# acappemin/Video-to-Audio-and-Piano-RP

Measured on AMD Instinct MI355X. Metric: mel-frames/sec (10s VGGSound shape, 32-step CFM, CFG 2.0), higher is better.
Workload: dtype bf16x3; 1 GPU; BASELINE.json configs[1]: 1 clip(s)/GPU x 750 latent frames x 128 ch, 32-point sway grid = 31 CFG evaluations (62 DiT forwards), T5 context 16 tokens, V2A zero roll; clips_per_gpu=1, global_clips=1, parallelism=clip-sharded x1, 1 all-gather, hipgraph=True, schedule=three streams, side_streams=True, cascade_passes=1

## Files before the change

include/v2a_cfm.h:

```cpp
#ifndef V2A_CFM_H
#define V2A_CFM_H

#include <stdint.h>

#ifdef __cplusplus
extern "C" {
#endif

typedef void* v2a_stream_t;

enum {
  V2A_F32 = 0,
  V2A_BF16 = 1,
  V2A_BF16_SPLIT = 2
};

enum {
  V2A_OK = 0,
  V2A_ERR_ARG = -1,
  V2A_ERR_LAUNCH = -2
};

int v2a_abi_version(void);
const char* v2a_last_error(void);

enum {
  V2A_EPI_STORE = 0,
  V2A_EPI_SIGMOID = 1,
  V2A_EPI_GEGLU = 2,
  V2A_EPI_RESID = 3,
  V2A_EPI_GATE_RESID = 4,
  V2A_EPI_GEGLU_TANH = 5,
  V2A_EPI_GELU = 6,
  V2A_EPI_SWIGLU = 7
};

typedef struct v2a_gemm_args {
  const void* a[3];
  int64_t lda[3];
  int32_t ka[3];
  int32_t nseg;
  int32_t a_dtype;
  const void* w;
  int64_t ldw;
  const float* bias;
  int32_t M, N;
  int32_t compute_dtype;
  int32_t epilogue;
  void* out;
  int64_t ldo;
  int32_t out_dtype;
  void* out_bf16;
  int64_t ld_out_bf16;
  const float* resid;
  int64_t ldr;
  const float* gate;
  const int32_t* step;
  int64_t gate_step_stride, gate_batch_stride;
  int32_t rows_per_batch;
  const float* rope_table;
  int32_t rope_cols, rope_pos_offset;
  int32_t relu;
  const int32_t* a_row_offset;
  const int32_t* a_ktile_offset;
  const int32_t* out_row_offset;
  int32_t tile_hint;
  const float* norm_gamma;
  int64_t norm_step_stride, norm_batch_stride;
  int32_t norm_switch_row, norm_switch_offset;
  float* norm_ssq;
  int64_t ld_norm_ssq;
  const float* row_ssq;
  int64_t ld_row_ssq;
  int32_t row_ssq_parts, row_norm_dim;
  int32_t out_bf16_split;
  int64_t a_lo_offset[3];
  int64_t out_bf16_lo_offset;
} v2a_gemm_args;

int v2a_gemm(const v2a_gemm_args* args, v2a_stream_t stream);
int v2a_gemm_args_size(void);

enum { V2A_GEMM_REGISTER_STAGED = 0, V2A_GEMM_RING = 1, V2A_GEMM_8PHASE = 2 };
typedef struct v2a_gemm_choice {
  int32_t family;
  int32_t split;
  int32_t bm, bn, bk;
  int32_t waves_m, waves_n;
  int32_t stages;
  int32_t tiles;
  int32_t xcd_gm, xcd_gn;
  int32_t vec_epi;
} v2a_gemm_choice;
int v2a_gemm_choose(const v2a_gemm_args* args, v2a_gemm_choice* choice);

typedef struct v2a_tuning {
  int32_t gemm_force_tile;
  int32_t gemm_k_rotation;
  int32_t gemm_8phase;
  int32_t gemm_8phase_min_tiles;
  int32_t dwconv_rows_per_wave;
  int32_t gemm_xcd_order_1x8;
  int32_t attn_one_group_from;
  int32_t reserved[1];
} v2a_tuning;
int v2a_set_tuning(const v2a_tuning* tuning);

int v2a_rmsnorm(const float* x, int64_t ldx, void* y, int64_t ldy, int32_t y_dtype,
                int64_t rows, int32_t d,
                const float* gamma, const int32_t* step, int64_t gamma_step_stride,
                int64_t gamma_batch_stride, int32_t rows_per_batch, v2a_stream_t stream);

int v2a_dwconv_silu_residual(const float* x, float* out, const float* wt, const float* bias,
                             int32_t B, int32_t N, int32_t d, int32_t ksize,
                             const int32_t* len, v2a_stream_t stream);
typedef struct v2a_dwconv_norm {
  void* out_bf16;
  int64_t ld_out_bf16;
  const float* norm_gamma;
  const int32_t* step;
  int64_t norm_step_stride, norm_batch_stride;
  float* norm_ssq;
  int64_t ld_norm_ssq;
  int32_t split;
  int32_t reserved;
} v2a_dwconv_norm;
int v2a_dwconv_silu_residual_norm(const float* x, float* out, const float* wt, const float* bias,
                                  int32_t B, int32_t N, int32_t d, int32_t ksize,
                                  const int32_t* len, const v2a_dwconv_norm* norm, v2a_stream_t stream);

int v2a_rope_inplace(void* qk, int32_t dtype, int64_t rows, int64_t row_stride, int32_t nheads,
                     int32_t rows_per_batch, int32_t pos_offset, const float* cs_table,
                     int32_t layout, v2a_stream_t stream);

typedef struct v2a_attn_args {
  const void *q, *k, *v, *gate;
  void* out;
  int64_t q_row_stride, k_row_stride, v_row_stride, gate_row_stride, out_row_stride;
  int64_t q_batch_stride, k_batch_stride, v_batch_stride, gate_batch_stride, out_batch_stride;
  int32_t B, H, Nq, Nk;
  const int32_t* kv_len;
  const int32_t* q_len;
  float scale, softclamp;
  int32_t dtype;
  int32_t out_split;
} v2a_attn_args;

int v2a_attention(const v2a_attn_args* args, v2a_stream_t stream);
int v2a_qproj_xattn(const v2a_gemm_args* gemm, const v2a_attn_args* attn, v2a_stream_t stream);

typedef struct v2a_xattn_prepare_args {
  const float* ctx_kv;
  int64_t ctx_ld;
  int32_t k_col, v_col;
  const float* wq;
  const float* wo;
  void* wqk;
  void* wvo;
  int32_t B, L, H, D, nc, KP;
} v2a_xattn_prepare_args;
int v2a_xattn_absorb_prepare(const v2a_xattn_prepare_args* args, v2a_stream_t stream);

typedef struct v2a_xattn_absorbed_args {
  const void* a;
  int64_t lda;
  int32_t K, M;
  const void* wqk;
  int64_t ldw, w_batch_stride;
  const float* gate_bias;
  void* out;
  int64_t ldo;
  int32_t rows_per_batch, B, H, KP;
  const int32_t* kv_len;
  const int32_t* q_len;
  float scale, softclamp;
  const float* row_ssq;
  int64_t ld_row_ssq;
  int32_t row_ssq_parts, row_norm_dim;
} v2a_xattn_absorbed_args;
int v2a_xattn_absorbed(const v2a_xattn_absorbed_args* args, v2a_stream_t stream);

int v2a_linear_small(const float* a, int64_t M, int32_t K, const float* wt, const float* bias,
                     const float* add, int32_t T, float* out, int64_t out_batch_stride,
                     int32_t row_off, int32_t d, int32_t dup_batch_offset,
                     const float* regs ,
                     void* out_bf16 , v2a_stream_t stream);

int v2a_fill_registers(float* out, int64_t out_batch_stride, const float* regs, int32_t B,
                       int32_t R, int32_t d, v2a_stream_t stream);

int v2a_time_cond(const float* t, int32_t S, const float* fourier_w, const float* wt,
                  const float* bias, float* out, int32_t d, v2a_stream_t stream);

int v2a_apg_reduce(const float* pred, double* apg, int32_t B, int32_t T, int32_t C,
                   int64_t pred_batch_stride, int32_t row_off,
                   const int32_t* valid_rows ,
                   v2a_stream_t stream);
int v2a_cfg_euler(float* y, const float* pred, int32_t B, int32_t T, int32_t C,
                  int64_t pred_batch_stride, int32_t row_off, float cfg_strength,
                  const float* dt, const int32_t* step, const double* apg,
                  float keep_parallel_frac, v2a_stream_t stream);
typedef struct v2a_y_planes {
  void* planes;
  int64_t ld;
  int64_t lo_offset;
  int32_t row_off;
  int32_t rows_per_seq;
  int32_t copies;
  int32_t reserved;
} v2a_y_planes;
int v2a_cfg_euler_planes(float* y, const float* pred, int32_t B, int32_t T, int32_t C,
                         int64_t pred_batch_stride, int32_t row_off, float cfg_strength,
                         const float* dt, const int32_t* step, const double* apg,
                         float keep_parallel_frac, const v2a_y_planes* planes, v2a_stream_t stream);
int v2a_split_bf16(const float* x, int64_t ldx, void* y, int64_t ldy, int64_t rows, int32_t d, v2a_stream_t stream);
int v2a_cast_bf16(const float* x, void* y, int64_t n, v2a_stream_t stream);
int v2a_step_advance(int32_t* step, v2a_stream_t stream);


int v2a_im2col(const float* x, int32_t B, int32_t H, int32_t W, int32_t C, int32_t kh, int32_t kw, int32_t stride,
               int32_t pad, int32_t Ho, int32_t Wo, void* col, int64_t ldo, int32_t out_dtype, int32_t window_t,
               int32_t window_first, v2a_stream_t stream);

int v2a_frames_pack(const float* frames, void* out, int32_t T, int32_t H, int32_t W, int32_t kw, int32_t stride, int32_t pad,
                    int32_t Wo, v2a_stream_t stream);
int v2a_frames_pack_split(const float* frames, void* out, int64_t lo_offset, int32_t T, int32_t H, int32_t W, int32_t kw,
                          int32_t stride, int32_t pad, int32_t Wo, v2a_stream_t stream);

int v2a_pool2d(const float* x, float* out, void* out_bf16, int32_t B, int32_t H, int32_t W, int32_t C, int32_t k,
               int32_t stride, int32_t pad, int32_t mode, int32_t Ho, int32_t Wo, int32_t in_border, int32_t out_border,
               v2a_stream_t stream);
int v2a_pool2d_split(const float* x, float* out, void* out_split, int64_t lo_offset, int32_t B, int32_t H, int32_t W, int32_t C,
                     int32_t k, int32_t stride, int32_t pad, int32_t mode, int32_t Ho, int32_t Wo, int32_t in_border,
                     int32_t out_border, v2a_stream_t stream);

typedef struct v2a_roll_head_args {
  const float *x2, *x3, *x4, *x5;
  int32_t B, P;
  const float *frb4_w1t, *frb4_b1, *frb4_w2t, *frb4_b2;
  const float *frb3_w1t, *frb3_b1, *frb3_w2t, *frb3_b2;
  const float *frb2_w1t, *frb2_b1, *frb2_w2t, *frb2_b2;
  const float *conv2_wt, *conv2_b;
  const float *fc_wt, *fc_b;
  int32_t notes;
  int32_t apply_sigmoid;
  float* out;
} v2a_roll_head_args;
int v2a_roll_head(const v2a_roll_head_args* args, v2a_stream_t stream);

int v2a_roll_expand(const float* roll, float* out, int32_t B, int32_t t, int32_t notes, int32_t rep, int32_t l,
                    v2a_stream_t stream);

int v2a_roll_expand_ratio(const float* roll, float* out, int32_t B, int32_t t, int32_t notes, int32_t rep, int32_t group, int32_t l,
                          v2a_stream_t stream);


int v2a_elu_pad(const float* x, float* out, int64_t T, int32_t C, int32_t pad, int32_t reflect, int32_t act,
                v2a_stream_t stream);

int v2a_lstm_layer(const float* gates_x, const float* w_hh, float* h, const float* resid, float* y, int32_t T, int32_t H,
                   int32_t* workspace, v2a_stream_t stream);

int v2a_lstm2(const float* gates_x0, const float* w_hh0, const float* w_ih1, const float* bias1, const float* w_hh1,
              const float* resid, float* y, int32_t T, int32_t H, int32_t* workspace, v2a_stream_t stream);


int v2a_elu_pad_lr(const float* x, float* out, int64_t T, int32_t C, int32_t pad_left, int32_t pad_right, int32_t act,
                   v2a_stream_t stream);

int v2a_encodec_stage0(const float* wave, const float* params, float* out, int64_t n, v2a_stream_t stream);


int v2a_t5_rmsnorm(const float* x, int64_t ldx, const int32_t* ids, int32_t vocab, float* resid, int64_t ldr, float* y, int64_t ldy,
                   int64_t rows, int32_t d, const float* w, float eps, v2a_stream_t stream);

typedef struct v2a_t5_attn_args {
  const float *q, *k, *v;
  float* out;
  int64_t q_row_stride, k_row_stride, v_row_stride, out_row_stride;
  int64_t q_batch_stride, k_batch_stride, v_batch_stride, out_batch_stride;
  int32_t B, H, N, d_kv;
  const float* bias;
  const int32_t* key_mask;
} v2a_t5_attn_args;
int v2a_t5_attention(const v2a_t5_attn_args* args, v2a_stream_t stream);

int v2a_gemm_skinny_f32(const v2a_gemm_args* args, v2a_stream_t stream);


int v2a_clip_resize_h(const uint8_t* frames, int32_t F, int32_t H, int32_t W, uint8_t* tmp, int32_t y0, int32_t rows, int32_t S,
                      const int32_t* bounds, const int32_t* coef, int32_t ksize, v2a_stream_t stream);
int v2a_clip_resize_v(const uint8_t* tmp, int32_t F, int32_t rows, int32_t S, int32_t P, const int32_t* bounds, const int32_t* coef,
                      int32_t ksize, const float* lut, void* patches, int64_t ldp, int32_t out_dtype, int64_t lo_offset, uint8_t* crop,
                      v2a_stream_t stream);
int v2a_clip_embed_init(float* h, int64_t ldh, int64_t rows, int32_t T, int32_t d, const float* cls, const float* pos,
                        v2a_stream_t stream);
int v2a_clip_layernorm(const float* x, int64_t ldx, void* y, int64_t ldy, int32_t y_dtype, int64_t rows, int32_t d, const float* gamma,
                       const float* beta, float eps, v2a_stream_t stream);
typedef struct v2a_clip_attn_args {
  const float *q, *k, *v;
  void* out;
  int64_t row_stride, batch_stride;
  int64_t out_row_stride, out_batch_stride;
  int32_t B, H, N, d_head;
  float scale;
  int32_t out_split;
} v2a_clip_attn_args;
int v2a_clip_attention(const v2a_clip_attn_args* args, v2a_stream_t stream);


int v2a_piano_resize_h(const uint8_t* frames, int32_t F, int32_t H, int32_t W, const int32_t* sel, int32_t n, uint8_t* tmp, int32_t ldt,
                       int32_t y0, int32_t rows, int32_t Wo, const int32_t* bounds, const int32_t* coef, int32_t ksize,
                       v2a_stream_t stream);
int v2a_piano_resize_v(const uint8_t* tmp, int32_t n, int32_t rows, int32_t ldt, int32_t Ho, int32_t Wo, const int32_t* bounds,
                       const int32_t* coef, int32_t ksize, const float* lut, float* out, v2a_stream_t stream);
int v2a_piano_resize_vt(const uint8_t* tmp, int32_t n, int32_t rows, int32_t ldt, int32_t Ho, int32_t Wo, const int32_t* bounds,
                        const int32_t* coef, int32_t ksize, const float* lut, float* out, v2a_stream_t stream);


int v2a_encodec_rvq_encode(const float* x, int64_t batch_stride, int64_t frame_stride, int64_t chan_stride, int32_t B, int32_t T,
                           const float* codebooks, const float* norms, int32_t S, int32_t Kc, int32_t D, int32_t n_q, int64_t* codes,
                           v2a_stream_t stream);
int v2a_encodec_rvq_decode(const int64_t* codes, int32_t n_q, int32_t B, int32_t T, const float* codebooks, int32_t S, int32_t Kc, int32_t D,
                           float* out, int64_t batch_stride, int64_t frame_stride, int64_t chan_stride, v2a_stream_t stream);


#define V2A_LOSS_MAX_PARTS 256

int v2a_cfm_interp(const float* x0, const float* x1, const float* t, const uint8_t* span, float* w, float* flow, float* cond, int32_t B,
                   int32_t T, int32_t C, v2a_stream_t stream);
int v2a_masked_sqerr(const float* pred, const float* target, const uint8_t* mask, int32_t B, int32_t T, int32_t C, double* scratch,
                     double* out, v2a_stream_t stream);
int v2a_roll_metrics(const float* roll, const float* midis, const uint8_t* mask, int32_t B, int32_t T, int32_t notes, double* scratch,
                     double* out, v2a_stream_t stream);


#define V2A_WAVE_MAX_PARTS 256
#define V2A_WAVE_LDS_BYTES (128 * 1024)
#define V2A_WAVE_TABLE_MAX (1 << 22)

int v2a_wave_resample(const float* x, int64_t L, const float* table, int32_t o, int32_t n, int32_t K, int32_t width, float* y,
                      int64_t out_len, void* parts, int32_t* n_parts, v2a_stream_t stream);
int v2a_wave_stats(const float* x, int64_t n, void* parts, int32_t* n_parts, v2a_stream_t stream);
int v2a_wave_normalize(const float* x, int64_t n, const void* parts, int32_t n_parts, float* out, int64_t n_out, float* stats,
                       v2a_stream_t stream);


int v2a_roll2midi_stem(const float* x, const float* wt, int32_t n, int32_t H, int32_t W, int32_t co, float* out, void* shadow,
                       int32_t shadow_mode, int64_t lo_offset, int64_t pitch, int32_t border, v2a_stream_t stream);
int v2a_leaky_shadow(float* x, void* shadow, int32_t shadow_mode, int64_t lo_offset, int32_t n, int32_t H, int32_t W, int32_t C,
                     int64_t pitch, int32_t border, v2a_stream_t stream);
int v2a_roll2midi_head(const float* u, int64_t u_pitch, int32_t nu, const float* d, int64_t d_pitch, int32_t nd, const float* w,
                       float bias, float threshold, int32_t n, int32_t H, int32_t W, int32_t border, float* logits, float* probs,
                       uint8_t* midi, v2a_stream_t stream);
int v2a_roll2midi_gate(float* x0, int64_t pitch0, int32_t C0, void* shadow0, int64_t lo_offset0, float* x1, int64_t pitch1, int32_t C1,
                       void* shadow1, int64_t lo_offset1, const float* w, float bias, int32_t shadow_mode, int32_t n, int32_t H, int32_t W,
                       int32_t border, float* logits, float* alpha, v2a_stream_t stream);


#define V2A_ROLL_NOTES_MAX_KEYS 128
#define V2A_ROLL_NOTES_TILE 256
#define V2A_ROLL_NOTES_MAX_FRAMES (1 << 24)

int v2a_roll_notes(const void* roll, int32_t elem_bytes, int64_t batch_stride, int64_t frame_stride, int64_t key_stride, float threshold,
                   int32_t B, int32_t T, int32_t keys, const int32_t* lens, int32_t* counts, int32_t* totals, int32_t* notes, int32_t cap,
                   int8_t* onset, v2a_stream_t stream);


#define V2A_MEL_MAX_FFT 2048
#define V2A_MEL_MAX_CHUNKS 16
// ... 27 lines not shown
```

video-to-audio-and-piano-rp_amd/_lib.py:

```python
from __future__ import annotations

import ctypes as C
import os
import subprocess
from typing import NamedTuple

import torch

_HERE = os.path.dirname(os.path.abspath(__file__))
LIB_PATH = os.path.join(_HERE, "libv2a_cfm.so")
CSRC = os.path.join(_HERE, "csrc")

F32, BF16, BF16_SPLIT = 0, 1, 2
EPI_STORE, EPI_SIGMOID, EPI_GEGLU, EPI_RESID, EPI_GATE_RESID = 0, 1, 2, 3, 4
EPI_GEGLU_TANH = 5
EPI_GELU = 6
EPI_SWIGLU = 7

_lib = None


class V2AError(RuntimeError):
    pass


class GemmArgs(C.Structure):
    _fields_ = [
        ("a", C.c_void_p * 3), ("lda", C.c_int64 * 3), ("ka", C.c_int32 * 3),
        ("nseg", C.c_int32), ("a_dtype", C.c_int32),
        ("w", C.c_void_p), ("ldw", C.c_int64), ("bias", C.c_void_p),
        ("M", C.c_int32), ("N", C.c_int32), ("compute_dtype", C.c_int32), ("epilogue", C.c_int32),
        ("out", C.c_void_p), ("ldo", C.c_int64), ("out_dtype", C.c_int32),
        ("out_bf16", C.c_void_p), ("ld_out_bf16", C.c_int64),
        ("resid", C.c_void_p), ("ldr", C.c_int64),
        ("gate", C.c_void_p), ("step", C.c_void_p),
        ("gate_step_stride", C.c_int64), ("gate_batch_stride", C.c_int64), ("rows_per_batch", C.c_int32),
        ("rope_table", C.c_void_p), ("rope_cols", C.c_int32), ("rope_pos_offset", C.c_int32), ("relu", C.c_int32),
        ("a_row_offset", C.c_void_p), ("a_ktile_offset", C.c_void_p), ("out_row_offset", C.c_void_p),
        ("tile_hint", C.c_int32),
        ("norm_gamma", C.c_void_p), ("norm_step_stride", C.c_int64), ("norm_batch_stride", C.c_int64),
        ("norm_switch_row", C.c_int32), ("norm_switch_offset", C.c_int32),
        ("norm_ssq", C.c_void_p), ("ld_norm_ssq", C.c_int64),
        ("row_ssq", C.c_void_p), ("ld_row_ssq", C.c_int64), ("row_ssq_parts", C.c_int32), ("row_norm_dim", C.c_int32),
        ("out_bf16_split", C.c_int32),
        ("a_lo_offset", C.c_int64 * 3), ("out_bf16_lo_offset", C.c_int64),
    ]


class GemmChoice(C.Structure):
    _fields_ = [(n, C.c_int32) for n in ("family", "split", "bm", "bn", "bk", "waves_m", "waves_n", "stages", "tiles", "xcd_gm", "xcd_gn",
                                         "vec_epi")]


GEMM_REGISTER_STAGED, GEMM_RING, GEMM_8PHASE = 0, 1, 2

TILE_128x128, TILE_8PHASE, TILE_128x128_8WAVES, TILE_128x64_8WAVES = 1, 6, 12, 14
SPLIT_TILE_8PHASE, SPLIT_TILE_128x256_K32 = 5, 6


class DwconvNorm(C.Structure):
    _fields_ = [("out_bf16", C.c_void_p), ("ld_out_bf16", C.c_int64), ("norm_gamma", C.c_void_p), ("step", C.c_void_p),
                ("norm_step_stride", C.c_int64), ("norm_batch_stride", C.c_int64), ("norm_ssq", C.c_void_p), ("ld_norm_ssq", C.c_int64),
                ("split", C.c_int32), ("reserved", C.c_int32)]


class Tuning(C.Structure):
    _fields_ = [("gemm_force_tile", C.c_int32), ("gemm_k_rotation", C.c_int32), ("gemm_8phase", C.c_int32),
                ("gemm_8phase_min_tiles", C.c_int32), ("dwconv_rows_per_wave", C.c_int32), ("gemm_xcd_order_1x8", C.c_int32),
                ("attn_one_group_from", C.c_int32), ("reserved", C.c_int32 * 1)]


class AttnArgs(C.Structure):
    _fields_ = [
        ("q", C.c_void_p), ("k", C.c_void_p), ("v", C.c_void_p), ("gate", C.c_void_p), ("out", C.c_void_p),
        ("q_row_stride", C.c_int64), ("k_row_stride", C.c_int64), ("v_row_stride", C.c_int64),
        ("gate_row_stride", C.c_int64), ("out_row_stride", C.c_int64),
        ("q_batch_stride", C.c_int64), ("k_batch_stride", C.c_int64), ("v_batch_stride", C.c_int64),
        ("gate_batch_stride", C.c_int64), ("out_batch_stride", C.c_int64),
        ("B", C.c_int32), ("H", C.c_int32), ("Nq", C.c_int32), ("Nk", C.c_int32),
        ("kv_len", C.c_void_p), ("q_len", C.c_void_p),
        ("scale", C.c_float), ("softclamp", C.c_float), ("dtype", C.c_int32), ("out_split", C.c_int32),
    ]


class XattnPrepareArgs(C.Structure):
    _fields_ = [("ctx_kv", C.c_void_p), ("ctx_ld", C.c_int64), ("k_col", C.c_int32), ("v_col", C.c_int32),
                ("wq", C.c_void_p), ("wo", C.c_void_p), ("wqk", C.c_void_p), ("wvo", C.c_void_p)] + \
               [(n, C.c_int32) for n in ("B", "L", "H", "D", "nc", "KP")]


class XattnAbsorbedArgs(C.Structure):
    _fields_ = [("a", C.c_void_p), ("lda", C.c_int64), ("K", C.c_int32), ("M", C.c_int32),
                ("wqk", C.c_void_p), ("ldw", C.c_int64), ("w_batch_stride", C.c_int64), ("gate_bias", C.c_void_p),
                ("out", C.c_void_p), ("ldo", C.c_int64),
                ("rows_per_batch", C.c_int32), ("B", C.c_int32), ("H", C.c_int32), ("KP", C.c_int32),
                ("kv_len", C.c_void_p), ("q_len", C.c_void_p), ("scale", C.c_float), ("softclamp", C.c_float),
                ("row_ssq", C.c_void_p), ("ld_row_ssq", C.c_int64), ("row_ssq_parts", C.c_int32), ("row_norm_dim", C.c_int32)]


class YPlanes(C.Structure):
    _fields_ = [("planes", C.c_void_p), ("ld", C.c_int64), ("lo_offset", C.c_int64), ("row_off", C.c_int32), ("rows_per_seq", C.c_int32),
                ("copies", C.c_int32), ("reserved", C.c_int32)]


class T5AttnArgs(C.Structure):
    _fields_ = [
        ("q", C.c_void_p), ("k", C.c_void_p), ("v", C.c_void_p), ("out", C.c_void_p),
        ("q_row_stride", C.c_int64), ("k_row_stride", C.c_int64), ("v_row_stride", C.c_int64), ("out_row_stride", C.c_int64),
        ("q_batch_stride", C.c_int64), ("k_batch_stride", C.c_int64), ("v_batch_stride", C.c_int64), ("out_batch_stride", C.c_int64),
        ("B", C.c_int32), ("H", C.c_int32), ("N", C.c_int32), ("d_kv", C.c_int32),
        ("bias", C.c_void_p), ("key_mask", C.c_void_p),
    ]


class ClipAttnArgs(C.Structure):
    _fields_ = [("q", C.c_void_p), ("k", C.c_void_p), ("v", C.c_void_p), ("out", C.c_void_p),
                ("row_stride", C.c_int64), ("batch_stride", C.c_int64), ("out_row_stride", C.c_int64), ("out_batch_stride", C.c_int64),
                ("B", C.c_int32), ("H", C.c_int32), ("N", C.c_int32), ("d_head", C.c_int32), ("scale", C.c_float), ("out_split", C.c_int32)]


class RollHeadArgs(C.Structure):
    _fields_ = ([(n, C.c_void_p) for n in ("x2", "x3", "x4", "x5")] + [("B", C.c_int32), ("P", C.c_int32)] +
                [(f"frb{i}_{n}", C.c_void_p) for i in (4, 3, 2) for n in ("w1t", "b1", "w2t", "b2")] +
                [(n, C.c_void_p) for n in ("conv2_wt", "conv2_b", "fc_wt", "fc_b")] +
                [("notes", C.c_int32), ("apply_sigmoid", C.c_int32), ("out", C.c_void_p)])


EXPORTS = [
    "v2a_abi_version", "v2a_last_error", "v2a_gemm", "v2a_gemm_args_size", "v2a_gemm_choose", "v2a_set_tuning", "v2a_rmsnorm", "v2a_dwconv_silu_residual", "v2a_dwconv_silu_residual_norm",
    "v2a_rope_inplace", "v2a_attention", "v2a_qproj_xattn", "v2a_linear_small", "v2a_fill_registers", "v2a_time_cond",
    "v2a_apg_reduce", "v2a_cfg_euler", "v2a_step_advance", "v2a_cast_bf16", "v2a_split_bf16",
    "v2a_im2col", "v2a_frames_pack", "v2a_pool2d", "v2a_roll_head", "v2a_roll_expand", "v2a_frames_pack_split", "v2a_pool2d_split",
    "v2a_elu_pad", "v2a_lstm_layer", "v2a_lstm2", "v2a_t5_rmsnorm", "v2a_t5_attention", "v2a_gemm_skinny_f32",
    "v2a_clip_resize_h", "v2a_clip_resize_v", "v2a_clip_embed_init", "v2a_clip_layernorm", "v2a_clip_attention",
    "v2a_elu_pad_lr", "v2a_encodec_stage0", "v2a_piano_resize_h", "v2a_piano_resize_v",
    "v2a_encodec_rvq_encode", "v2a_encodec_rvq_decode", "v2a_cfm_interp", "v2a_masked_sqerr", "v2a_roll_metrics",
    "v2a_wave_resample", "v2a_wave_stats", "v2a_wave_normalize",
    "v2a_roll2midi_stem", "v2a_leaky_shadow", "v2a_roll2midi_head", "v2a_roll2midi_gate",
    "v2a_xattn_absorb_prepare", "v2a_xattn_absorbed",
    "v2a_roll_expand_ratio", "v2a_piano_resize_vt",
    "v2a_roll_notes",
    "v2a_cfg_euler_planes",
    "v2a_mel_pad", "v2a_mel_from_dft",
    "v2a_vocos_stage_in", "v2a_vocos_dwconv_ln", "v2a_vocos_gelu", "v2a_vocos_scale_residual", "v2a_vocos_spectrum", "v2a_vocos_overlap_add",
]


def build(force: bool = False, verbose: bool = False) -> str:
    if force:
        for f in os.listdir(os.path.join(CSRC, "build")) if os.path.isdir(os.path.join(CSRC, "build")) else []:
            os.remove(os.path.join(CSRC, "build", f))
    r = subprocess.run(["bash", os.path.join(CSRC, "build.sh")], capture_output=True, text=True)
    if verbose or r.returncode != 0:
        print(r.stdout[-4000:])
        print(r.stderr[-8000:])
    if r.returncode != 0:
        raise V2AError("hipcc build of libv2a_cfm.so failed")
    return LIB_PATH


ABI_VERSION = 9


def _declare(lib):
    vp, i32, i64, f32 = C.c_void_p, C.c_int32, C.c_int64, C.c_float
    lib.v2a_abi_version.restype = C.c_int
    lib.v2a_last_error.restype = C.c_char_p
    lib.v2a_gemm.argtypes = [C.POINTER(GemmArgs), vp]
    lib.v2a_gemm_args_size.restype = C.c_int
    lib.v2a_gemm_choose.argtypes = [C.POINTER(GemmArgs), C.POINTER(GemmChoice)]
    lib.v2a_set_tuning.argtypes = [C.POINTER(Tuning)]
    lib.v2a_attention.argtypes = [C.POINTER(AttnArgs), vp]
    lib.v2a_qproj_xattn.argtypes = [C.POINTER(GemmArgs), C.POINTER(AttnArgs), vp]
    lib.v2a_xattn_absorb_prepare.argtypes = [C.POINTER(XattnPrepareArgs), vp]
    lib.v2a_xattn_absorbed.argtypes = [C.POINTER(XattnAbsorbedArgs), vp]
    lib.v2a_rmsnorm.argtypes = [vp, i64, vp, i64, i32, i64, i32, vp, vp, i64, i64, i32, vp]
    lib.v2a_dwconv_silu_residual.argtypes = [vp, vp, vp, vp, i32, i32, i32, i32, vp, vp]
    lib.v2a_dwconv_silu_residual_norm.argtypes = [vp, vp, vp, vp, i32, i32, i32, i32, vp, C.POINTER(DwconvNorm), vp]
    lib.v2a_rope_inplace.argtypes = [vp, i32, i64, i64, i32, i32, i32, vp, i32, vp]
    lib.v2a_linear_small.argtypes = [vp, i64, i32, vp, vp, vp, i32, vp, i64, i32, i32, i32, vp, vp, vp]
    lib.v2a_fill_registers.argtypes = [vp, i64, vp, i32, i32, i32, vp]
    lib.v2a_time_cond.argtypes = [vp, i32, vp, vp, vp, vp, i32, vp]
    lib.v2a_apg_reduce.argtypes = [vp, vp, i32, i32, i32, i64, i32, vp, vp]
    lib.v2a_cfg_euler.argtypes = [vp, vp, i32, i32, i32, i64, i32, f32, vp, vp, vp, f32, vp]
    lib.v2a_cfg_euler_planes.argtypes = [vp, vp, i32, i32, i32, i64, i32, f32, vp, vp, vp, f32, C.POINTER(YPlanes), vp]
    lib.v2a_step_advance.argtypes = [vp, vp]
    lib.v2a_cast_bf16.argtypes = [vp, vp, i64, vp]
    lib.v2a_split_bf16.argtypes = [vp, i64, vp, i64, i64, i32, vp]
    lib.v2a_im2col.argtypes = [vp, i32, i32, i32, i32, i32, i32, i32, i32, i32, i32, vp, i64, i32, i32, i32, vp]
    lib.v2a_frames_pack.argtypes = [vp, vp, i32, i32, i32, i32, i32, i32, i32, vp]
    lib.v2a_pool2d.argtypes = [vp, vp, vp, i32, i32, i32, i32, i32, i32, i32, i32, i32, i32, i32, i32, vp]
    lib.v2a_frames_pack_split.argtypes = [vp, vp, i64, i32, i32, i32, i32, i32, i32, i32, vp]
    lib.v2a_pool2d_split.argtypes = [vp, vp, vp, i64, i32, i32, i32, i32, i32, i32, i32, i32, i32, i32, i32, i32, vp]
    lib.v2a_roll_head.argtypes = [C.POINTER(RollHeadArgs), vp]
    lib.v2a_roll_expand.argtypes = [vp, vp, i32, i32, i32, i32, i32, vp]
    lib.v2a_roll_expand_ratio.argtypes = [vp, vp, i32, i32, i32, i32, i32, i32, vp]
    lib.v2a_elu_pad.argtypes = [vp, vp, i64, i32, i32, i32, i32, vp]
    lib.v2a_lstm_layer.argtypes = [vp, vp, vp, vp, vp, i32, i32, vp, vp]
    lib.v2a_lstm2.argtypes = [vp, vp, vp, vp, vp, vp, vp, i32, i32, vp, vp]
    lib.v2a_t5_rmsnorm.argtypes = [vp, i64, vp, i32, vp, i64, vp, i64, i64, i32, vp, f32, vp]
    lib.v2a_t5_attention.argtypes = [C.POINTER(T5AttnArgs), vp]
    lib.v2a_gemm_skinny_f32.argtypes = [C.POINTER(GemmArgs), vp]
    lib.v2a_clip_resize_h.argtypes = [vp, i32, i32, i32, vp, i32, i32, i32, vp, vp, i32, vp]
    lib.v2a_clip_resize_v.argtypes = [vp, i32, i32, i32, i32, vp, vp, i32, vp, vp, i64, i32, i64, vp, vp]
    lib.v2a_clip_embed_init.argtypes = [vp, i64, i64, i32, i32, vp, vp, vp]
    lib.v2a_clip_layernorm.argtypes = [vp, i64, vp, i64, i32, i64, i32, vp, vp, f32, vp]
    lib.v2a_clip_attention.argtypes = [C.POINTER(ClipAttnArgs), vp]
    lib.v2a_elu_pad_lr.argtypes = [vp, vp, i64, i32, i32, i32, i32, vp]
    lib.v2a_encodec_stage0.argtypes = [vp, vp, vp, i64, vp]
    lib.v2a_piano_resize_h.argtypes = [vp, i32, i32, i32, vp, i32, vp, i32, i32, i32, i32, vp, vp, i32, vp]
    lib.v2a_piano_resize_v.argtypes = [vp, i32, i32, i32, i32, i32, vp, vp, i32, vp, vp, vp]
    lib.v2a_piano_resize_vt.argtypes = lib.v2a_piano_resize_v.argtypes
    lib.v2a_encodec_rvq_encode.argtypes = [vp, i64, i64, i64, i32, i32, vp, vp, i32, i32, i32, i32, vp, vp]
    lib.v2a_encodec_rvq_decode.argtypes = [vp, i32, i32, i32, vp, i32, i32, i32, vp, i64, i64, i64, vp]
    lib.v2a_cfm_interp.argtypes = [vp, vp, vp, vp, vp, vp, vp, i32, i32, i32, vp]
    lib.v2a_masked_sqerr.argtypes = [vp, vp, vp, i32, i32, i32, vp, vp, vp]
    lib.v2a_roll_metrics.argtypes = [vp, vp, vp, i32, i32, i32, vp, vp, vp]
    lib.v2a_wave_resample.argtypes = [vp, i64, vp, i32, i32, i32, i32, vp, i64, vp, C.POINTER(i32), vp]
    lib.v2a_wave_stats.argtypes = [vp, i64, vp, C.POINTER(i32), vp]
    lib.v2a_wave_normalize.argtypes = [vp, i64, vp, i32, vp, i64, vp, vp]
    lib.v2a_roll2midi_stem.argtypes = [vp, vp, i32, i32, i32, i32, vp, vp, i32, i64, i64, i32, vp]
    lib.v2a_leaky_shadow.argtypes = [vp, vp, i32, i64, i32, i32, i32, i32, i64, i32, vp]
    lib.v2a_roll2midi_head.argtypes = [vp, i64, i32, vp, i64, i32, vp, f32, f32, i32, i32, i32, i32, vp, vp, vp, vp]
    lib.v2a_roll2midi_gate.argtypes = [vp, i64, i32, vp, i64, vp, i64, i32, vp, i64, vp, f32, i32, i32, i32, i32, i32, vp, vp, vp]
    lib.v2a_roll_notes.argtypes = [vp, i32, i64, i64, i64, f32, i32, i32, i32, vp, vp, vp, vp, i32, vp, vp]
    lib.v2a_mel_pad.argtypes = [vp, i64, i32, i64, i32, vp, i64, vp]
    lib.v2a_mel_from_dft.argtypes = [vp, i64, i64, i32, i64, i32, i32, i32, i32, i32, vp, vp, vp, i32, i32, f32, vp, i64, i64, vp]
    lib.v2a_vocos_stage_in.argtypes = [vp, i64, i64, i32, i32, i32, vp, vp, i32, vp]
    lib.v2a_vocos_dwconv_ln.argtypes = [vp, i64, vp, vp, vp, vp, f32, i32, i32, i64, i32, vp, vp, i64, vp]
    lib.v2a_vocos_gelu.argtypes = [vp, i64, i64, i32, vp]
    lib.v2a_vocos_scale_residual.argtypes = [vp, i64, vp, vp, i64, vp, i64, i64, i32, vp]
    lib.v2a_vocos_spectrum.argtypes = [vp, i64, i64, i32, vp, i64, vp]
    lib.v2a_vocos_overlap_add.argtypes = [vp, i64, i64, vp, i32, i32, i32, i32, vp, vp, i64, vp]
    for name in EXPORTS:
        if name not in ("v2a_abi_version", "v2a_last_error", "v2a_gemm_args_size"):
            getattr(lib, name).restype = C.c_int


def lib():
    global _lib
    if _lib is None:
        if not os.path.exists(LIB_PATH):
            raise V2AError(f"{LIB_PATH} is missing: run `python -c 'import __graft_entry__ as g; g.build()'` "
                           "(hipcc --offload-arch=gfx950).  There is no CPU fallback for the sampler.")
        _lib = C.CDLL(LIB_PATH)
        _declare(_lib)
        if _lib.v2a_abi_version() != ABI_VERSION:
            raise V2AError("libv2a_cfm.so reports ABI version %d, this binding was written for %d: rebuild (csrc/build.sh)"
                           % (_lib.v2a_abi_version(), ABI_VERSION))
        if _lib.v2a_gemm_args_size() != C.sizeof(GemmArgs):
            raise V2AError("libv2a_cfm.so was built with sizeof(v2a_gemm_args) = %d, this binding mirrors %d bytes: rebuild "
                           "(csrc/build.sh)" % (_lib.v2a_gemm_args_size(), C.sizeof(GemmArgs)))
    return _lib


def set_tuning(force_tile: int = -1, k_rotation: bool = False, eight_phase: int | None = None, eight_phase_min_tiles: int = 0,
               dwconv_rows_per_wave: int = 0, xcd_order_1x8: bool = False, attn_one_group_from: int = 0, reserved: int = 0):
    if (force_tile == -1 and not k_rotation and eight_phase is None and eight_phase_min_tiles == 0 and dwconv_rows_per_wave == 0
            and not xcd_order_1x8 and attn_one_group_from == 0 and not reserved):
        check(lib().v2a_set_tuning(None))
        return
    t = Tuning(force_tile, 1 if k_rotation else 0, 1 if eight_phase is None else eight_phase, eight_phase_min_tiles, dwconv_rows_per_wave,
               1 if xcd_order_1x8 else 0, attn_one_group_from, (C.c_int32 * 1)(reserved))
    check(lib().v2a_set_tuning(C.byref(t)))


def check(rc: int):
    if rc != 0:
        raise V2AError(f"v2a_cfm call failed ({rc}): {lib().v2a_last_error().decode()}")


def stream_ptr() -> int:
    return torch.cuda.current_stream().cuda_stream


def dt_code(t: torch.dtype) -> int:
    if t == torch.float32:
        return F32
    if t == torch.bfloat16:
        return BF16
    raise V2AError(f"unsupported dtype {t}")


def _p(t):
    return 0 if t is None else t.data_ptr()


class Operand(NamedTuple):
    t: torch.Tensor
    ld: int
    k: int
    lo: int = 0


def split_planes(w):
    w = w.float()
    hi = w.bfloat16()
    return torch.cat([hi, (w - hi.float()).bfloat16()], 1)


_prof = None


class KernelProfiler:

    def __init__(self, shapes: bool = False, inner: int = 1, external: bool = False):
        self.recs = []
        self.shapes = shapes
        self.inner = inner
        self.external = external
        self.marks, self.end, self.tot = [], None, {}

    def launch(self, key, flops, nbytes, call):
        if self.external:
            e = torch.cuda.Event(enable_timing=True, external=True)
            e.record()
            self.marks.append((key, flops, nbytes, e))
            call()
            return
        n = self.inner if key.startswith("gemm") else 1
        s, e = torch.cuda.Event(enable_timing=True), torch.cuda.Event(enable_timing=True)
        s.record()
        for _ in range(n):
            call()
        e.record()
        self.recs.append((key, flops, nbytes, s, e, n))

    def close(self):
        self.end = torch.cuda.Event(enable_timing=True, external=True)
        self.end.record()

    def collect(self):
        for i, (key, flops, nbytes, e) in enumerate(self.marks):
            nxt = self.marks[i + 1][3] if i + 1 < len(self.marks) else self.end
            a = self.tot.setdefault(key, dict(launches=0, ms=0.0, flops=0.0, bytes=0.0))
            a["launches"] += 1
            a["ms"] += e.elapsed_time(nxt)
            a["flops"] += flops
            a["bytes"] += nbytes
# ... 106 lines not shown
    _launch("rmsnorm<%s>" % ("f32" if y.dtype == torch.float32 else ("bf16x2" if split else "bf16")), 0.0,
            rows * d * (4 + y.element_size() * (2 if split else 1)),
            lambda: lib().v2a_rmsnorm(x.data_ptr(), ldx or d, y.data_ptr(), ldy or d, ydt, rows, d,
                                      gamma.data_ptr(), _p(step), gamma_step_stride, gamma_batch_stride, rows_per_batch,
                                      stream_ptr()))


def _dwconv_norm(norm, d):
    n = DwconvNorm()
    n.out_bf16, n.ld_out_bf16 = norm["out_bf16"].data_ptr(), norm.get("ld_out_bf16", d)
    n.norm_gamma, n.step = norm["gamma"].data_ptr(), _p(norm.get("step"))
    n.norm_step_stride, n.norm_batch_stride = norm.get("step_stride", 0), norm.get("batch_stride", 0)
    n.norm_ssq, n.ld_norm_ssq = norm["ssq"].data_ptr(), norm["ssq"].stride(-2)
    n.split = 1 if norm.get("split") else 0
    if n.split:
        n.ld_out_bf16 = norm.get("ld_out_bf16", 2 * d)
    return n


def dwconv(x, out, wt, bias, *, B, N, d, ksize, lens=None, norm=None):
    if norm is None:
        _launch("dwconv", 2.0 * B * N * d * ksize, B * N * d * 8,
                lambda: lib().v2a_dwconv_silu_residual(x.data_ptr(), out.data_ptr(), wt.data_ptr(), bias.data_ptr(),
                                                       B, N, d, ksize, _p(lens), stream_ptr()))
        return
    n = _dwconv_norm(norm, d)
    _launch("dwconv+norm", 2.0 * B * N * d * ksize, B * N * d * (12 if n.split else 10),
            lambda: lib().v2a_dwconv_silu_residual_norm(x.data_ptr(), out.data_ptr(), wt.data_ptr(), bias.data_ptr(),
                                                        B, N, d, ksize, _p(lens), C.byref(n), stream_ptr()))


def rope(qk, *, rows, row_stride, nheads, rows_per_batch, pos_offset, table, layout):
    _launch("rope<%s>" % ("f32" if qk.dtype == torch.float32 else "bf16"), 0.0, rows * nheads * 64 * 2 * qk.element_size(),
            lambda: lib().v2a_rope_inplace(qk.data_ptr(), dt_code(qk.dtype), rows, row_stride, nheads, rows_per_batch,
                                           pos_offset, table.data_ptr(), layout, stream_ptr()))


def attention(q, k, v, gate, out, **kw):
    a, key, flops, nbytes = attention_args(q, k, v, gate, out, **kw)
    _launch(key, flops, nbytes, lambda: lib().v2a_attention(C.byref(a), stream_ptr()))


def attention_args(q, k, v, gate, out, *, strides, B, H, Nq, Nk, kv_len=None, q_len=None, scale, softclamp, dtype, out_split=False):
    a = AttnArgs()
    a.q, a.k, a.v, a.gate, a.out = q, k, v, gate, out
    (a.q_row_stride, a.k_row_stride, a.v_row_stride, a.gate_row_stride, a.out_row_stride,
     a.q_batch_stride, a.k_batch_stride, a.v_batch_stride, a.gate_batch_stride, a.out_batch_stride) = strides
    a.B, a.H, a.Nq, a.Nk = B, H, Nq, Nk
    a.kv_len, a.q_len = _p(kv_len), _p(q_len)
    a.scale, a.softclamp, a.dtype = scale, softclamp, dtype
    a.out_split = 1 if out_split else 0
    esz = 2 if dtype == BF16 else 4
    return a, "attention<%s>" % {BF16: "bf16", F32: "f32", BF16_SPLIT: "bf16x3"}[dtype], 4.0 * B * H * Nq * Nk * 64, B * H * 64 * (2 * Nq + 2 * Nk) * esz


def qproj_xattn(a, lda, K, w, *, bias, M, N, rows_per_batch, k, v, out, kv_strides, out_strides, B, H, Nk, kv_len=None, q_len=None,
                scale, softclamp, rope_table=None, rope_cols=0, rope_pos_offset=0, row_ssq=None, row_norm_dim=0, split=False):
    g = GemmArgs()
    g.a[0], g.lda[0], g.ka[0], g.nseg = a.data_ptr(), lda, K, 1
    g.compute_dtype = BF16
    g.a_dtype = BF16_SPLIT if split else BF16
    g.w, g.ldw = w.data_ptr(), w.stride(0)
    g.bias = _p(bias)
    g.M, g.N = M, N
    g.epilogue = EPI_STORE
    g.out_dtype = F32 if split else BF16
    g.rows_per_batch = rows_per_batch
    g.rope_table = _p(rope_table)
    g.rope_cols, g.rope_pos_offset = rope_cols, rope_pos_offset
    g.row_ssq = _p(row_ssq)
    g.ld_row_ssq = row_ssq.stride(-2) if row_ssq is not None else 0
    g.row_ssq_parts = row_norm_dim // 32 if row_ssq is not None else 0
    g.row_norm_dim = row_norm_dim
    t = AttnArgs()
    t.k, t.v, t.out = k, v, out
    t.k_row_stride, t.v_row_stride, t.k_batch_stride, t.v_batch_stride = kv_strides
    t.out_row_stride, t.out_batch_stride = out_strides
    t.B, t.H, t.Nq, t.Nk = B, H, rows_per_batch, Nk
    t.kv_len, t.q_len = _p(kv_len), _p(q_len)
    t.scale, t.softclamp, t.dtype = scale, softclamp, (BF16_SPLIT if split else BF16)
    t.out_split = 1 if split else 0
    _launch("qproj_xattn<%s>" % ("bf16x3" if split else "bf16"), (3.0 if split else 1.0) * (2.0 * M * (H * 65) * K + 4.0 * B * H * rows_per_batch * Nk * 64),
            M * K * 2 + H * 65 * K * 2 + M * H * 64 * 2 + 2 * B * Nk * H * 64 * 2,
            lambda: lib().v2a_qproj_xattn(C.byref(g), C.byref(t), stream_ptr()))


def xattn_kp(nc):
    return 16 if nc <= 16 else 32


def xattn_absorb_prepare(ctx_kv, wq, wo, wqk, wvo, *, B, L, H, D, nc, KP, k_col, v_col):
    a = XattnPrepareArgs()
    a.ctx_kv, a.ctx_ld, a.k_col, a.v_col = ctx_kv.data_ptr(), ctx_kv.stride(-2), k_col, v_col
    a.wq, a.wo, a.wqk, a.wvo = wq.data_ptr(), wo.data_ptr(), wqk.data_ptr(), wvo.data_ptr()
    a.B, a.L, a.H, a.D, a.nc, a.KP = B, L, H, D, nc, KP
    _launch("xattn_absorb_prepare", 4.0 * B * L * H * KP * 64 * D,
            L * (2 * H * 64 + H) * D * 4 + B * L * ((H * KP + H) * D + D * H * KP) * 4 + 2 * B * nc * L * H * 64 * 4,
            lambda: lib().v2a_xattn_absorb_prepare(C.byref(a), stream_ptr()))


def xattn_absorbed(a, lda, K, wqk, out, *, ldw, w_batch_stride, ldo, M, rows_per_batch, B, H, KP, kv_len, q_len=None, gate_bias=None,
                   scale, softclamp, row_ssq=None, row_norm_dim=0):
    g = XattnAbsorbedArgs()
    g.a, g.lda, g.K, g.M = a.data_ptr(), lda, K, M
    g.wqk, g.ldw, g.w_batch_stride, g.gate_bias = wqk.data_ptr(), ldw, w_batch_stride, _p(gate_bias)
    g.out, g.ldo = out.data_ptr(), ldo
    g.rows_per_batch, g.B, g.H, g.KP = rows_per_batch, B, H, KP
    g.kv_len, g.q_len = _p(kv_len), _p(q_len)
    g.scale, g.softclamp = scale, softclamp
    g.row_ssq = _p(row_ssq)
    g.ld_row_ssq = row_ssq.stride(-2) if row_ssq is not None else 0
    g.row_ssq_parts = row_norm_dim // 32 if row_ssq is not None else 0
    g.row_norm_dim = row_norm_dim
    n = H * KP + H
    _launch("xattn_absorbed<bf16x3>", 6.0 * M * n * K, (M * K + B * n * K + M * H * KP) * 4,
            lambda: lib().v2a_xattn_absorbed(C.byref(g), stream_ptr()))


def linear_small(a, wt, bias, add, out, *, M, K, T, out_batch_stride, row_off, d, dup=0, regs=None, out_bf16=None):
    _launch("linear_small", 2.0 * M * K * d, M * (K + d) * 4,
            lambda: lib().v2a_linear_small(a.data_ptr(), M, K, wt.data_ptr(), _p(bias), _p(add), T, out.data_ptr(),
                                           out_batch_stride, row_off, d, dup, _p(regs), _p(out_bf16), stream_ptr()))


def fill_registers(out, regs, *, B, R, d, out_batch_stride):
    check(lib().v2a_fill_registers(out.data_ptr(), out_batch_stride, regs.data_ptr(), B, R, d, stream_ptr()))


def time_cond(t, fourier_w, wt, bias, out, *, S, d):
    check(lib().v2a_time_cond(t.data_ptr(), S, fourier_w.data_ptr(), wt.data_ptr(), bias.data_ptr(),
                              out.data_ptr(), d, stream_ptr()))


def apg_reduce(pred, apg, *, B, T, C_, pred_batch_stride, row_off, valid_rows=None):
    check(lib().v2a_apg_reduce(pred.data_ptr(), apg.data_ptr(), B, T, C_, pred_batch_stride, row_off, _p(valid_rows), stream_ptr()))


def cfg_euler(y, pred, *, B, T, C_, pred_batch_stride, row_off, cfg_strength, dt, step=None, apg=None, keep=0.0, planes=None):
    if planes is None:
        _launch("cfg_euler", 0.0, 16.0 * B * T * C_,
                lambda: lib().v2a_cfg_euler(y.data_ptr(), pred.data_ptr(), B, T, C_, pred_batch_stride, row_off,
                                            float(cfg_strength), dt.data_ptr(), _p(step), _p(apg), float(keep), stream_ptr()))
        return
    pl = YPlanes(planes["out"].data_ptr(), planes["ld"], planes["lo_offset"], planes["row_off"], planes["rows_per_seq"], planes["copies"], 0)
    _launch("cfg_euler", 0.0, (16.0 + 4.0 * planes["copies"]) * B * T * C_,
            lambda: lib().v2a_cfg_euler_planes(y.data_ptr(), pred.data_ptr(), B, T, C_, pred_batch_stride, row_off, float(cfg_strength),
                                               dt.data_ptr(), _p(step), _p(apg), float(keep), C.byref(pl), stream_ptr()))


def step_advance(step):
    check(lib().v2a_step_advance(step.data_ptr(), stream_ptr()))


def split_bf16(x, y, *, rows, d, ldx=None, ldy=None):
    _launch("split_bf16", 0.0, rows * d * 8, lambda: lib().v2a_split_bf16(x.data_ptr(), ldx or d, y.data_ptr(), ldy or 2 * d, rows, d, stream_ptr()))


def cast_bf16(x, y):
    _launch("cast_bf16", 0.0, x.numel() * 6, lambda: lib().v2a_cast_bf16(x.data_ptr(), y.data_ptr(), x.numel(), stream_ptr()))


def im2col(x, col, *, B, H, W, C_, kh, kw, stride, pad, Ho, Wo, ldo, window_t=0, window_first=0):
    K = kh * kw * C_
    _launch("im2col<%s>" % ("f32" if col.dtype == torch.float32 else "bf16"), 0.0, B * Ho * Wo * (4.0 * K + col.element_size() * ldo),
            lambda: lib().v2a_im2col(x.data_ptr(), B, H, W, C_, kh, kw, stride, pad, Ho, Wo, col.data_ptr(), ldo,
                                     dt_code(col.dtype), window_t, window_first, stream_ptr()))


def frames_pack(frames, out, *, T, H, W, kw, stride, pad, Wo):
    _launch("frames_pack", 0.0, 4.0 * T * H * W + 32.0 * (T + 4) * Wo * (H + 2 * pad),
            lambda: lib().v2a_frames_pack(frames.data_ptr(), out.data_ptr(), T, H, W, kw, stride, pad, Wo, stream_ptr()))


def frames_pack_split(frames, out, *, lo_offset, T, H, W, kw, stride, pad, Wo):
    _launch("frames_pack_split", 0.0, 4.0 * T * H * W + 64.0 * (T + 4) * Wo * (H + 2 * pad),
            lambda: lib().v2a_frames_pack_split(frames.data_ptr(), out.data_ptr(), lo_offset, T, H, W, kw, stride, pad, Wo, stream_ptr()))


def pool2d(x, out, *, B, H, W, C_, k, stride, pad, mode, Ho, Wo, out_bf16=None, in_border=0, out_border=0):
    _launch("pool2d", 0.0, 4.0 * B * C_ * (H * W + Ho * Wo),
            lambda: lib().v2a_pool2d(x.data_ptr(), out.data_ptr(), _p(out_bf16), B, H, W, C_, k, stride, pad, mode, Ho, Wo,
                                     in_border, out_border, stream_ptr()))


def pool2d_split(x, out, out_split, *, lo_offset, B, H, W, C_, k, stride, pad, mode, Ho, Wo, in_border=0, out_border=0):
    _launch("pool2d_split", 0.0, 4.0 * B * C_ * (H * W + 2 * Ho * Wo),
            lambda: lib().v2a_pool2d_split(x.data_ptr(), out.data_ptr(), out_split.data_ptr(), lo_offset, B, H, W, C_, k, stride, pad,
                                           mode, Ho, Wo, in_border, out_border, stream_ptr()))


def roll_head(args: "RollHeadArgs"):
    _launch("roll_head", 0.0, 4.0 * args.B * args.P * (3 * 128 + 64), lambda: lib().v2a_roll_head(C.byref(args), stream_ptr()))


def roll_expand(roll, out, *, B, t, notes, rep, l):
    check(lib().v2a_roll_expand(roll.data_ptr(), out.data_ptr(), B, t, notes, rep, l, stream_ptr()))


def roll_expand_ratio(roll, out, *, B, t, notes, rep, group, l):
    check(lib().v2a_roll_expand_ratio(roll.data_ptr(), out.data_ptr(), B, t, notes, rep, group, l, stream_ptr()))


SH_NONE, SH_BF16, SH_SPLIT = 0, 1, 2


def roll2midi_stem(x, wt, out, shadow, *, n, H, W, co, shadow_mode, lo_offset, pitch, border):
    _launch("roll2midi_stem", 18.0 * n * H * W * co, n * H * W * (4.0 + co * (4 + 2 * shadow_mode)),
            lambda: lib().v2a_roll2midi_stem(x.data_ptr(), wt.data_ptr(), n, H, W, co, out.data_ptr(), _p(shadow), shadow_mode, lo_offset,
                                             pitch, border, stream_ptr()))


def leaky_shadow(x, shadow, *, n, H, W, C_, shadow_mode, lo_offset, pitch, border):
    _launch("leaky_shadow", 0.0, n * H * W * C_ * (8.0 + 2 * shadow_mode),
            lambda: lib().v2a_leaky_shadow(x.data_ptr(), _p(shadow), shadow_mode, lo_offset, n, H, W, C_, pitch, border, stream_ptr()))


def roll2midi_head(u, d, w, *, u_pitch, nu, d_pitch, nd, bias, threshold, n, H, W, border, logits=None, probs=None, midi=None):
    _launch("roll2midi_head", 2.0 * n * H * W * (nu + nd), n * H * W * (4.0 * (nu + nd) + 9),
            lambda: lib().v2a_roll2midi_head(u.data_ptr(), u_pitch, nu, d.data_ptr(), d_pitch, nd, w.data_ptr(), float(bias), float(threshold),
                                             n, H, W, border, _p(logits), _p(probs), _p(midi), stream_ptr()))


def roll2midi_gate(seg0, seg1, w, *, bias, shadow_mode, n, H, W, border, logits=None, alpha=None):
    x0, p0, c0, s0, l0 = seg0
    x1, p1, c1, s1, l1 = seg1 if seg1 is not None else (None, 0, 0, None, 0)
    _launch("roll2midi_gate", 2.0 * n * H * W * (c0 + c1), n * H * W * (c0 + c1) * (8.0 + 2 * shadow_mode) + 4.0 * (c0 + c1),
            lambda: lib().v2a_roll2midi_gate(x0.data_ptr(), p0, c0, _p(s0), l0, _p(x1), p1, c1, _p(s1), l1, w.data_ptr(), float(bias),
                                             shadow_mode, n, H, W, border, _p(logits), _p(alpha), stream_ptr()))


ROLL_NOTES_MAX_KEYS, ROLL_NOTES_TILE, ROLL_NOTES_MAX_FRAMES = 128, 256, 1 << 24


def roll_notes(roll, counts, totals, notes, *, strides, B, T, keys, cap, threshold=0.0, lens=None, onset=None):
    _launch("roll_notes<%s>" % ("f32" if roll.dtype == torch.float32 else "u8"), 0.0, 2.0 * B * T * keys * roll.element_size(),
            lambda: lib().v2a_roll_notes(roll.data_ptr(), roll.element_size(), strides[0], strides[1], strides[2], float(threshold), B, T, keys,
                                         _p(lens), counts.data_ptr(), totals.data_ptr(), _p(notes), cap, _p(onset), stream_ptr()))


def elu_pad(x, out, *, T, C_, pad, reflect, act=True):
    _launch("elu_pad", 0.0, 4.0 * C_ * (2 * T + pad),
            lambda: lib().v2a_elu_pad(x.data_ptr(), out.data_ptr(), T, C_, pad, 1 if reflect else 0, 1 if act else 0, stream_ptr()))


def elu_pad_lr(x, out, *, T, C_, pad_left, pad_right, act=True):
    _launch("elu_pad_lr", 0.0, 4.0 * C_ * (2 * T + pad_left + pad_right),
            lambda: lib().v2a_elu_pad_lr(x.data_ptr(), out.data_ptr(), T, C_, pad_left, pad_right, 1 if act else 0, stream_ptr()))


ENCODEC_STAGE0_PARAMS = 3376


def encodec_stage0(wave, params, out, *, n):
    _launch("encodec_stage0", 2.0 * n * 3744, 4.0 * n * 33,
            lambda: lib().v2a_encodec_stage0(wave.data_ptr(), params.data_ptr(), out.data_ptr(), n, stream_ptr()))


def encodec_rvq_encode(x, strides, codebooks, norms, codes, *, B, T, n_q):
    S, Kc, D = codebooks.shape
    _launch("encodec_rvq_encode", 2.0 * B * T * n_q * Kc * D, 4.0 * (B * T * D + n_q * Kc * D * -(-B * T // 16)) + 8.0 * n_q * B * T,
            lambda: lib().v2a_encodec_rvq_encode(x.data_ptr(), strides[0], strides[1], strides[2], B, T, codebooks.data_ptr(), norms.data_ptr(),
                                                 S, Kc, D, n_q, codes.data_ptr(), stream_ptr()))


def encodec_rvq_decode(codes, codebooks, out, strides, *, B, T, n_q):
    S, Kc, D = codebooks.shape
    _launch("encodec_rvq_decode", 1.0 * B * T * n_q * D, B * T * (4.0 * D * (n_q + 1) + 8.0 * n_q),
            lambda: lib().v2a_encodec_rvq_decode(codes.data_ptr(), n_q, B, T, codebooks.data_ptr(), S, Kc, D, out.data_ptr(),
                                                 strides[0], strides[1], strides[2], stream_ptr()))


LOSS_MAX_PARTS = 256


def cfm_interp(x0, x1, t, span, w, flow, cond=None):
    B, T, C_ = x1.shape
    _launch("cfm_interp", 4.0 * B * T * C_, 4.0 * B * T * C_ * (4 if cond is None else 5),
            lambda: lib().v2a_cfm_interp(x0.data_ptr(), x1.data_ptr(), t.data_ptr(), _p(span), w.data_ptr(), flow.data_ptr(), _p(cond),
                                         B, T, C_, stream_ptr()))


def masked_sqerr(pred, target, mask, out):
    B, T, C_ = pred.shape
    scratch = torch.empty(LOSS_MAX_PARTS * 2, dtype=torch.float64, device=pred.device)
    _launch("masked_sqerr", 3.0 * B * T * C_, 8.0 * B * T * C_,
            lambda: lib().v2a_masked_sqerr(pred.data_ptr(), target.data_ptr(), mask.data_ptr(), B, T, C_, scratch.data_ptr(), out.data_ptr(),
                                           stream_ptr()))


def roll_metrics(roll, midis, mask, out):
    B, T, notes = roll.shape
    scratch = torch.empty(LOSS_MAX_PARTS * 6, dtype=torch.float64, device=roll.device)
    _launch("roll_metrics", 5.0 * B * T * notes, 16.0 * B * T * notes,
            lambda: lib().v2a_roll_metrics(roll.data_ptr(), midis.data_ptr(), mask.data_ptr(), B, T, notes, scratch.data_ptr(), out.data_ptr(),
                                           stream_ptr()))


def lstm_layer(gates_x, w_hh, h, workspace, *, T, H, resid=None, y=None):
    _launch("lstm_layer", 2.0 * T * 4 * H * H, 4.0 * T * 6 * H,
            lambda: lib().v2a_lstm_layer(gates_x.data_ptr(), w_hh.data_ptr(), h.data_ptr(), _p(resid), _p(y), T, H,
                                         workspace.data_ptr(), stream_ptr()))


def lstm2(gates_x0, w_hh0, w_ih1, bias1, w_hh1, y, workspace, *, T, H, resid=None):
    _launch("lstm2", 2.0 * T * 4 * H * H * 3, 4.0 * T * 6 * H,
            lambda: lib().v2a_lstm2(gates_x0.data_ptr(), w_hh0.data_ptr(), w_ih1.data_ptr(), bias1.data_ptr(), w_hh1.data_ptr(),
# ... 38 lines not shown
```

video-to-audio-and-piano-rp_amd/csrc/gemm.hip:

```cpp
#include "gemm_common.h"

namespace {


template <typename T, bool A_F32, int EPI, typename OutT, int BM, int BN>
__global__ __launch_bounds__(256) void gemm_kernel(GemmParams p) {
  constexpr int BK = TileCfg<T>::BK;
  constexpr int LR = TileCfg<T>::LDS_ROW;
  constexpr int WM = BM / 2, WN = BN / 2;
  constexpr int TM = WM / 16, TN = WN / 16;
  static_assert(!is_glu(EPI) || (TN % 2 == 0), "GEGLU / SWIGLU need value/gate tile pairs");

  extern __shared__ __attribute__((aligned(16))) char smem_raw[];
  T* smem = reinterpret_cast<T*>(smem_raw);
  constexpr int STAGE_ELEMS = (BM + BN) * LR;

  const int tid = threadIdx.x;
  const int lane = tid & 63;
  const int wave = tid >> 6;
  const int wm = wave >> 1, wn = wave & 1;
  const int lr = lane & 15, lq = lane >> 4;

  const int tiles_n = (p.N + BN - 1) / BN;
  const int tiles_m = (p.M + BM - 1) / BM;
  const int bid = xcd_chunk_position(blockIdx.x, tiles_m * tiles_n);
  const int tm = bid / tiles_n, tn = bid % tiles_n;
  const int m0 = tm * BM, n0 = tn * BN;

  f32x4 acc[TM][TN];
#pragma unroll
  for (int i = 0; i < TM; ++i)
#pragma unroll
    for (int j = 0; j < TN; ++j) acc[i][j] = f32x4{0.f, 0.f, 0.f, 0.f};

  typename StageSel<T, A_F32, BM>::type sa;
  typename StageSel<T, false, BN>::type sw;

  const int nk = p.K / BK;

  auto seg_load = [&](int kt) {
    const int k0 = kt * BK;
    int s = 0, kbeg = 0;
    if (p.nseg > 1 && k0 >= p.kend[0]) { s = 1; kbeg = p.kend[0]; }
    if (p.nseg > 2 && k0 >= p.kend[1]) { s = 2; kbeg = p.kend[1]; }
    sa.load(p.a[s], p.lda[s], m0, p.M, k0 - kbeg, tid);
    sw.load(p.w, p.ldw, n0, p.N, k0, tid);
  };

  seg_load(0);
  sa.store(smem, tid);
  sw.store(smem + BM * LR, tid);
  __syncthreads();

  for (int kt = 0; kt < nk; ++kt) {
    const T* As = smem + (kt & 1) * STAGE_ELEMS;
    const T* Ws = As + BM * LR;
    if (kt + 1 < nk) seg_load(kt + 1);

    if constexpr (sizeof(T) == 2) {
#pragma unroll
      for (int kk = 0; kk < 2; ++kk) {
        bf16x8 af[TM], bf[TN];
#pragma unroll
        for (int i = 0; i < TM; ++i) {
          const int row = wm * WM + i * 16 + lr;
          af[i] = *reinterpret_cast<const bf16x8*>(As + row * 64 + (((kk * 4 + lq) ^ (row & 7)) << 3));
        }
#pragma unroll
        for (int j = 0; j < TN; ++j) {
          const int row = wn * WN + j * 16 + lr;
          bf[j] = *reinterpret_cast<const bf16x8*>(Ws + row * 64 + (((kk * 4 + lq) ^ (row & 7)) << 3));
        }
#pragma unroll
        for (int i = 0; i < TM; ++i)
#pragma unroll
          for (int j = 0; j < TN; ++j)
            acc[i][j] = __builtin_amdgcn_mfma_f32_16x16x32_bf16(af[i], bf[j], acc[i][j], 0, 0, 0);
      }
    } else {
#pragma unroll
      for (int kk = 0; kk < 4; ++kk) {
        float af[TM], bf[TN];
#pragma unroll
        for (int i = 0; i < TM; ++i) af[i] = As[(wm * WM + i * 16 + lr) * 20 + kk * 4 + lq];
#pragma unroll
        for (int j = 0; j < TN; ++j) bf[j] = Ws[(wn * WN + j * 16 + lr) * 20 + kk * 4 + lq];
#pragma unroll
        for (int i = 0; i < TM; ++i)
#pragma unroll
          for (int j = 0; j < TN; ++j)
            acc[i][j] = __builtin_amdgcn_mfma_f32_16x16x4f32(af[i], bf[j], acc[i][j], 0, 0, 0);
      }
    }

    if (kt + 1 < nk) {
      T* An = smem + ((kt + 1) & 1) * STAGE_ELEMS;
      sa.store(An, tid);
      sw.store(An + BM * LR, tid);
    }
    __syncthreads();
  }

  gemm_epilogue<EPI, OutT, TM, TN, WM, WN>(p, acc, m0, n0, wm, wn, lr, lq);
}

template <typename T, bool A_F32, int EPI, typename OutT, int BM, int BN>
int launch(const GemmParams& p, GemmTarget to) {
  constexpr int LR = TileCfg<T>::LDS_ROW;
  constexpr size_t smem = 2 * (size_t)(BM + BN) * LR * sizeof(T);
  const int tiles = ((p.M + BM - 1) / BM) * ((p.N + BN - 1) / BN);
  auto kern = gemm_kernel<T, A_F32, EPI, OutT, BM, BN>;
  if (to.chosen(p, V2A_GEMM_REGISTER_STAGED, false, BM, BN, TileCfg<T>::BK, 2, 2, 2, tiles)) return V2A_OK;
  if constexpr (smem > 48 * 1024) {
    static std::atomic<uint64_t> lds_set{0};
    if (int rc = v2a_enable_lds(reinterpret_cast<const void*>(kern), smem, lds_set, "v2a_gemm")) return rc;
  }
  hipLaunchKernelGGL(kern, dim3(tiles), dim3(256), smem, to.stream, p);
  return v2a_check_launch("v2a_gemm");
}

template <typename T, bool A_F32, int BM, int BN>
int dispatch_epi(const v2a_gemm_args* a, const GemmParams& p, GemmTarget to) {
  const bool out_f32 = a->out_dtype == V2A_F32;
  switch (a->epilogue) {
    case V2A_EPI_STORE:
      if (out_f32) return launch<T, A_F32, V2A_EPI_STORE, float, BM, BN>(p, to);
      if constexpr (sizeof(T) == 2) return launch<T, A_F32, V2A_EPI_STORE, bf16_t, BM, BN>(p, to);
      break;
    case V2A_EPI_SIGMOID:
      if (out_f32) return launch<T, A_F32, V2A_EPI_SIGMOID, float, BM, BN>(p, to);
      break;
    case V2A_EPI_GELU:
      if (out_f32) return launch<T, A_F32, V2A_EPI_GELU, float, BM, BN>(p, to);
      break;
    case V2A_EPI_GEGLU:
      if (out_f32) {
        if constexpr (sizeof(T) == 4) return launch<T, A_F32, V2A_EPI_GEGLU, float, BM, BN>(p, to);
      } else {
        if constexpr (sizeof(T) == 2) return launch<T, A_F32, V2A_EPI_GEGLU, bf16_t, BM, BN>(p, to);
      }
      break;
    case V2A_EPI_SWIGLU:
      if constexpr (sizeof(T) == 4) {
        if (out_f32) return launch<T, A_F32, V2A_EPI_SWIGLU, float, BM, BN>(p, to);
      }
      break;
    case V2A_EPI_RESID:
      if (out_f32) return launch<T, A_F32, V2A_EPI_RESID, float, BM, BN>(p, to);
      break;
    case V2A_EPI_GATE_RESID:
      if (out_f32) return launch<T, A_F32, V2A_EPI_GATE_RESID, float, BM, BN>(p, to);
      break;
  }
  return v2a_fail(V2A_ERR_ARG, "v2a_gemm: unsupported epilogue %d / out_dtype %d for compute dtype %d", a->epilogue,
                  a->out_dtype, a->compute_dtype);
}



template <int EPI, typename OutT, int BM, int BN, int WGM, int WGN, int NST = 3, bool S3 = false, int BK = 64>
__global__ __launch_bounds__(64 * WGM * WGN) void gemm_bf16_dma_kernel(const GemmParams p) {
  static_assert(BK == 64 || BK == 32, "K extent of a stage");
  constexpr int NW = WGM * WGN;
  constexpr int WM = BM / WGM, WN = BN / WGN;
  constexpr int TM = WM / 16, TN = WN / 16;
  constexpr int ROWB = BK * 2;
  constexpr int RPG = 1024 / ROWB;
  constexpr int CPR = BK / 8;
  constexpr int KK = BK / 32;
  constexpr int PLANE_BYTES = (BM + BN) * ROWB;
  constexpr int STAGE_BYTES = PLANE_BYTES * (S3 ? 2 : 1);
  constexpr int GA = BM / RPG, GW = BN / RPG;
  constexpr int LPW = (GA + GW) / NW;
  static_assert((GA + GW) % NW == 0, "DMA groups must divide evenly over the waves");
  auto swz = [](int row) { return BK == 64 ? (row & 7) : (((row >> 3) & 1) * 3); };
  static_assert(!is_glu(EPI) || (TN % 2 == 0), "GEGLU / SWIGLU need value/gate tile pairs");
  extern __shared__ __attribute__((aligned(16))) char smem_raw[];

  const int tid = threadIdx.x;
  const int lane = tid & 63;
  const int wave = __builtin_amdgcn_readfirstlane(tid >> 6);
  const int wm = wave / WGN, wn = wave % WGN;
  const int lr = lane & 15, lq = lane >> 4;

  int tm, tn;
  tile_of_block(p, blockIdx.x, tm, tn);
  const int m0 = tm * BM, n0 = tn * BN;

  f32x4 acc[TM][TN];
#pragma unroll
  for (int i = 0; i < TM; ++i)
#pragma unroll
    for (int j = 0; j < TN; ++j) acc[i][j] = f32x4{0.f, 0.f, 0.f, 0.f};

  const int srow = lane / CPR;
  const int schunk = ((lane % CPR) ^ swz(srow)) << 3;
  int grow[LPW];
  uint32_t goff[LPW];
  auto set_offsets = [&](int64_t lda) {
#pragma unroll
    for (int i = 0; i < LPW; ++i) {
      const int g = wave + i * NW;
      const int64_t rbase = g < GA ? (p.a_rowoff ? (int64_t)p.a_rowoff[grow[i]] : (int64_t)grow[i] * lda) : (int64_t)grow[i] * p.ldw;
      goff[i] = (uint32_t)((rbase + schunk) * 2);
    }
  };
#pragma unroll
  for (int i = 0; i < LPW; ++i) {
    const int g = wave + i * NW;
    if (g < GA) {
      const int r = m0 + g * RPG + srow;
      grow[i] = r < p.M ? r : p.M - 1;
    } else {
      const int r = n0 + (g - GA) * RPG + srow;
      grow[i] = r < p.N ? r : p.N - 1;
    }
  }
  set_offsets(p.lda[0]);
  typedef const __attribute__((address_space(4))) int32_t* const_i32_ptr;
  const const_i32_ptr koff_tab = (const_i32_ptr)p.a_koff;

  const char* a_run = reinterpret_cast<const char*>(p.a[0]);
  const char* w_run = reinterpret_cast<const char*>(p.w);
  const char* const a_first = a_run;
  const int nseg = p.nseg;
  int seg = 0;
  int seg_left = (nseg > 1 ? p.kend[0] : p.K) / BK;
  int64_t a_lo_bytes = S3 ? p.alo[0] * 2 : 0;
  const int64_t w_lo_bytes = S3 ? (int64_t)p.K * 2 : 0;
  int kt_next = 0;
  auto issue = [&](int stage) {
    if (seg_left == 0) {
      ++seg;
      a_run = reinterpret_cast<const char*>(seg == 1 ? p.a[1] : p.a[2]);
      seg_left = (seg == 1 ? (nseg > 2 ? p.kend[1] : p.K) - p.kend[0] : p.K - p.kend[1]) / BK;
      if constexpr (S3) a_lo_bytes = (seg == 1 ? p.alo[1] : p.alo[2]) * 2;
      set_offsets(seg == 1 ? p.lda[1] : p.lda[2]);
    }
    const char* ab = a_run;
    if (koff_tab) ab = a_first + (int64_t)koff_tab[kt_next] * 2;
    const char* wb = w_run;
    char* st = smem_raw + stage * STAGE_BYTES;
#pragma unroll
    for (int i = 0; i < LPW; ++i) {
      const int g = wave + i * NW;
      if (g < GA)
        __builtin_amdgcn_global_load_lds((const __attribute__((address_space(1))) void*)(ab + goff[i]),
                                         (__attribute__((address_space(3))) void*)(st + g * 1024), 16, 0, 0);
      else
        __builtin_amdgcn_global_load_lds((const __attribute__((address_space(1))) void*)(wb + goff[i]),
                                         (__attribute__((address_space(3))) void*)(st + g * 1024), 16, 0, 0);
    }
    if constexpr (S3) {
#pragma unroll
      for (int i = 0; i < LPW; ++i) {
        const int g = wave + i * NW;
        if (g < GA)
          __builtin_amdgcn_global_load_lds((const __attribute__((address_space(1))) void*)(ab + a_lo_bytes + goff[i]),
                                           (__attribute__((address_space(3))) void*)(st + PLANE_BYTES + g * 1024), 16, 0, 0);
        else
          __builtin_amdgcn_global_load_lds((const __attribute__((address_space(1))) void*)(wb + w_lo_bytes + goff[i]),
                                           (__attribute__((address_space(3))) void*)(st + PLANE_BYTES + g * 1024), 16, 0, 0);
      }
    }
    a_run += ROWB;
    w_run += ROWB;
    --seg_left;
    ++kt_next;
  };

  constexpr bool PF = BM * BN <= 128 * 256 && !((EPI == V2A_EPI_GATE_RESID || EPI == V2A_EPI_STORE) && BM * BN == 128 * 256);
  EpiPrefetch<EPI, TM, WN, PF> pf;
  if (p.vec_epi) pf.load(p, m0 + wm * WM, n0 + wn * WN, lane);
  static_assert(BM <= 64 * NW, "one thread per tile row");
  float* rs_lds = reinterpret_cast<float*>(smem_raw + NST * STAGE_BYTES);
  const bool scaled = p.rssq != nullptr && p.vec_epi;
  RowScaleLoad rsl;
  if (scaled && tid < BM) rowscale_load(p, m0 + tid, rsl);
  const int nk = p.K / BK;
#pragma unroll
  for (int s0 = 0; s0 < NST - 1; ++s0)
    if (s0 < nk) issue(s0);
  if (scaled && tid < BM) rs_lds[tid] = rowscale_finish(p, rsl);
  auto tile = [&](auto stage_c, int kt) {
    constexpr int STAGE = decltype(stage_c)::value;
#ifdef V2A_GEMM_PROBE
    if (!(p.dbg & 2))
#endif
    ring_wait<NST - 2 < 0 ? 0 : NST - 2, LPW * (S3 ? 2 : 1)>(nk - 1 - kt);
    __builtin_amdgcn_s_barrier();
#ifdef V2A_GEMM_PROBE
    if (p.dbg & 1) {
      if (kt + NST - 1 < nk) issue((STAGE + NST - 1) % NST);
      return;
    }
#endif
    const bf16_t* As = reinterpret_cast<const bf16_t*>(smem_raw + STAGE * STAGE_BYTES);
    const bf16_t* Ws = As + BM * BK;
    bf16x8 af[KK][TM], bf[KK][TN];
#pragma unroll
    for (int kk = 0; kk < KK; ++kk) {
#pragma unroll
      for (int i = 0; i < TM; ++i) {
        const int row = wm * WM + i * 16 + lr;
        af[kk][i] = *reinterpret_cast<const bf16x8*>(As + row * BK + (((kk * 4 + lq) ^ swz(row)) << 3));
      }
#pragma unroll
      for (int j = 0; j < TN; ++j) {
        const int row = wn * WN + j * 16 + lr;
        bf[kk][j] = *reinterpret_cast<const bf16x8*>(Ws + row * BK + (((kk * 4 + lq) ^ swz(row)) << 3));
      }
    }
    if constexpr (S3) {
      const bf16_t* Al = As + PLANE_BYTES / 2;
      const bf16_t* Wl = Al + BM * BK;
      bf16x8 afl[KK][TM], bfl[KK][TN];
#pragma unroll
      for (int kk = 0; kk < KK; ++kk) {
#pragma unroll
        for (int i = 0; i < TM; ++i) {
          const int row = wm * WM + i * 16 + lr;
          afl[kk][i] = *reinterpret_cast<const bf16x8*>(Al + row * BK + (((kk * 4 + lq) ^ swz(row)) << 3));
        }
#pragma unroll
        for (int j = 0; j < TN; ++j) {
          const int row = wn * WN + j * 16 + lr;
          bfl[kk][j] = *reinterpret_cast<const bf16x8*>(Wl + row * BK + (((kk * 4 + lq) ^ swz(row)) << 3));
        }
      }
#ifdef V2A_GEMM_PROBE
      if (!(p.dbg & 2))
#endif
      if (kt + NST - 1 < nk) issue((STAGE + NST - 1) % NST);
#pragma unroll
      for (int kk = 0; kk < KK; ++kk)
#pragma unroll
        for (int i = 0; i < TM; ++i)
#pragma unroll
          for (int j = 0; j < TN; ++j) {
#ifdef V2A_GEMM_PROBE
            if (!(p.dbg & 32)) {
              acc[i][j] = __builtin_amdgcn_mfma_f32_16x16x32_bf16(afl[kk][i], bf[kk][j], acc[i][j], 0, 0, 0);
              acc[i][j] = __builtin_amdgcn_mfma_f32_16x16x32_bf16(af[kk][i], bfl[kk][j], acc[i][j], 0, 0, 0);
            }
#else
            acc[i][j] = __builtin_amdgcn_mfma_f32_16x16x32_bf16(afl[kk][i], bf[kk][j], acc[i][j], 0, 0, 0);
            acc[i][j] = __builtin_amdgcn_mfma_f32_16x16x32_bf16(af[kk][i], bfl[kk][j], acc[i][j], 0, 0, 0);
#endif
            acc[i][j] = __builtin_amdgcn_mfma_f32_16x16x32_bf16(af[kk][i], bf[kk][j], acc[i][j], 0, 0, 0);
          }
    } else {
#ifdef V2A_GEMM_PROBE
    if (!(p.dbg & 2))
#endif
    if (kt + NST - 1 < nk) issue((STAGE + NST - 1) % NST);
#pragma unroll
    for (int kk = 0; kk < KK; ++kk)
#pragma unroll
      for (int i = 0; i < TM; ++i)
#pragma unroll
        for (int j = 0; j < TN; ++j)
          acc[i][j] = __builtin_amdgcn_mfma_f32_16x16x32_bf16(af[kk][i], bf[kk][j], acc[i][j], 0, 0, 0);
    if constexpr (BK == 64) {
      constexpr int NL = TM + TN, NM = TM * TN, PER = NM / NL > 0 ? NM / NL : 1;
      __builtin_amdgcn_sched_group_barrier(0x100, NL, 0);
      __builtin_amdgcn_sched_group_barrier(0x020, LPW, 0);
#pragma unroll
      for (int l = 0; l < NL; ++l) {
        __builtin_amdgcn_sched_group_barrier(0x008, PER, 0);
        __builtin_amdgcn_sched_group_barrier(0x100, 1, 0);
      }
      __builtin_amdgcn_sched_group_barrier(0x008, 2 * NM - PER * NL, 0);
    }
    }
  };
  static_assert(NST >= 2 && NST <= 6, "ring depth");
  for (int kt = 0; kt < nk; kt += NST) {
    tile(std::integral_constant<int, 0>{}, kt);
    if (kt + 1 < nk) tile(std::integral_constant<int, 1>{}, kt + 1);
    if constexpr (NST > 2) { if (kt + 2 < nk) tile(std::integral_constant<int, 2>{}, kt + 2); }
    if constexpr (NST > 3) { if (kt + 3 < nk) tile(std::integral_constant<int, 3>{}, kt + 3); }
    if constexpr (NST > 4) { if (kt + 4 < nk) tile(std::integral_constant<int, 4>{}, kt + 4); }
    if constexpr (NST > 5) { if (kt + 5 < nk) tile(std::integral_constant<int, 5>{}, kt + 5); }
  }
  if (p.vec_epi) {
    __builtin_amdgcn_s_barrier();
    static_assert(NW * 16 * (WN + 4) * 4 <= NST * STAGE_BYTES, "epilogue slabs must fit in the ring memory");
    float* tile = reinterpret_cast<float*>(smem_raw) + wave * (16 * (WN + 4));
    gemm_epilogue_lds<EPI, OutT, TM, TN, WM, WN, PF>(p, acc, tile, m0 + wm * WM, n0 + wn * WN, lane, pf, scaled ? rs_lds + wm * WM : nullptr);
  } else {
    gemm_epilogue<EPI, OutT, TM, TN, WM, WN>(p, acc, m0, n0, wm, wn, lr, lq);
  }
}

template <int EPI, typename OutT, int BM, int BN, int WGM, int WGN, int NST, bool S3 = false, int BK = 64>
int launch_dma(const GemmParams& p_in, GemmTarget to) {
  GemmParams p = p_in;
  v2a_detail::fill_tile_map(p, BM, BN);
  V2A_REQUIRE((int64_t)p.tiles_m * p.tiles_n < (1 << 24), "v2a_gemm: %d x %d tiles exceed the tile map", p.tiles_m, p.tiles_n);
  constexpr size_t smem = NST * (size_t)(BM + BN) * (BK * 2) * (S3 ? 2 : 1) + BM * 4 + 16;
  static_assert(smem <= 160 * 1024, "ring does not fit the LDS");
  const int tiles = ((p.M + BM - 1) / BM) * ((p.N + BN - 1) / BN);
  auto kern = gemm_bf16_dma_kernel<EPI, OutT, BM, BN, WGM, WGN, NST, S3, BK>;
  if constexpr (BK != 64) V2A_REQUIRE(!p.a_koff, "v2a_gemm(dma): K-tile offset tables are laid out for 64-wide K tiles");
  if (to.chosen(p, V2A_GEMM_RING, S3, BM, BN, BK, WGM, WGN, NST, tiles)) return V2A_OK;
  static std::atomic<uint64_t> lds_set{0};
  if (int rc = v2a_enable_lds(reinterpret_cast<const void*>(kern), smem, lds_set, "v2a_gemm(dma)")) return rc;
  hipLaunchKernelGGL(kern, dim3(tiles), dim3(64 * WGM * WGN), smem, to.stream, p);
  return v2a_check_launch("v2a_gemm(dma)");
}

template <int BM, int BN, int WGM, int WGN, int NST = 3>
int dispatch_dma(const v2a_gemm_args* a, const GemmParams& p, GemmTarget to) {
  const bool out_f32 = a->out_dtype == V2A_F32;
  switch (a->epilogue) {
    case V2A_EPI_STORE:
      return out_f32 ? launch_dma<V2A_EPI_STORE, float, BM, BN, WGM, WGN, NST>(p, to) : launch_dma<V2A_EPI_STORE, bf16_t, BM, BN, WGM, WGN, NST>(p, to);
    case V2A_EPI_GEGLU:
      if constexpr ((BN / WGN / 16) % 2 == 0)
        return out_f32 ? launch_dma<V2A_EPI_GEGLU, float, BM, BN, WGM, WGN, NST>(p, to) : launch_dma<V2A_EPI_GEGLU, bf16_t, BM, BN, WGM, WGN, NST>(p, to);
      break;
    case V2A_EPI_RESID:
      if (out_f32) return launch_dma<V2A_EPI_RESID, float, BM, BN, WGM, WGN, NST>(p, to);
      break;
    case V2A_EPI_GATE_RESID:
      if (out_f32) return launch_dma<V2A_EPI_GATE_RESID, float, BM, BN, WGM, WGN, NST>(p, to);
      break;
  }
  return v2a_fail(V2A_ERR_ARG, "v2a_gemm(dma): unsupported epilogue %d / out_dtype %d", a->epilogue, a->out_dtype);
}

template <int BM, int BN, int WGM, int WGN, int NST, int BK = 64>
int dispatch_s3(const v2a_gemm_args* a, const GemmParams& p, GemmTarget to) {
  const bool out_f32 = a->out_dtype == V2A_F32;
  switch (a->epilogue) {
    case V2A_EPI_STORE:
      if (out_f32) return launch_dma<V2A_EPI_STORE, float, BM, BN, WGM, WGN, NST, true, BK>(p, to);
      break;
    case V2A_EPI_GEGLU:
      if constexpr ((BN / WGN / 16) % 2 == 0) {
        if (a->out_dtype == V2A_BF16_SPLIT) return launch_dma<V2A_EPI_GEGLU, bf16_t, BM, BN, WGM, WGN, NST, true, BK>(p, to);
      }
      break;
    case V2A_EPI_SWIGLU:
      if constexpr ((BN / WGN / 16) % 2 == 0) {
        if (out_f32) return launch_dma<V2A_EPI_SWIGLU, float, BM, BN, WGM, WGN, NST, true, BK>(p, to);
        if (a->out_dtype == V2A_BF16_SPLIT) return launch_dma<V2A_EPI_SWIGLU, bf16_t, BM, BN, WGM, WGN, NST, true, BK>(p, to);
      }
      break;
    case V2A_EPI_GELU:
      if (out_f32) return launch_dma<V2A_EPI_GELU, float, BM, BN, WGM, WGN, NST, true, BK>(p, to);
      if (a->out_dtype == V2A_BF16_SPLIT) return launch_dma<V2A_EPI_GELU, bf16_t, BM, BN, WGM, WGN, NST, true, BK>(p, to);
      break;
    case V2A_EPI_RESID:
      if (out_f32) return launch_dma<V2A_EPI_RESID, float, BM, BN, WGM, WGN, NST, true, BK>(p, to);
      break;
    case V2A_EPI_GATE_RESID:
      if (out_f32) return launch_dma<V2A_EPI_GATE_RESID, float, BM, BN, WGM, WGN, NST, true, BK>(p, to);
      break;
  }
  return v2a_fail(V2A_ERR_ARG, "v2a_gemm(split bf16): unsupported epilogue %d / out_dtype %d for this tile shape", a->epilogue, a->out_dtype);
}

#define V2A_RING_TILES(X)                                                                    \
  X(0, 128, 256, 2, 4, 3)                           \
  X(1, 128, 128, 2, 2, 3)                                               \
  X(2, 128, 64, 2, 2, 3)                               \
  X(3, 64, 64, 2, 2, 3)                                \
  X(5, 256, 256, 2, 4, 2)       \
  X(7, 64, 128, 2, 2, 6)    \
  X(8, 64, 64, 2, 2, 6)     \
  X(9, 64, 64, 2, 2, 4)                                                                      \
  X(10, 64, 64, 2, 2, 5)                                                                     \
  X(11, 128, 128, 2, 2, 4)                                                                   \
  X(12, 128, 128, 2, 4, 3)                      \
  X(13, 64, 64, 2, 4, 3)                            \
  X(14, 128, 64, 4, 2, 3)                                      \
  X(15, 64, 128, 2, 4, 3)
enum { kTile128x256 = 0, kTile128x128 = 1, kTile128x64 = 2, kTile64x64 = 3, kTile64x64Again = 4, kTile256x256 = 5, kTile8Phase = 6,
       kTileForceMax = 8, kTile64x64Waves8 = 13, kTileMax = 15 };
#define V2A_SPLIT_RING_TILES(X)                                                            \
  X(1, 64, 64, 2, 2, 3, 64)                                                    \
  X(2, 128, 64, 2, 2, 3, 64)                                                   \
  X(3, 128, 128, 2, 4, 2, 64)                                         \
  X(4, 64, 128, 2, 4, 3, 64)                                          \
  X(6, 128, 256, 2, 4, 3, 32)   \
  X(7, 128, 128, 2, 4, 3, 32)
enum { kSplit64x64 = 1, kSplit128x64 = 2, kSplit128x128 = 3, kSplit64x128 = 4, kSplit8Phase = 5, kSplit128x256K32 = 6, kSplitMax = 7, kSplitScatteredMax = 4 };

#define V2A_TILE_CASE(id, ...) case id:
constexpr bool is_ring_tile(int k) { switch (k) { V2A_RING_TILES(V2A_TILE_CASE) return true; } return false; }
#define V2A_LAUNCH_PLAIN(id, BM, BN, WGM, WGN, NST) case id: return dispatch_dma<BM, BN, WGM, WGN, NST>(a, p, to);
#define V2A_LAUNCH_SPLIT(id, BM, BN, WGM, WGN, NST, BK) case id: return dispatch_s3<BM, BN, WGM, WGN, NST, BK>(a, p, to);
int launch_ring_tile(bool split, int id, const v2a_gemm_args* a, const GemmParams& p, GemmTarget to) {
  if (split) switch (id) { V2A_SPLIT_RING_TILES(V2A_LAUNCH_SPLIT) }
  else switch (id == kTile64x64Again ? kTile64x64 : id) { V2A_RING_TILES(V2A_LAUNCH_PLAIN) }
  return v2a_fail(V2A_ERR_ARG, "v2a_gemm: no %s ring tile %d", split ? "split" : "plain", id);
}

constexpr int64_t ntiles(int M, int N, int bm, int bn) { return (int64_t)((M + bm - 1) / bm) * ((N + bn - 1) / bn); }
int fp32_tile_by_shape(int M, int N) { return ntiles(M, N, 128, 128) < 224 && M > 64 ? 64 : 128; }

int plain_tile_by_shape(int M, int N, bool dense, const v2a_detail::GemmTuning& tune) {
  const bool can8 = tune.use_8phase && dense;
  auto nt = [&](int bm, int bn) { return ntiles(M, N, bm, bn); };
  if (N <= 64) return nt(128, 64) >= 512 ? kTile128x64 : kTile64x64;
  if (N <= 128) return nt(128, 128) >= 512 ? kTile128x128 : (nt(128, 64) >= 512 ? kTile128x64 : kTile64x64);
  if (N >= 2048) {
    if (can8 && nt(256, 256) >= tune.min_tiles_8phase) return kTile8Phase;
    if (nt(256, 256) >= 512) return kTile256x256;
    return nt(128, 256) >= 96 ? kTile128x256 : kTile64x64;
  }
  if (N > 512) {
    if (can8 && nt(256, 256) >= 150) return kTile8Phase;
    if (nt(128, 256) >= 180) return kTile128x256;
    if (nt(128, 128) >= 180) return kTile128x128;
  } else {
    if (nt(128, 256) >= 150) return kTile128x256;
    if (nt(128, 128) >= 256) return kTile128x128;
  }
  return nt(64, 64) >= 2048 && nt(128, 64) >= 512 ? kTile128x64 : kTile64x64;
}

int split_tile_by_shape(int M, int N, bool glu, bool scattered, const v2a_detail::GemmTuning& tune) {
  auto nt = [&](int bm, int bn) { return ntiles(M, N, bm, bn); };
  if (scattered) {
    return N <= 64 ? kSplit128x64 : (nt(128, 128) >= 256 ? kSplit128x128 : kSplit64x128);
  }
  if (tune.use_8phase && N > 512 && nt(256, 256) >= 150) return kSplit8Phase;
  if (glu || N >= 2048) return nt(128, 128) >= 200 ? kSplit128x128 : kSplit64x128;
  if (N <= 512 && nt(128, 256) >= 128) return kSplit128x256K32;
  return nt(64, 128) >= 160 ? kSplit64x128 : kSplit64x64;
}

}

static constexpr v2a_detail::GemmTuning kDefaultTuning = {-1, 0, 1, 400, 1, 0};
v2a_detail::GemmTuning v2a_detail::g_gemm_tuning = kDefaultTuning;
// ... 76 lines not shown
  else if (p.out2_split)
    V2A_REQUIRE(p.out2_lo >= a->N && p.out2_lo % 4 == 0 && a->ld_out_bf16 >= p.out2_lo + (int64_t)a->N,
                "v2a_gemm: a split shadow needs out_bf16_lo_offset (%lld) >= N, a multiple of 4, and ld_out_bf16 >= lo offset + N", (long long)p.out2_lo);
  else
    V2A_REQUIRE(a->out_bf16_lo_offset == 0, "v2a_gemm: out_bf16_lo_offset goes with out_bf16_split");
  for (int sg = 0; sg < a->nseg; ++sg) {
    p.alo[sg] = a->a_lo_offset[sg] > 0 ? a->a_lo_offset[sg] : a->ka[sg];
    if (split_in && a->a_row_offset)
      V2A_REQUIRE(a->a_lo_offset[sg] > 0 && a->a_lo_offset[sg] % 8 == 0,
                  "v2a_gemm: split operands with offset tables need an explicit a_lo_offset (%lld) > 0, a multiple of 8",
                  (long long)a->a_lo_offset[sg]);
    else if (split_in)
      V2A_REQUIRE(p.alo[sg] >= a->ka[sg] && p.alo[sg] % 8 == 0 && a->lda[sg] >= p.alo[sg] + (int64_t)a->ka[sg],
                  "v2a_gemm: split segment %d: a_lo_offset (%lld) must be >= K, a multiple of 8, and lda >= lo offset + K", sg, (long long)p.alo[sg]);
    else
      V2A_REQUIRE(a->a_lo_offset[sg] == 0, "v2a_gemm: a_lo_offset goes with split operands");
  }
  p.out_split = a->out_dtype == V2A_BF16_SPLIT ? 1 : 0;
  if (p.out_split)
    V2A_REQUIRE((a->epilogue == V2A_EPI_GEGLU && a->ldo >= a->N) || (a->epilogue == V2A_EPI_SWIGLU && split_in && a->ldo >= a->N) ||
                    (a->epilogue == V2A_EPI_GELU && split_in && a->ldo >= 2 * (int64_t)a->N),
                "v2a_gemm: out_dtype V2A_BF16_SPLIT goes with the GEGLU epilogue and ldo >= N, SWIGLU on split operands and ldo >= N, or GELU on split "
                "operands and ldo >= 2N");
  if (a->epilogue == V2A_EPI_GELU)
    V2A_REQUIRE((a->compute_dtype == V2A_F32 || split_in) && !a->out_bf16 && !a->relu && !a->rope_table && !a->a_row_offset && !a->out_row_offset &&
                    !a->norm_gamma && !a->norm_ssq && !a->row_ssq,
                "v2a_gemm: the GELU epilogue needs fp32 compute or split operands, dense rows, and none of out_bf16 / relu / rope / norm folding");
  if (a->epilogue == V2A_EPI_SWIGLU)
    V2A_REQUIRE((a->compute_dtype == V2A_F32 || split_in) && !a->relu && !a->rope_table && !a->a_row_offset && !a->out_row_offset && !a->norm_gamma &&
                    !a->norm_ssq && !a->row_ssq && a->ldo >= a->N / 2,
                "v2a_gemm: the SWIGLU epilogue needs fp32 compute or split operands (plain bf16 compute has no SWIGLU instantiation), dense rows, "
                "ldo >= N / 2 and none of relu / rope / norm folding");
  p.resid = a->resid;
  p.ldr = a->ldr;
  p.gate = a->gate;
  p.step = a->step;
  p.gss = a->gate_step_stride;
  p.gbs = a->gate_batch_stride;
  p.rpb = a->rows_per_batch > 0 ? a->rows_per_batch : a->M;
  {
    auto al16 = [](const void* q) { return ((uintptr_t)q & 15) == 0; };
    const int osz = a->out_dtype == V2A_F32 ? 4 : 2;
    const int ncols = glu ? a->N / 2 : a->N;
    bool ok = a->N % 4 == 0 && ncols % 4 == 0 && ((uintptr_t)a->out % (4 * osz)) == 0 && (a->ldo * osz) % (4 * osz) == 0;
    if (a->bias) ok = ok && al16(a->bias);
    if (a->resid) ok = ok && al16(a->resid) && a->ldr % 4 == 0;
    if (a->gate) ok = ok && al16(a->gate) && a->gate_step_stride % 4 == 0 && a->gate_batch_stride % 4 == 0;
    if (a->out_bf16) ok = ok && ((uintptr_t)a->out_bf16 & 7) == 0 && a->ld_out_bf16 % 4 == 0;
    p.vec_epi = ok ? 1 : 0;
  }
  if (p.out2_split)
    V2A_REQUIRE(a->compute_dtype == V2A_BF16 && a->a_dtype != V2A_F32 && a->epilogue != V2A_EPI_SIGMOID && p.vec_epi,
                "v2a_gemm: out_bf16_split needs bf16 compute on bf16 or split A, an epilogue other than SIGMOID and 16-byte aligned epilogue "
                "operands (compute dtype %d, A dtype %d, epilogue %d): no other kernel writes the lo plane",
                a->compute_dtype, a->a_dtype, a->epilogue);
  p.relu = a->relu;
  const v2a_detail::GemmTuning tune = v2a_detail::g_gemm_tuning;
  p.krot = 0;
  p.dbg = tune.dbg;
  {
    const double ab = (double)a->M * K * (a->a_dtype == V2A_F32 ? 4 : 2), wb = (double)a->N * K * (a->compute_dtype == V2A_F32 ? 4 : 2);
    int best_gm = 1;
    double best = ab * 8 + wb;
    if (tune.xcd_grid) {
      for (int gm = 2; gm <= 8; gm *= 2) {
        const double c = ab * (8 / gm) + wb * gm;
        if (c < best * 0.95) { best = c; best_gm = gm; }
      }
    }
    p.xcd_gm = best_gm;
    p.xcd_gn = 8 / best_gm;
  }
  p.a_rowoff = a->a_row_offset;
  p.a_koff = a->a_ktile_offset;
  p.o_rowoff = a->out_row_offset;
  if (a->a_row_offset || a->a_ktile_offset || a->out_row_offset) {
    V2A_REQUIRE((a->a_row_offset != nullptr) == (a->a_ktile_offset != nullptr), "v2a_gemm: a_row_offset and a_ktile_offset go together");
    V2A_REQUIRE(a->nseg == 1 && a->compute_dtype == V2A_BF16 && (a->a_dtype == V2A_BF16 || split_in) && p.vec_epi &&
                    (a->epilogue == V2A_EPI_STORE || a->epilogue == V2A_EPI_RESID) && !a->rope_table,
                "v2a_gemm: row/K-tile offset tables need one bf16 (or split bf16) segment, bf16 compute, STORE/RESID and 16-byte aligned rows");
  }
  V2A_REQUIRE(!a->relu || !glu, "v2a_gemm: relu with GEGLU / SWIGLU");
  p.ngam = a->norm_gamma;
  p.ngss = a->norm_step_stride;
  p.ngbs = a->norm_batch_stride;
  p.nsw_row = a->norm_switch_row > 0 ? a->norm_switch_row : INT32_MAX;
  p.nsw_off = a->norm_switch_offset;
  p.ssq = a->norm_ssq;
  p.ssq_ld = a->ld_norm_ssq;
  if (a->norm_gamma || a->norm_ssq || a->row_ssq) {
    V2A_REQUIRE(a->compute_dtype == V2A_BF16 && (a->a_dtype == V2A_BF16 || split_in) && p.vec_epi && a->epilogue != V2A_EPI_SIGMOID && !a->out_row_offset,
                "v2a_gemm: a folded RMSNorm needs bf16 x bf16 (or split bf16) operands, dense rows and 16-byte aligned epilogue operands");
    if (a->norm_gamma || a->norm_ssq)
      V2A_REQUIRE(a->out_bf16 && (a->epilogue == V2A_EPI_RESID || a->epilogue == V2A_EPI_GATE_RESID) && a->N % 32 == 0 &&
                      (!a->norm_gamma || (((uintptr_t)a->norm_gamma & 15) == 0 && a->norm_step_stride % 4 == 0 && a->norm_batch_stride % 4 == 0 &&
                                          a->norm_switch_offset % 4 == 0)) &&
                      (!a->norm_ssq || a->ld_norm_ssq >= a->N / 32),
                  "v2a_gemm: norm_gamma / norm_ssq go with RESID / GATE_RESID, an out_bf16 shadow and N %% 32 == 0 (N=%d)", a->N);
  }
  if (int rc = v2a_detail::fill_row_scale(p, a->row_ssq, a->ld_row_ssq, a->row_ssq_parts, a->row_norm_dim, "v2a_gemm")) return rc;
  p.rope = a->rope_table;
  p.rope_cols = a->rope_cols;
  p.rope_pos_off = a->rope_pos_offset;
  if (a->rope_table) {
    V2A_REQUIRE(a->epilogue == V2A_EPI_STORE && a->compute_dtype == V2A_BF16 && (a->a_dtype == V2A_BF16 || split_in) && p.vec_epi &&
                    a->rope_cols % 64 == 0 && a->rope_cols <= a->N && ((uintptr_t)a->rope_table & 15) == 0,
                "v2a_gemm: fused RoPE needs the bf16 STORE epilogue with 16-byte aligned rows and rope_cols %% 64 == 0");
  }
  if (a->epilogue == V2A_EPI_RESID || a->epilogue == V2A_EPI_GATE_RESID)
    V2A_REQUIRE(a->resid != nullptr, "v2a_gemm: epilogue %d needs resid", a->epilogue);
  if (a->epilogue == V2A_EPI_GATE_RESID) V2A_REQUIRE(a->gate != nullptr, "v2a_gemm: GATE_RESID needs gate");
  if (glu) V2A_REQUIRE(a->N % 32 == 0, "v2a_gemm: GEGLU / SWIGLU need N %% 32 == 0 (N=%d)", a->N);
  return V2A_OK;
}

static int gemm_dispatch(const v2a_gemm_args* a, GemmTarget to) {
  GemmParams p;
  if (int rc = gemm_prepare(a, p)) return rc;
  const v2a_detail::GemmTuning tune = v2a_detail::g_gemm_tuning;
  const bool scattered = a->a_row_offset || a->out_row_offset;
  if (a->compute_dtype == V2A_F32)
    return fp32_tile_by_shape(a->M, a->N) == 64 ? dispatch_epi<float, false, 64, 64>(a, p, to) : dispatch_epi<float, false, 128, 128>(a, p, to);
  if (a->a_dtype == V2A_BF16_SPLIT) {
    V2A_REQUIRE(p.vec_epi, "v2a_gemm: split operands need 16-byte aligned epilogue operands");
    V2A_REQUIRE(a->tile_hint >= 0 && a->tile_hint <= kSplitMax, "v2a_gemm: tile_hint %d with split operands (0 = by shape, 1..7)", a->tile_hint);
    V2A_REQUIRE(!scattered || a->tile_hint <= kSplitScatteredMax,
                "v2a_gemm: tile_hint %d with split operands and offset tables (0 = by shape, 1..4: the 64-wide K stage ring shapes)", a->tile_hint);
    int id = a->tile_hint ? a->tile_hint : split_tile_by_shape(a->M, a->N, is_glu(a->epilogue), scattered, tune);
    if (id == kSplit8Phase && !tune.use_8phase) id = kSplit64x128;
    if (id != kSplit8Phase) return launch_ring_tile(true, id, a, p, to);
    p.s3_kl = p.K;
#ifdef V2A_GEMM_PROBE
    if (tune.dbg & 32) p.s3_kl = 0;
#endif
    return v2a_detail::launch_gemm_8phase(p, a->epilogue, a->out_dtype == V2A_BF16_SPLIT ? V2A_BF16 : a->out_dtype, to);
  }
  if (a->a_dtype == V2A_F32) return dispatch_epi<bf16_t, true, 128, 128>(a, p, to);
  if (a->epilogue == V2A_EPI_SIGMOID) return dispatch_epi<bf16_t, false, 128, 128>(a, p, to);
  V2A_REQUIRE(a->tile_hint >= 0 && a->tile_hint <= kTileMax + 1, "v2a_gemm: tile_hint %d", a->tile_hint);
  V2A_REQUIRE(a->tile_hint != kTile64x64Waves8 + 1 || !a->norm_ssq,
              "v2a_gemm: tile_hint 14 (64x64 tiles, wave tile 32x16) cannot write norm_ssq: the partial sums per 32 columns need wave tiles of "
              "at least 32 columns");
  const bool dense = !scattered && p.vec_epi;
  const bool hinted = a->tile_hint > 0 && tune.force_tile < 0;
  V2A_REQUIRE(!hinted || a->tile_hint - 1 != kTile8Phase || dense, "v2a_gemm: tile_hint 7 (256x256 8-phase) needs dense rows and 16-byte aligned epilogue operands");
  const bool forced = tune.force_tile >= 0 && (tune.force_tile != kTile8Phase || dense);
  const int k = hinted ? a->tile_hint - 1 : (forced ? tune.force_tile : plain_tile_by_shape(a->M, a->N, dense, tune));
  if (k == kTile8Phase) return v2a_detail::launch_gemm_8phase(p, a->epilogue, a->out_dtype, to);
  return launch_ring_tile(false, k, a, p, to);
}

extern "C" int v2a_gemm(const v2a_gemm_args* a, v2a_stream_t stream) { return gemm_dispatch(a, {(hipStream_t)stream, nullptr}); }

extern "C" int v2a_gemm_choose(const v2a_gemm_args* a, v2a_gemm_choice* choice) {
  V2A_REQUIRE(choice != nullptr, "v2a_gemm_choose: null choice");
  *choice = {};
  return gemm_dispatch(a, {nullptr, choice});
}
```

video-to-audio-and-piano-rp_amd/csrc/gemm_common.h:

```cpp
#pragma once
#include "v2a_common.h"
#include <stdlib.h>
#include <type_traits>

namespace v2a_detail {

struct GemmParams {
  const void* a[3];
  int64_t lda[3];
  int32_t kend[3];
  int32_t nseg;
  const void* w;
  int64_t ldw;
  const float* bias;
  int32_t M, N, K;
  void* out;
  int64_t ldo;
  bf16_t* out2;
  int64_t ldo2;
  const float* resid;
  int64_t ldr;
  const float* gate;
  const int32_t* step;
  int64_t gss, gbs;
  int32_t rpb;
  const float* rope;
  int32_t rope_cols, rope_pos_off;
  int32_t vec_epi;
  int32_t relu;
  const int32_t* a_rowoff;
  const int32_t* a_koff;
  const int32_t* o_rowoff;
  int32_t krot;
  const float* ngam;
  int64_t ngss, ngbs;
  int32_t nsw_row, nsw_off;
  float* ssq;
  int64_t ssq_ld;
  const float* rssq;
  int64_t rssq_ld;
  int32_t rssq_parts;
  float rnorm;
  int32_t xcd_gm, xcd_gn;
  struct Rect { int32_t m_lo, n_lo, cnt, hm; float rcp; } rect[8];
  int32_t nrect, tiles_m, tiles_n;
  int32_t out2_split, out_split;
  int64_t alo[3];
  int64_t out2_lo;
  int32_t s3_kl;
  int32_t dbg;
};

struct GemmTuning {
  int force_tile;
  int krot;
  int use_8phase;
  int min_tiles_8phase;
  int xcd_grid;
  int dbg;
};
extern GemmTuning g_gemm_tuning;
extern int g_attn_one_group_from;
extern int g_dwconv_rows_per_wave;
extern int g_probe_dbg;
extern int g_dwconv_stream;

struct GemmTarget {
  hipStream_t stream;
  v2a_gemm_choice* report;
  bool chosen(const GemmParams& p, int family, bool split, int bm, int bn, int bk, int waves_m, int waves_n, int stages, int tiles) const {
    if (report) *report = {family, split, bm, bn, bk, waves_m, waves_n, stages, tiles, p.xcd_gm, p.xcd_gn, p.vec_epi};
    return report != nullptr;
  }
};

int launch_gemm_8phase(const GemmParams& p, int epilogue, int out_dtype, GemmTarget to);

inline void fill_tile_map(GemmParams& p, int BM, int BN) {
  p.tiles_m = (p.M + BM - 1) / BM;
  p.tiles_n = (p.N + BN - 1) / BN;
  const int gm = p.xcd_gm, gn = p.xcd_gn;
  p.nrect = gm * gn;
  for (int r = 0; r < p.nrect; ++r) {
    const int xm = r / gn, xn = r % gn;
    const int m_lo = xm * p.tiles_m / gm, m_hi = (xm + 1) * p.tiles_m / gm;
    const int n_lo = xn * p.tiles_n / gn, n_hi = (xn + 1) * p.tiles_n / gn;
    const int hm = m_hi - m_lo;
    p.rect[r].m_lo = m_lo;
    p.rect[r].n_lo = n_lo;
    p.rect[r].cnt = hm * (n_hi - n_lo);
    p.rect[r].hm = hm > 0 ? hm : 1;
    p.rect[r].rcp = 1.0f / (float)(hm > 0 ? hm : 1);
  }
}

inline int fill_row_scale(GemmParams& p, const float* row_ssq, int64_t ld_row_ssq, int row_ssq_parts, int row_norm_dim, const char* who) {
  p.rssq = row_ssq;
  p.rssq_ld = ld_row_ssq;
  p.rssq_parts = row_ssq_parts;
  p.rnorm = sqrtf((float)row_norm_dim);
  if (row_ssq)
    V2A_REQUIRE(row_ssq_parts > 0 && row_ssq_parts <= 40 && row_norm_dim > 0 && ld_row_ssq >= (row_ssq_parts + 3) / 4 * 4 && ld_row_ssq % 4 == 0 &&
                    ((uintptr_t)row_ssq & 15) == 0,
                "%s: row_ssq needs row_ssq_parts <= 40 (%d), row_norm_dim (%d) and rows of whole float4 (zero padded)", who, row_ssq_parts, row_norm_dim);
  return V2A_OK;
}

}

namespace {

using v2a_detail::GemmParams;
using v2a_detail::GemmTarget;

__device__ __forceinline__ void tile_of_index(const GemmParams& p, int L, int& tm, int& tn) {
  tm = tn = 0;
#pragma unroll
  for (int r = 0; r < 8; ++r) {
    if (r < p.nrect) {
      const int cnt = p.rect[r].cnt;
      if (L >= 0 && L < cnt) {
        const int hm = p.rect[r].hm;
        int q = (int)((float)L * p.rect[r].rcp);
        int rem = L - q * hm;
        if (rem < 0) { --q; rem += hm; }
        else if (rem >= hm) { ++q; rem -= hm; }
        tn = p.rect[r].n_lo + q;
        tm = p.rect[r].m_lo + rem;
      }
      L -= cnt;
    }
  }
}
__device__ __forceinline__ int xcd_chunk_position(int bid, int nwg) {
  const int q = nwg >> 3, r = nwg & 7, xcd = bid & 7;
  return (xcd < r ? xcd * (q + 1) : r * (q + 1) + (xcd - r) * q) + (bid >> 3);
}
__device__ __forceinline__ void tile_of_block(const GemmParams& p, int bid, int& tm, int& tn) {
  tile_of_index(p, xcd_chunk_position(bid, p.tiles_m * p.tiles_n), tm, tn);
}

template <int J, int LPW>
__device__ __forceinline__ void ring_wait(int younger) {
  if constexpr (J == 0) {
    asm volatile("s_waitcnt vmcnt(0)" ::: "memory");
  } else {
    static_assert(J * LPW <= 63, "vmcnt is a 6-bit field");
    if (younger >= J) asm volatile("s_waitcnt vmcnt(%0)" ::"n"(J * LPW) : "memory");
    else ring_wait<J - 1, LPW>(younger);
  }
}

__host__ __device__ constexpr bool is_glu(int epi) { return epi == V2A_EPI_GEGLU || epi == V2A_EPI_SWIGLU; }
template <int EPI, bool FAST> __device__ __forceinline__ float glu_act(float g) {
  if constexpr (EPI == V2A_EPI_SWIGLU) return FAST ? silu_f(g) : silu_exact_f(g);
  else return FAST ? gelu_fast_f(g) : gelu_erf_f(g);
}

template <typename T> struct TileCfg;
template <> struct TileCfg<bf16_t> {
  static constexpr int BK = 64;
  static constexpr int LDS_ROW = 64;
};
template <> struct TileCfg<float> {
  static constexpr int BK = 16;
  static constexpr int LDS_ROW = 20;
};

template <int ROWS, bool SRC_F32> struct StageBf16 {
  static constexpr int N = ROWS / 32;
  bf16x8 r[N];
  __device__ __forceinline__ void load(const void* base, int64_t ld, int row0, int rows_total, int k0, int tid) {
    const int chunk = tid & 7;
#pragma unroll
    for (int i = 0; i < N; ++i) {
      int row = row0 + (tid >> 3) + 32 * i;
      row = row < rows_total ? row : rows_total - 1;
      if constexpr (SRC_F32) {
        const float* p = reinterpret_cast<const float*>(base) + (int64_t)row * ld + k0 + chunk * 8;
        f32x4 lo = *reinterpret_cast<const f32x4*>(p);
        f32x4 hi = *reinterpret_cast<const f32x4*>(p + 4);
        bf16x8 v;
#pragma unroll
        for (int j = 0; j < 4; ++j) {
          v[j] = (bf16_t)lo[j];
          v[4 + j] = (bf16_t)hi[j];
        }
        r[i] = v;
      } else {
        const bf16_t* p = reinterpret_cast<const bf16_t*>(base) + (int64_t)row * ld + k0 + chunk * 8;
        r[i] = *reinterpret_cast<const bf16x8*>(p);
      }
    }
  }
  __device__ __forceinline__ void store(bf16_t* lds, int tid) const {
    const int chunk = tid & 7;
#pragma unroll
    for (int i = 0; i < N; ++i) {
      int row = (tid >> 3) + 32 * i;
      *reinterpret_cast<bf16x8*>(lds + row * 64 + ((chunk ^ (row & 7)) << 3)) = r[i];
    }
  }
};
// ... 535 lines not shown
```

video-to-audio-and-piano-rp_amd/csrc/rowops.hip:

```cpp
#include "v2a_common.h"
#include <utility>

namespace v2a_detail { extern int g_dwconv_rows_per_wave; extern int g_dwconv_stream; }

thread_local char v2a_err_buf[512] = {0};

extern "C" int v2a_abi_version(void) { return 9; }
extern "C" const char* v2a_last_error(void) { return v2a_err_buf; }

namespace {

template <typename OutT, int VPL , bool SPLIT = false >
__global__ __launch_bounds__(256) void rmsnorm_kernel(const float* __restrict__ x, int64_t ldx, OutT* __restrict__ y,
                                                      int64_t ldy, int64_t rows, int d, const float* gamma,
                                                      const int32_t* step, int64_t gss, int64_t gbs, int rpb) {
  const int lane = threadIdx.x & 63;
  const int64_t row = (int64_t)blockIdx.x * 4 + (threadIdx.x >> 6);
  if (row >= rows) return;
  const float* xr = x + row * ldx;
  const float* g = step_vec(gamma, step, gss, gbs, row / rpb);
  const int nvec = d >> 2;
  f32x4 v[VPL];
  float ss = 0.f;
#pragma unroll
// ... 352 lines not shown
    }
  } else {
#pragma unroll
    for (int i = 0; i < 4; ++i) {
      a[i] = to_f32(base[quad * 4 + i]);
      b[i] = to_f32(base[32 + quad * 4 + i]);
    }
  }
#pragma unroll
  for (int i = 0; i < 4; ++i) {
    const float co = c[2 * i], si = c[2 * i + 1];
    const float ra = a[i] * co - b[i] * si;
    const float rb = b[i] * co + a[i] * si;
    a[i] = ra;
    b[i] = rb;
  }
  if (layout == 0) {
#pragma unroll
    for (int i = 0; i < 4; ++i) {
      base[quad * 8 + 2 * i] = from_f32<T>(a[i]);
      base[quad * 8 + 2 * i + 1] = from_f32<T>(b[i]);
    }
  } else {
#pragma unroll
    for (int i = 0; i < 4; ++i) {
      base[quad * 4 + i] = from_f32<T>(a[i]);
      base[32 + quad * 4 + i] = from_f32<T>(b[i]);
    }
  }
}

template <int ROWS>
__global__ __launch_bounds__(256) void linear_small_kernel(const float* __restrict__ a, int K, const float* __restrict__ wt,
                                                           const float* __restrict__ bias, const float* __restrict__ add,
                                                           int T, float* __restrict__ out, int64_t obs, int row_off, int d,
                                                           int dup, const float* __restrict__ regs, bf16_t* __restrict__ out2) {
  extern __shared__ __attribute__((aligned(16))) char smem_raw[];
  typedef float f32x2 __attribute__((ext_vector_type(2)));
  f32x2* as = reinterpret_cast<f32x2*>(smem_raw);
  const int b = blockIdx.y;
  const int fill = regs ? row_off : 0;
  const int rr0 = blockIdx.x * ROWS;
  for (int i = threadIdx.x; i < ROWS * K; i += blockDim.x) {
    const int t = rr0 + i / K - fill;
    const float v = (t >= 0 && t < T) ? a[((int64_t)b * T + t) * K + (i % K)] : 0.f;
    as[i] = f32x2{v, v};
  }
  __syncthreads();
  for (int n = threadIdx.x * 4; n < d; n += blockDim.x * 4) {
    f32x2 acc2[ROWS][2];
#pragma unroll
    for (int r = 0; r < ROWS; ++r) acc2[r][0] = acc2[r][1] = f32x2{0.f, 0.f};
#pragma unroll 8
    for (int k = 0; k < K; ++k) {
      const f32x4 w = *reinterpret_cast<const f32x4*>(wt + (int64_t)k * d + n);
      const f32x2 w0 = {w[0], w[1]}, w1 = {w[2], w[3]};
#pragma unroll
      for (int r = 0; r < ROWS; ++r) {
        const f32x2 aa = as[r * K + k];
        acc2[r][0] += aa * w0;
        acc2[r][1] += aa * w1;
      }
    }
    f32x4 acc[ROWS];
#pragma unroll
    for (int r = 0; r < ROWS; ++r) acc[r] = f32x4{acc2[r][0][0], acc2[r][0][1], acc2[r][1][0], acc2[r][1][1]};
    f32x4 bv = {0.f, 0.f, 0.f, 0.f};
    if (bias) bv = *reinterpret_cast<const f32x4*>(bias + n);
#pragma unroll
    for (int r = 0; r < ROWS; ++r) {
      const int rr = rr0 + r;
      if (rr >= fill + T) break;
      f32x4 v;
      int orow;
      if (rr < fill) {
        v = *reinterpret_cast<const f32x4*>(regs + (int64_t)rr * d + n);
        orow = rr;
      } else {
        const int t = rr - fill;
        v = acc[r];
#pragma unroll
        for (int e = 0; e < 4; ++e) v[e] += bv[e];
        if (add) {
          const f32x4 ad = *reinterpret_cast<const f32x4*>(add + (int64_t)t * d + n);
#pragma unroll
          for (int e = 0; e < 4; ++e) v[e] += ad[e];
        }
        orow = row_off + t;
      }
      bf16x4 o2;
#pragma unroll
      for (int e = 0; e < 4; ++e) o2[e] = (bf16_t)v[e];
      for (int h = 0; h < (dup > 0 ? 2 : 1); ++h) {
        const int64_t off = (int64_t)(b + h * dup) * obs + (int64_t)orow * d + n;
        *reinterpret_cast<f32x4*>(out + off) = v;
        if (out2) *reinterpret_cast<bf16x4*>(out2 + off) = o2;
      }
    }
  }
}

__global__ void fill_registers_kernel(float* __restrict__ out, int64_t obs, const float* __restrict__ regs, int B, int R,
                                      int d) {
  const int64_t idx = (int64_t)blockIdx.x * blockDim.x + threadIdx.x;
  const int64_t per = (int64_t)R * d;
  if (idx >= per * B) return;
  const int64_t b = idx / per, r = idx % per;
  out[b * obs + r] = regs[r];
}

__global__ __launch_bounds__(256) void time_cond_kernel(const float* __restrict__ t, const float* __restrict__ fw,
                                                        const float* __restrict__ wt, const float* __restrict__ bias,
                                                        float* __restrict__ out, int d) {
  extern __shared__ __attribute__((aligned(16))) char smem_raw[];
  float* e = reinterpret_cast<float*>(smem_raw);
  const int s = blockIdx.x;
  const float ts = t[s];
  const int half = d / 2;
  if (threadIdx.x == 0) e[0] = ts;
  for (int i = threadIdx.x; i < half; i += blockDim.x) {
    const float f = ts * fw[i] * 2.0f * 3.14159265358979323846f;
    e[1 + i] = sinf(f);
    e[1 + half + i] = cosf(f);
  }
  __syncthreads();
  const int n = blockIdx.y * blockDim.x + threadIdx.x;
  if (n >= d) return;
  float acc = bias[n];
#pragma unroll 8
  for (int k = 0; k < d + 1; ++k) acc += e[k] * wt[(int64_t)k * d + n];
  out[(int64_t)s * d + n] = silu_f(acc);
}

__device__ __forceinline__ f32x4 cfg_euler_update(float* __restrict__ y, const float* __restrict__ pred, int B, int C, int64_t pbs,
                                                  int row_off, float s, const float* __restrict__ dt, const int32_t* step,
                                                  const double* apg, float keep, int64_t e, int64_t b, int64_t r) {
  const float h = dt[step ? step[0] : 0];
  const f32x4 pc = *reinterpret_cast<const f32x4*>(pred + b * pbs + (int64_t)row_off * C + r);
  const f32x4 pn = *reinterpret_cast<const f32x4*>(pred + (b + B) * pbs + (int64_t)row_off * C + r);
  f32x4 yv = *reinterpret_cast<const f32x4*>(y + e);
  float coef = 0.f;
  if (apg) {
    const double dot = apg[2 * b], nn = apg[2 * b + 1];
    const double nrm = sqrt(nn) > 1e-12 ? sqrt(nn) : 1e-12;
    coef = (float)(dot / (nrm * nrm));
  }
#pragma unroll
  for (int j = 0; j < 4; ++j) {
    float upd = pc[j] - pn[j];
    if (apg) {
      const float par = coef * pc[j];
      upd = (upd - par) + par * keep;
    }
    yv[j] += h * (pc[j] + upd * s);
  }
  *reinterpret_cast<f32x4*>(y + e) = yv;
  return yv;
}

__global__ __launch_bounds__(256) void cfg_euler_kernel(float* __restrict__ y, const float* __restrict__ pred, int B,
                                                        int T, int C, int64_t pbs, int row_off, float s,
                                                        const float* __restrict__ dt, const int32_t* step,
                                                        const double* apg, float keep) {
  const int64_t idx4 = (int64_t)blockIdx.x * blockDim.x + threadIdx.x;
  const int64_t per_b = (int64_t)T * C;
  const int64_t total4 = (int64_t)B * per_b / 4;
  if (idx4 >= total4) return;
  const int64_t e = idx4 * 4;
  cfg_euler_update(y, pred, B, C, pbs, row_off, s, dt, step, apg, keep, e, e / per_b, e % per_b);
}

__global__ __launch_bounds__(256) void cfg_euler_planes_kernel(float* __restrict__ y, const float* __restrict__ pred, int B,
                                                               int T, int C, int64_t pbs, int row_off, float s,
                                                               const float* __restrict__ dt, const int32_t* step,
                                                               const double* apg, float keep, bf16_t* __restrict__ planes,
                                                               int64_t ldp, int64_t lo_off, int plane_row_off, int rows_per_seq, int copies) {
  const int64_t idx4 = (int64_t)blockIdx.x * blockDim.x + threadIdx.x;
  const int64_t per_b = (int64_t)T * C;
  const int64_t total4 = (int64_t)B * per_b / 4;
  if (idx4 >= total4) return;
  const int64_t e = idx4 * 4;
  const int64_t b = e / per_b, r = e % per_b;
  float sv = s;
  asm volatile("" : "+v"(sv));
  const f32x4 yv = cfg_euler_update(y, pred, B, C, pbs, row_off, sv, dt, step, apg, keep, e, b, r);
  bf16x4 hi, lo;
#pragma unroll
  for (int j = 0; j < 4; ++j) {
    hi[j] = (bf16_t)yv[j];
    lo[j] = (bf16_t)(yv[j] - (float)hi[j]);
  }
  const int64_t t = r / C, c = r % C;
  for (int k = 0; k < copies; ++k) {
    bf16_t* row = planes + (((int64_t)k * B + b) * rows_per_seq + plane_row_off + t) * ldp + c;
    *reinterpret_cast<bf16x4*>(row) = hi;
    *reinterpret_cast<bf16x4*>(row + lo_off) = lo;
  }
}

__global__ __launch_bounds__(256) void apg_reduce_kernel(const float* __restrict__ pred, double* __restrict__ apg, int B,
                                                         int T, int C, int64_t pbs, int row_off, const int32_t* __restrict__ valid_rows) {
  const int b = blockIdx.y;
  int rows = T;
  if (valid_rows) rows = min(T, max(0, valid_rows[0]));
  const int64_t per_b = (int64_t)rows * C;
  double dot = 0.0, nn = 0.0;
  const float* pc = pred + (int64_t)b * pbs + (int64_t)row_off * C;
  const float* pn = pred + (int64_t)(b + B) * pbs + (int64_t)row_off * C;
  for (int64_t i = (int64_t)blockIdx.x * blockDim.x + threadIdx.x; i < per_b; i += (int64_t)gridDim.x * blockDim.x) {
    const double c = pc[i], n = pn[i];
    dot += (c - n) * c;
    nn += c * c;
  }
  __shared__ double sd[256], sn[256];
  sd[threadIdx.x] = dot;
  sn[threadIdx.x] = nn;
  __syncthreads();
  for (int o = 128; o > 0; o >>= 1) {
    if (threadIdx.x < o) {
      sd[threadIdx.x] += sd[threadIdx.x + o];
      sn[threadIdx.x] += sn[threadIdx.x + o];
    }
    __syncthreads();
  }
  if (threadIdx.x == 0) {
    atomicAdd(&apg[2 * b], sd[0]);
    atomicAdd(&apg[2 * b + 1], sn[0]);
  }
}

__global__ void step_advance_kernel(int32_t* step) { step[0] += 1; }

__global__ __launch_bounds__(256) void split_bf16_kernel(const float* __restrict__ x, int64_t ldx, bf16_t* __restrict__ y, int64_t ldy,
                                                         int64_t rows, int d) {
  const int64_t i = (int64_t)blockIdx.x * blockDim.x + threadIdx.x;
  const int per = d >> 2;
  if (i >= rows * per) return;
  const int64_t r = i / per;
  const int c = (int)(i % per) * 4;
  const f32x4 v = *reinterpret_cast<const f32x4*>(x + r * ldx + c);
  bf16x4 hi, lo;
#pragma unroll
  for (int j = 0; j < 4; ++j) {
    hi[j] = (bf16_t)v[j];
    lo[j] = (bf16_t)(v[j] - (float)hi[j]);
  }
  *reinterpret_cast<bf16x4*>(y + r * ldy + c) = hi;
  *reinterpret_cast<bf16x4*>(y + r * ldy + d + c) = lo;
}

__global__ __launch_bounds__(256) void cast_bf16_kernel(const float* __restrict__ x, bf16_t* __restrict__ y, int64_t n4) {
  const int64_t i = (int64_t)blockIdx.x * blockDim.x + threadIdx.x;
  if (i >= n4) return;
  const f32x4 v = *reinterpret_cast<const f32x4*>(x + 4 * i);
  bf16x4 o;
#pragma unroll
  for (int j = 0; j < 4; ++j) o[j] = (bf16_t)v[j];
  *reinterpret_cast<bf16x4*>(y + 4 * i) = o;
}

}

extern "C" int v2a_rmsnorm(const float* x, int64_t ldx, void* y, int64_t ldy, int32_t y_dtype, int64_t rows, int32_t d,
                           const float* gamma, const int32_t* step, int64_t gss, int64_t gbs, int32_t rpb,
                           v2a_stream_t stream) {
  V2A_REQUIRE(x && y && gamma, "v2a_rmsnorm: null pointer");
  V2A_REQUIRE(rows > 0 && d > 0 && d % 4 == 0 && d <= 2048, "v2a_rmsnorm: d=%d (need d %% 4 == 0, d <= 2048)", d);
  V2A_REQUIRE(ldx % 4 == 0 && ldy % 4 == 0 && gss % 4 == 0 && gbs % 4 == 0, "v2a_rmsnorm: strides must be multiples of 4");
  V2A_REQUIRE(y_dtype == V2A_F32 || y_dtype == V2A_BF16 || y_dtype == V2A_BF16_SPLIT, "v2a_rmsnorm: y dtype %d", y_dtype);
  V2A_REQUIRE(y_dtype != V2A_BF16_SPLIT || ldy >= 2 * (int64_t)d, "v2a_rmsnorm: split output needs ldy >= 2*d");
  if (rpb <= 0) rpb = (int32_t)rows;
  hipStream_t s = (hipStream_t)stream;
  const dim3 grid((unsigned)((rows + 3) / 4)), block(256);
  const int vpl = (d / 4 + 63) / 64;
#define V2A_RMS(OT, V) \
  hipLaunchKernelGGL((rmsnorm_kernel<OT, V>), grid, block, 0, s, x, ldx, (OT*)y, ldy, rows, d, gamma, step, gss, gbs, rpb)
  if (y_dtype == V2A_BF16_SPLIT) {
#define V2A_RMS_S(V) hipLaunchKernelGGL((rmsnorm_kernel<bf16_t, V, true>), grid, block, 0, s, x, ldx, (bf16_t*)y, ldy, rows, d, gamma, step, gss, gbs, rpb)
    if (vpl <= 1) V2A_RMS_S(1); else if (vpl <= 2) V2A_RMS_S(2); else if (vpl <= 3) V2A_RMS_S(3); else if (vpl <= 4) V2A_RMS_S(4);
    else if (vpl <= 5) V2A_RMS_S(5); else if (vpl <= 6) V2A_RMS_S(6); else V2A_RMS_S(8);
#undef V2A_RMS_S
  } else if (y_dtype == V2A_F32) {
    if (vpl <= 1) V2A_RMS(float, 1); else if (vpl <= 2) V2A_RMS(float, 2); else if (vpl <= 3) V2A_RMS(float, 3); else if (vpl <= 4) V2A_RMS(float, 4);
    else if (vpl <= 5) V2A_RMS(float, 5); else if (vpl <= 6) V2A_RMS(float, 6); else V2A_RMS(float, 8);
  } else {
    if (vpl <= 1) V2A_RMS(bf16_t, 1); else if (vpl <= 2) V2A_RMS(bf16_t, 2); else if (vpl <= 3) V2A_RMS(bf16_t, 3); else if (vpl <= 4) V2A_RMS(bf16_t, 4);
    else if (vpl <= 5) V2A_RMS(bf16_t, 5); else if (vpl <= 6) V2A_RMS(bf16_t, 6); else V2A_RMS(bf16_t, 8);
  }
#undef V2A_RMS
  return v2a_check_launch("v2a_rmsnorm");
}

static int dwconv_launch(const float* x, float* out, const float* wt, const float* bias, int32_t B, int32_t N, int32_t d, int32_t ksize,
                         const int32_t* len, const v2a_dwconv_norm* norm, v2a_stream_t stream) {
  V2A_REQUIRE(x && out && wt && bias, "v2a_dwconv: null pointer");
  V2A_REQUIRE(x != out, "v2a_dwconv: out must not alias x (halo reads)");
  V2A_REQUIRE(ksize == 31, "v2a_dwconv: kernel_size %d (only 31 is built, x3:726)", ksize);
  V2A_REQUIRE(d % 4 == 0 && B > 0 && N > 0, "v2a_dwconv: B=%d N=%d d=%d", B, N, d);
  if (norm)
    V2A_REQUIRE(norm->out_bf16 && norm->norm_gamma && norm->norm_ssq && d % 32 == 0 && norm->ld_out_bf16 % 4 == 0 && norm->ld_out_bf16 >= d &&
                    ((uintptr_t)norm->out_bf16 & 7) == 0 && ((uintptr_t)norm->norm_gamma & 15) == 0 && norm->norm_step_stride % 4 == 0 &&
                    norm->norm_batch_stride % 4 == 0 && norm->ld_norm_ssq >= d / 32 && (!norm->split || norm->ld_out_bf16 >= 2 * (int64_t)d),
                "v2a_dwconv: the folded norm needs out_bf16, norm_gamma, norm_ssq, d %% 32 == 0 (d=%d) and aligned rows", d);
  const int cb = (d / 4 + 63) / 64;
  hipStream_t s = (hipStream_t)stream;
  {
    int nseg = (256 + B * cb - 1) / (B * cb);
// ... 200 lines not shown
```

video-to-audio-and-piano-rp_amd/csrc/v2a_common.h:

```cpp
#pragma once
#include <hip/hip_runtime.h>
#include <stdint.h>
#include <stdio.h>
#include <stdarg.h>
#include <atomic>

#include "../../include/v2a_cfm.h"

typedef __bf16 bf16_t;
typedef __bf16 bf16x8 __attribute__((ext_vector_type(8)));
typedef __bf16 bf16x4 __attribute__((ext_vector_type(4)));
typedef __bf16 bf16x2 __attribute__((ext_vector_type(2)));
typedef float f32x4 __attribute__((ext_vector_type(4)));
typedef float f32x2 __attribute__((ext_vector_type(2)));
typedef float f32x16 __attribute__((ext_vector_type(16)));

#define V2A_WAVE 64

extern thread_local char v2a_err_buf[512];
static inline int v2a_fail(int code, const char* fmt, ...) {
  va_list ap;
  va_start(ap, fmt);
  vsnprintf(v2a_err_buf, sizeof(v2a_err_buf), fmt, ap);
  va_end(ap);
  return code;
}
#define V2A_REQUIRE(cond, ...) \
  do {                         \
    if (!(cond)) return v2a_fail(V2A_ERR_ARG, __VA_ARGS__); \
  } while (0)
static inline int v2a_check_launch(const char* what) {
  hipError_t e = hipGetLastError();
  if (e != hipSuccess) return v2a_fail(V2A_ERR_LAUNCH, "%s: %s", what, hipGetErrorString(e));
  return V2A_OK;
}

static inline int v2a_enable_lds(const void* kern, size_t bytes, std::atomic<uint64_t>& done, const char* what) {
  int dev = 0;
  if (hipGetDevice(&dev) != hipSuccess) dev = 0;
  const uint64_t bit = 1ull << (dev & 63);
  if (done.load(std::memory_order_acquire) & bit) return V2A_OK;
  const hipError_t e = hipFuncSetAttribute(kern, hipFuncAttributeMaxDynamicSharedMemorySize, (int)bytes);
  if (e != hipSuccess) return v2a_fail(V2A_ERR_LAUNCH, "%s: hipFuncSetAttribute(%zu bytes of LDS) on device %d: %s", what, bytes, dev, hipGetErrorString(e));
  done.fetch_or(bit, std::memory_order_release);
  return V2A_OK;
}

__device__ __forceinline__ float wave_sum(float v) {
#pragma unroll
  for (int o = 32; o > 0; o >>= 1) v += __shfl_xor(v, o, 64);
  return v;
}
__device__ __forceinline__ float wave_max(float v) {
#pragma unroll
  for (int o = 32; o > 0; o >>= 1) v = fmaxf(v, __shfl_xor(v, o, 64));
  return v;
}
__device__ __forceinline__ float sigmoid_f(float x) { return 1.0f / (1.0f + __expf(-x)); }
__device__ __forceinline__ float silu_f(float x) { return x / (1.0f + __expf(-x)); }
__device__ __forceinline__ float silu_exact_f(float x) { return x / (1.0f + expf(-x)); }
__device__ __forceinline__ float gelu_erf_f(float x) { return 0.5f * x * (1.0f + erff(x * 0.70710678118654752f)); }
__device__ __forceinline__ float gelu_fast_f(float x) {
  const float z = fabsf(x) * 0.70710678118654752f;
  const float t = __builtin_amdgcn_rcpf(1.0f + 0.3275911f * z);
  const float poly = t * (0.254829592f + t * (-0.284496736f + t * (1.421413741f + t * (-1.453152027f + t * 1.061405429f))));
  const float erfz = 1.0f - poly * __expf(-z * z);
  return 0.5f * x * (1.0f + copysignf(erfz, x));
}

__device__ __forceinline__ float octet_sum(float v) {
  v += __builtin_bit_cast(float, __builtin_amdgcn_update_dpp(0, __builtin_bit_cast(int, v), 0xB1, 0xF, 0xF, true));
  v += __builtin_bit_cast(float, __builtin_amdgcn_update_dpp(0, __builtin_bit_cast(int, v), 0x4E, 0xF, 0xF, true));
  v += __builtin_bit_cast(float, __builtin_amdgcn_update_dpp(0, __builtin_bit_cast(int, v), 0x141, 0xF, 0xF, true));
  return v;
}

__device__ __forceinline__ const float* step_vec(const float* base, const int32_t* step, int64_t step_stride,
                                                 int64_t batch_stride, int64_t batch) {
  int64_t s = step ? (int64_t)step[0] : 0;
  return base + s * step_stride + batch * batch_stride;
}

template <typename T> struct dtype_of;
template <> struct dtype_of<float> { static constexpr int value = V2A_F32; };
template <> struct dtype_of<bf16_t> { static constexpr int value = V2A_BF16; };

__device__ __forceinline__ float to_f32(float v) { return v; }
__device__ __forceinline__ float to_f32(bf16_t v) { return (float)v; }
template <typename T> __device__ __forceinline__ T from_f32(float v);
template <> __device__ __forceinline__ float from_f32<float>(float v) { return v; }
template <> __device__ __forceinline__ bf16_t from_f32<bf16_t>(float v) { return (bf16_t)v; }
```

video-to-audio-and-piano-rp_amd/dit.py:

```python
from __future__ import annotations

import math
import os
from collections import OrderedDict
from dataclasses import dataclass, asdict
from typing import NamedTuple

import torch

from . import _lib as L

NOTES = 51


@dataclass
class DiTConfig:
    dim: int = 1024
    dim_text: int = 1280
    dim_frames: int = 512
    depth: int = 12
    heads: int = 16
    dim_head: int = 64
    frames_heads: int = 8
    ff_mult: int = 4
# ... 73 lines not shown
        w[:n] = torch.cat([p.float() for p in parts], 0)
        b = torch.zeros(self.n_pad, dtype=torch.float32)
        self.gate_col = n - heads
        b[self.gate_col:n] = bg.float()
        self.w_in = pack_weight(w, dev, cd, split)
        self.b_in = b.to(dev)
        self.w_out = pack_weight(sd[f"{prefix}.to_out.weight"], dev, cd, split)
        self.wk, self.wv = (wk, wv) if cross else (None, None)
        self.wq32, self.wo32 = (torch.cat([wq.float(), wg.float()], 0), sd[f"{prefix}.to_out.weight"].float()) if cross and split else (None, None)


class _FF:

    def __init__(self, sd, prefix, dim, cd, dev, split=False):
        w1, b1 = sd[f"{prefix}.ff.0.proj.weight"].float(), sd[f"{prefix}.ff.0.proj.bias"].float()
        inner = w1.shape[0] // 2
        assert inner % 16 == 0
        self.inner = inner
        wv, wg = w1[:inner].reshape(inner // 16, 1, 16, dim), w1[inner:].reshape(inner // 16, 1, 16, dim)
        self.w1 = pack_weight(torch.cat([wv, wg], 1).reshape(2 * inner, dim), dev, cd, split)
        bv, bgt = b1[:inner].reshape(inner // 16, 1, 16), b1[inner:].reshape(inner // 16, 1, 16)
        self.b1 = torch.cat([bv, bgt], 1).reshape(2 * inner).to(dev).contiguous()
        self.w2 = pack_weight(sd[f"{prefix}.ff.2.weight"], dev, cd, split)
        self.b2 = sd[f"{prefix}.ff.2.bias"].float().to(dev).contiguous()


class _Conv:
    def __init__(self, sd, prefix, dev):
        w = sd[f"{prefix}.dw_conv1d.0.weight"].float()
        self.k = w.shape[-1]
        self.wt = w[:, 0, :].t().contiguous().to(dev)
        self.b = sd[f"{prefix}.dw_conv1d.0.bias"].float().to(dev).contiguous()


class PackedWeights:

    def __init__(self, cfg: DiTConfig, sd: dict, dev, cd: torch.dtype, split: bool = False):
        c = cfg
        pk = lambda w: pack_weight(w, dev, cd, split)
        T = "transformer"
        f32 = lambda k: sd[k].float().to(dev).contiguous()
        self.pos_emb = f32(f"{T}.abs_pos_emb.weight")
        self.regs = f32(f"{T}.registers")
        self.text_regs = f32(f"{T}.text_registers")
        self.frames_regs = f32(f"{T}.frames_registers")
        self.fourier_w = f32(f"{T}.time_cond_mlp.0.weights")
        self.time_wt = sd[f"{T}.time_cond_mlp.1.weight"].float().t().contiguous().to(dev)
        self.time_b = f32(f"{T}.time_cond_mlp.1.bias")
        self.final_g = f32(f"{T}.final_norm.g")
        self.pin_wt = sd["proj_in.weight"].float().t().contiguous().to(dev)
        self.pin_b = f32("proj_in.bias")
        self.pf_wt = sd["proj_frames.weight"].float().t().contiguous().to(dev)
        self.pf_b = f32("proj_frames.bias")
        self.pred_w = pk(sd["to_pred.weight"])
        self.pred_b = f32("to_pred.bias")
        if c.cond_proj_in:
            wc = sd["cond_proj_in.weight"].float()
            self.cond_k = _ru(c.num_channels, 64)
            wp = torch.zeros(wc.shape[0], self.cond_k)
            wp[:, :c.num_channels] = wc
            self.cond_w = pk(wp)
            self.cond_b = (sd["cond_proj_in.bias"].float() if "cond_proj_in.bias" in sd else torch.zeros(wc.shape[0])).to(dev).contiguous()
        self.layers = []
        ng, gw, gb, kw, vw = [], [], [], [], []
        for i in range(c.depth):
            P = f"{T}.layers.{i}"
            ly = {}
            if i >= c.depth // 2:
                ly["skip"] = pk(sd[f"{P}.0.0.weight"])
                if cd == torch.bfloat16:
                    ws = sd[f"{P}.0.0.weight"].double()
                    w1 = sd[f"{P}.1.5.text_frames_to_audio.weight"].double()
                    wsx, wss = ws[:, :c.dim], ws[:, c.dim:]
                    fused = torch.cat([wsx @ w1[:, :c.dim] + wsx, wss, wsx @ w1[:, c.dim:c.dim + c.dim_text], wsx @ w1[:, c.dim + c.dim_text:]], 1)
                    ly["x_skip"] = pk(fused.float())
            ly["a_conv"] = _Conv(sd, f"{P}.0.1", dev)
            ly["a_attn"] = _Attn(sd, f"{P}.0.3", c.dim, c.heads, c.dim_head, cd, dev, split=split)
            ly["a_attn2"] = _Attn(sd, f"{P}.0.6", c.dim, c.heads, c.dim_head, cd, dev, cross=True, split=split)
            ly["a_ff"] = _FF(sd, f"{P}.0.9", c.dim, cd, dev, split)
            ng += [sd[f"{P}.0.2.to_gamma.weight"], sd[f"{P}.0.5.to_gamma.weight"], sd[f"{P}.0.8.to_gamma.weight"]]
            gw += [sd[f"{P}.0.4.to_gamma.weight"], sd[f"{P}.0.7.to_gamma.weight"], sd[f"{P}.0.10.to_gamma.weight"]]
            gb += [sd[f"{P}.0.4.to_gamma.bias"], sd[f"{P}.0.7.to_gamma.bias"], sd[f"{P}.0.10.to_gamma.bias"]]
            kw.append(ly["a_attn2"].wk)
            vw.append(ly["a_attn2"].wv)
            ly["t_conv"] = _Conv(sd, f"{P}.1.0", dev)
            ly["t_g1"] = f32(f"{P}.1.1.g")
            ly["t_attn"] = _Attn(sd, f"{P}.1.2", c.dim_text, c.heads, c.dim_head, cd, dev, split=split)
            ly["t_g2"] = f32(f"{P}.1.3.g")
            ly["t_ff"] = _FF(sd, f"{P}.1.4", c.dim_text, cd, dev, split)
            ly["x_tfa"] = pk(sd[f"{P}.1.5.text_frames_to_audio.weight"])
            if i != c.depth - 1:
                ly["x_at"] = pk(sd[f"{P}.1.5.audio_to_text.weight"])
                ly["x_af"] = pk(sd[f"{P}.1.5.audio_to_frames.weight"])
            ly["f_conv"] = _Conv(sd, f"{P}.2.0", dev)
            ly["f_g1"] = f32(f"{P}.2.1.g")
            ly["f_attn"] = _Attn(sd, f"{P}.2.2", c.dim_frames, c.frames_heads, c.dim_head, cd, dev, split=split)
            ly["f_g2"] = f32(f"{P}.2.3.g")
            ly["f_ff"] = _FF(sd, f"{P}.2.4", c.dim_frames, cd, dev, split)
            self.layers.append(ly)
        self.norm_gamma_w = torch.cat([w.float() for w in ng], 0).to(dev).contiguous()
        self.norm_gamma_b = torch.ones(self.norm_gamma_w.shape[0], device=dev)
        self.gate_w = torch.cat([w.float() for w in gw], 0).to(dev).contiguous()
        self.gate_b = torch.cat([b.float() for b in gb], 0).to(dev).contiguous()
        self.ctx_kv_w = pk(torch.cat([w.float() for w in kw] + [w.float() for w in vw], 0))
        self.xattn_wq = self.xattn_wo = None
        if split:
            self.xattn_wq = torch.stack([ly["a_attn2"].wq32 for ly in self.layers]).to(dev).contiguous()
            self.xattn_wo = torch.stack([ly["a_attn2"].wo32 for ly in self.layers]).to(dev).contiguous()
        for ly in self.layers:
            ly["a_attn2"].wk = ly["a_attn2"].wv = ly["a_attn2"].wq32 = ly["a_attn2"].wo32 = None
        self.fold_g = None
        if split and c.num_channels % 64 == 0 and c.depth >= 2:
            self.fold_g = tuple(pk(g.float()) for g in fold_embed_weights(sd, c.dim))


SHIPPED_WIDTHS = (1024, 1280, 512, 4)
_R2, _R3 = "profiles/r02 A/B runs (DESIGN.md appendix A, `scripts/gpu_ci.sh sidetiles`)", "profiles/r03_tile_sweep.txt"
_R5 = "profiles/r05_bf16x3_tile_sweeps.txt"
_W8, _NARROW, _PH8 = L.TILE_128x128_8WAVES, L.TILE_128x64_8WAVES, L.TILE_8PHASE
_S_PH8, _S_FAT = L.SPLIT_TILE_8PHASE, L.SPLIT_TILE_128x256_K32
TUNED_TILES = {
    ("bf16", 0, SHIPPED_WIDTHS): {
        ("t", "cross"): (_W8, _R3), ("t", "out"): (_W8, _R3), ("t", "ff2"): (_W8, _R3), ("t", "ff1"): (_PH8, _R2),
        ("f", "cross"): (_W8, _R3), ("f", "out"): (_W8, _R3), ("f", "ff2"): (_W8, _R3), ("f", "ff1"): (_PH8, _R2), ("f", "qkv"): (_PH8, _R2),
        ("a", "x_tfa"): (_NARROW, _R3), ("a", "skip"): (_NARROW, _R3), ("a", "out"): (_NARROW, _R3), ("a", "out2"): (_NARROW, _R3),
        ("a", "ff2"): (_NARROW, _R3), ("a", "qkv"): (L.TILE_128x128, _R2), ("a", "ff1"): (_PH8, _R2),
    },
    ("bf16", 1, SHIPPED_WIDTHS): {},
    ("bf16", 2, SHIPPED_WIDTHS): {},
    ("bf16x3", 0, SHIPPED_WIDTHS): {("a", "qkv"): (_S_PH8, "profiles/r04_bf16x3_qkv_8phase_ab.txt"), ("t", "qkv"): (_S_PH8, "profiles/r04_bf16x3_qkv_8phase_ab.txt"),
                                    ("f", "qkv"): (_S_PH8, _R5), ("f", "ff1"): (_S_PH8, _R5), ("f", "cross"): (_S_FAT, _R5), ("f", "out"): (_S_FAT, _R5),
                                    ("f", "ff2"): (_S_FAT, _R5)},
    ("bf16x3", 2, SHIPPED_WIDTHS): {},
}


def tuned_tiles(mode: str, regime: int, widths) -> dict:
    return {k: v[0] for k, v in TUNED_TILES.get((mode, regime, tuple(widths)), {}).items()}


_STREAMS: dict = {}


def process_streams(dev):
    dev = torch.device(dev)
    key = (dev.type, dev.index if dev.index is not None else torch.cuda.current_device())
    s = _STREAMS.get(key)
    if s is None:
        s = _STREAMS[key] = tuple(torch.cuda.Stream(device=dev) for _ in range(3))
        assert len({x.cuda_stream for x in s}) == 3
    return s


class DiTEngine:

    def __init__(self, cfg: DiTConfig, state_dict: dict, device="cuda", compute: str = "bf16",
                 rope_layout: str = "interleaved", rope_cross: bool = False,
                 zero_masked_queries: bool = True, softclamp: float = 50.0, multi_stream: bool = True):
        assert compute in ("bf16", "fp32", "bf16x3")
        self.split = compute == "bf16x3"
        self.multi_stream = multi_stream
        self.side_tile = 0 if multi_stream else -1
        self.fuse_skip = True
        widths = (cfg.dim, cfg.dim_text, cfg.dim_frames, cfg.ff_mult)
        one_clip = tuned_tiles("bf16", 0, widths)
        self.side_tiles = {k: v for k, v in one_clip.items() if not (k[0] == "a" and v == _NARROW)}
        self.main_tile = _NARROW if any(k[0] == "a" and v == _NARROW for k, v in one_clip.items()) else -1
        self.big_tiles = tuned_tiles("bf16", 2, widths)
        self.split_tiles = tuned_tiles("bf16x3", 0, widths)
        self.split_big_tiles = tuned_tiles("bf16x3", 2, widths)
        self.fold_norm = True
        self.fold_gemm_all = False
        self.fuse_xattn = True
        self.absorb_xattn = os.environ.get("V2A_ABSORB_XATTN", "1") != "0"
        self.fold_embed = os.environ.get("V2A_FOLD_EMBED", "1") != "0"
        self.cross_on_main = False
        self.interleave_capture = False
        self._fuse_rope = compute != "fp32" and rope_layout == "interleaved"
        assert cfg.dim_head == 64, "kernels are built for dim_head = 64 (x3:717)"
        self.cfg = cfg
        self.dev = torch.device(device)
        self.cd = torch.float32 if compute == "fp32" else torch.bfloat16
        self.cdc = L.F32 if compute == "fp32" else L.BF16
        self.ad = torch.bfloat16 if compute == "bf16" else torch.float32
        self.adc = {"bf16": L.BF16, "fp32": L.F32, "bf16x3": L.BF16_SPLIT}[compute]
        self.rope_layout = {"interleaved": 0, "half": 1}[rope_layout]
        self.rope_cross = rope_cross
        self.zero_masked_queries = zero_masked_queries
        self.softclamp = float(softclamp)
        L.lib()
        self.W = PackedWeights(cfg, state_dict, self.dev, self.cd, self.split)
        self.plans: OrderedDict = OrderedDict()
        self.max_plans = 4
        self.plan = None

    def setup(self, B: int, T: int, nc: int, S: int, cfg_mode: bool = True):
        key = (B, T, nc, S, cfg_mode)
        p = self.plans.get(key)
        if p is not None:
            self.plans.move_to_end(key)
            self.plan = p
            self._alloc_absorbed(p)
            self._alloc_folded(p)
            return p
        c, dev, cd = self.cfg, self.dev, self.cd
        R = c.num_registers
        N = T + R
        if T > c.max_seq_len:
            raise ValueError(f"{T} latent frames exceed max_seq_len = {c.max_seq_len} of the position table")
        Bt = 2 * B if cfg_mode else B
        rows = Bt * N
        e = lambda *s, dt=torch.float32: torch.empty(*s, dtype=dt, device=dev)
        p = dict(key=key, B=B, Bt=Bt, T=T, N=N, nc=nc, S=S, rows=rows, cfg_mode=cfg_mode, graphs={})
        D, Dt, Df = c.dim, c.dim_text, c.dim_frames
        w2 = 2 if self.split else 1
        bf = cd == torch.bfloat16

        def stream(d):
            return _Stream(e(Bt, N, d), L.Operand(e(Bt, N, w2 * d, dt=cd), w2 * d, d) if bf else None)

        ld, lo = w2 * 2 * D, 2 * D if self.split else 0
        wide = [e(Bt, N, ld, dt=cd) for _ in range(c.depth // 2)] if bf else []
        p["wide"] = [_Wide(L.Operand(w, ld, 2 * D, lo), L.Operand(w[..., :D], ld, D, lo), L.Operand(w[..., D:2 * D], ld, D, lo)) for w in wide]
        p["skips"] = [_Stream(e(Bt, N, D), p["wide"][j].skip if bf else None) for j in range(c.depth // 2)]
        p["xA"], p["xB"], p["xS"] = stream(D), stream(D), e(Bt, N, D)
        p["tA"], p["tB"], p["t0"], p["tL0"] = stream(Dt), stream(Dt), e(Bt, N, Dt), stream(Dt)
        p["fA"], p["fB"], p["f0"], p["fL0"] = stream(Df), stream(Df), e(Bt, N, Df), stream(Df)
        W0 = self.W.layers[0]
        for s, d, attn, ff in (("a", D, W0["a_attn"], W0["a_ff"]), ("t", Dt, W0["t_attn"], W0["t_ff"]),
                               ("f", Df, W0["f_attn"], W0["f_ff"])):
            p[f"hn_{s}"] = e(rows, w2 * d, dt=cd)
            p[f"ssq_{s}"] = torch.zeros(rows, (d // 32 + 3) // 4 * 4, device=dev)
            p[f"qkv_{s}"] = e(rows, attn.n_pad, dt=self.ad)
            p[f"ao_{s}"] = e(rows, w2 * attn.inner, dt=cd)
            p[f"ffh_{s}"] = e(rows, w2 * ff.inner, dt=cd)
        p["q2"] = e(B * N, W0["a_attn2"].n_pad, dt=self.ad)
        inner = c.heads * c.dim_head
        p["ctx_kv"] = e(B * nc, 2 * c.depth * inner, dt=self.ad)
        p["xattn_kp"] = 0
        self._alloc_absorbed(p)
        p["armed"], p["c0_ok"], p["grid_host"] = False, False, None
        self._alloc_folded(p)
        p["ctx"] = e(B * nc, w2 * c.ctx_dim, dt=cd)
        p["ctx_len"] = torch.full((B,), nc, dtype=torch.int32, device=dev)
        p["pred"] = e(Bt, N, c.num_channels)
        p["tc"] = e(S, D)
        p["norm_tab"] = e(S, c.depth, 3, D)
        p["gate_tab"] = e(S, c.depth, 3, D)
        p["t_pts"] = e(S)
        p["dt"] = e(S)
        p["step"] = torch.zeros(1, dtype=torch.int32, device=dev)
        p["apg"] = torch.zeros(2 * B, dtype=torch.float64, device=dev)
        p["valid_T"] = torch.full((1,), T, dtype=torch.int32, device=dev)
        p["seq_len"] = torch.full((Bt,), N, dtype=torch.int32, device=dev)
        p["ragged"] = False
        inv = 1.0 / (10000 ** (torch.arange(0, c.dim_head, 2).float() / c.dim_head))
        ang = torch.arange(N + nc).float()[:, None] * inv[None, :]
        p["rope"] = torch.stack((ang.cos(), ang.sin()), -1).contiguous().to(dev)
        p["per_sample_t"] = False
        p["has_cond"] = False
        if c.cond_proj_in:
            p["condbuf"] = torch.zeros(B * N, w2 * self.W.cond_k, dtype=cd, device=dev)
            p["padd"] = e(T, D)
        if self.dev.type == "cuda" and self.multi_stream:
            p["st"], p["sf"], _ = process_streams(self.dev)
        self.plan = p
        self.plans[key] = p
        while len(self.plans) > max(1, self.max_plans):
            self.plans.popitem(last=False)
        return p

    def launch_signature(self):
        p = self.plan
        return (p["ragged"], p["has_cond"], p["per_sample_t"], self.multi_stream, self.side_tile, tuple(sorted(self.side_tiles.items())),
                tuple(sorted(self.big_tiles.items())), tuple(sorted(self.split_tiles.items())), tuple(sorted(self.split_big_tiles.items())), self.main_tile, self.fold_norm, self.fold_gemm_all, self.fuse_skip, self.fuse_xattn, self.cross_on_main,
                self.interleave_capture, self.rope_cross, self.zero_masked_queries, self.absorb_xattn, p["xattn_kp"], self.fold_embed, p["armed"])

    def _rows(self, t):
        return L.Operand(t, t.stride(-2), t.shape[-1] // (2 if self.split else 1))

    def _mm(self, segs, W, out, shadow=None, **kw):
        if shadow is not None:
            kw.update(out_bf16=shadow.t, ld_out_bf16=shadow.ld)
            if self.split:
                kw.update(out_bf16_split=True, out_bf16_lo_offset=shadow.lo)
        if self.split:
            return L.gemm(segs, W, out, compute=L.BF16, a_split=True, **kw)
        return L.gemm(segs, W, out, compute=self.cdc, **kw)

    def _norm_plain(self, x, hn, rows, d, g):
        L.rmsnorm(x, hn, rows=rows, d=d, gamma=g, split=self.split)

    def _norm_ada(self, x, hn, rows, d, layer, slot):
        p = self.plan
        tab = p["norm_tab"][0, layer, slot]
        ss = p["norm_tab"].stride(0)
        if p["per_sample_t"]:
            L.rmsnorm(x, hn, rows=rows, d=d, gamma=tab, gamma_batch_stride=ss, rows_per_batch=p["N"], split=self.split)
        else:
            L.rmsnorm(x, hn, rows=rows, d=d, gamma=tab, step=p["step"], gamma_step_stride=ss, rows_per_batch=p["N"], split=self.split)

    def _fuse_skip(self):
        return self.fuse_skip and self.cd == torch.bfloat16 and "x_skip" in self.W.layers[-1]

    def _fold(self):
        c = self.cfg
        return (self.fold_norm and self.cd == torch.bfloat16
                and all(d % 32 == 0 and d <= 1280 for d in (c.dim, c.dim_text, c.dim_frames)))

    def _regime(self):
        c = self.cfg
        tiles = -(-self.plan["rows"] // 128) * max(1, c.dim // 128)
        return 0 if tiles <= 140 else (1 if tiles <= 281 else 2)

    def _tuned_dims(self):
        c = self.cfg
        return ("bf16", 0, (c.dim, c.dim_text, c.dim_frames, c.ff_mult)) in TUNED_TILES

    def _fold_gemm(self):
        return self._fold() and (self._regime() < 2 or self.fold_gemm_all)

    def _nprod_ada(self, layer, slot, switch_row=0):
        p, D = self.plan, self.cfg.dim
        ss = p["norm_tab"].stride(0)
        kw = dict(norm_gamma=p["norm_tab"][0, layer, slot], norm_ssq=p["ssq_a"], shadow=self._rows(p["hn_a"]))
        kw["norm_batch_stride" if p["per_sample_t"] else "norm_step_stride"] = ss
        if switch_row:
            kw.update(norm_switch_row=switch_row, norm_switch_offset=D)
        return kw

    def _ncons(self, s, d):
        return dict(row_ssq=self.plan[f"ssq_{s}"], row_norm_dim=d) if self._fold() else {}

    def _gate_kw(self, layer, slot):
        p = self.plan
        tab = p["gate_tab"][0, layer, slot]
        ss = p["gate_tab"].stride(0)
        if p["per_sample_t"]:
            return dict(gate=tab, gate_batch_stride=ss, rows_per_batch=p["N"])
        return dict(gate=tab, step=p["step"], gate_step_stride=ss, rows_per_batch=p["N"])

    def _self_attn(self, A: _Attn, x, s, nseq, d, out_kw, in_kw={}):
        p = self.plan
        N, rows = p["N"], nseq * p["N"]
        hn, qkv, ao = p[f"hn_{s}"], p[f"qkv_{s}"], p[f"ao_{s}"]
        if self._fuse_rope:
            self._mm([self._rows(hn)], A.w_in, qkv, M=rows, N=A.n_pad, bias=A.b_in, ldo=A.n_pad,
                     rope_table=p["rope"], rope_cols=2 * A.inner, rope_pos_offset=0, rows_per_batch=N, **in_kw)
        else:
            self._mm([self._rows(hn)], A.w_in, qkv, M=rows, N=A.n_pad, bias=A.b_in, ldo=A.n_pad, **in_kw)
            L.rope(qkv, rows=rows, row_stride=A.n_pad, nheads=2 * A.heads, rows_per_batch=N, pos_offset=0,
                   table=p["rope"], layout=self.rope_layout)
        es = qkv.element_size()
        base = qkv.data_ptr()
        lens = p["seq_len"] if p["ragged"] else None
        aw = ao.stride(-2)
        L.attention(base, base + A.inner * es, base + 2 * A.inner * es, base + A.gate_col * es, ao.data_ptr(),
                    strides=(A.n_pad, A.n_pad, A.n_pad, A.n_pad, aw,
                             N * A.n_pad, N * A.n_pad, N * A.n_pad, N * A.n_pad, N * aw),
                    B=nseq, H=A.heads, Nq=N, Nk=N, kv_len=lens,
                    q_len=lens if self.zero_masked_queries else None,
                    scale=self.cfg.dim_head ** -0.5, softclamp=self.softclamp, dtype=self.adc, out_split=self.split)
        self._mm([self._rows(ao)], A.w_out, x, M=rows, N=d, resid=x, ldo=d, ldr=d, **out_kw)

    def _ff(self, Fw: _FF, x, s, nseq, d, out_kw, in_kw={}):
        p = self.plan
        rows = nseq * p["N"]
        hn, ffh = p[f"hn_{s}"], p[f"ffh_{s}"]
        self._mm([self._rows(hn)], Fw.w1, ffh, M=rows, N=2 * Fw.inner, epilogue=L.EPI_GEGLU, bias=Fw.b1, ldo=ffh.stride(-2),
                 **(dict(out_split=True) if self.split else {}), **in_kw)
        self._mm([self._rows(ffh)], Fw.w2, x, M=rows, N=d, bias=Fw.b2, resid=x, ldo=d, ldr=d, **out_kw)

    def _tile_hint(self, stream, op):
        r = self._regime()
        if self.split:
            return (self.split_big_tiles if r == 2 else self.split_tiles).get((stream, op), 0)
        side = stream != "a"
        if side and self.side_tile < 0:
            return 0
        if r == 2:
            return self.big_tiles.get((stream, op), -1) + 1
        if r == 1 or not self._tuned_dims():
            return self.side_tile + 1 if side else 0
        narrow = self.main_tile if op in ("x_tfa", "skip", "out", "out2", "ff2") else -1
        return max(self.side_tiles.get((stream, op), self.side_tile if side else narrow), -1) + 1

    def _side_block(self, ly, s, src, dst, nseq, d, parts=(0, 1, 2)):
        p = self.plan
        N, rows = p["N"], nseq * p["N"]
        lens = p["seq_len"] if p["ragged"] else None
        cv = ly[f"{s}_conv"]
        hq, ho, h1, h2 = (self._tile_hint(s, op) for op in ("qkv", "out", "ff1", "ff2"))
        fold, fold2 = self._fold(), self._fold_gemm()
        hn, ssq = p[f"hn_{s}"], p[f"ssq_{s}"]
        nc = self._ncons(s, d)
        cons = dict(tile_hint=hq, **nc)
        cons2 = dict(tile_hint=h1, **(nc if fold2 else {}))
        x = dst.x
        if 0 in parts:
            if fold:
                L.dwconv(src, x, cv.wt, cv.b, B=nseq, N=N, d=d, ksize=cv.k, lens=lens,
                         norm=dict(out_bf16=hn, ld_out_bf16=hn.stride(-2), gamma=ly[f"{s}_g1"], ssq=ssq, split=self.split))
            else:
                L.dwconv(src, x, cv.wt, cv.b, B=nseq, N=N, d=d, ksize=cv.k, lens=lens)
                self._norm_plain(x, hn, rows, d, ly[f"{s}_g1"])
        if 1 in parts:
            prod = dict(shadow=self._rows(hn), norm_gamma=ly[f"{s}_g2"], norm_ssq=ssq) if fold2 else {}
            self._self_attn(ly[f"{s}_attn"], x, s, nseq, d, dict(epilogue=L.EPI_RESID, tile_hint=ho, **prod), cons)
        if 2 in parts:
            if not fold2:
                self._norm_plain(x, hn, rows, d, ly[f"{s}_g2"])
            self._ff(ly[f"{s}_ff"], x, s, nseq, d, dict(epilogue=L.EPI_RESID, tile_hint=h2, shadow=dst.sh), cons2)

    def _absorb(self, B, N, nc):
        c = self.cfg
        A2 = self.W.layers[0]["a_attn2"]
        return (self.absorb_xattn and self.split and not self.rope_cross and 0 < nc <= 32 and (c.heads * L.xattn_kp(nc)) % 64 == 0
                and c.dim % 512 == 0 and c.dim <= 2048 and A2.gate_col == A2.inner and B * -(-N // 64) * A2.heads <= 704)

    def _alloc_absorbed(self, p):
        c = self.cfg
        if p["xattn_kp"] or not self._absorb(p["B"], p["N"], p["nc"]):
            return
        kp = p["xattn_kp"] = L.xattn_kp(p["nc"])
        e = lambda *s: torch.empty(*s, dtype=self.cd, device=self.dev)
        p["wqk"] = e(p["B"], c.depth, c.heads * kp + c.heads, 2 * c.dim)
        p["wvo"] = e(p["B"], c.depth, c.dim, 2 * c.heads * kp)
        p["xp"] = e(p["B"] * p["N"], 2 * c.heads * kp)

    def _fold_ok(self, p):
        return self.fold_embed and self.split and self.W.fold_g is not None and p["cfg_mode"] and not p.get("per_sample_t", False)

    def _alloc_folded(self, p):
        c = self.cfg
        if "ybuf" in p or not self._fold_ok(p):
            return
        z = lambda *s, dt=torch.float32: torch.zeros(*s, dtype=dt, device=self.dev)
        C_ = c.num_channels
        p["ybuf"] = L.Operand(z(p["rows"], 2 * C_, dt=self.cd), 2 * C_, C_)
        p["y_zero"] = z(p["B"], p["T"], C_)
        for s, d in (("a", c.dim), ("t", c.dim_text), ("f", c.dim_frames)):
            p[f"c0_{s}"] = torch.empty(p["Bt"], p["N"], d, dtype=torch.float32, device=self.dev)

    def _audio_cross_attention_absorbed(self, i, ly, x, nctx, cons2, fold2, lens):
        p, c = self.plan, self.cfg
        N, D, H, kp = p["N"], c.dim, c.heads, p["xattn_kp"]
        A2 = ly["a_attn2"]
        r2 = nctx * N
        if not fold2:
            self._norm_ada(x, p["hn_a"], r2, D, i, 1)
        nk = dict(row_ssq=cons2["row_ssq"], row_norm_dim=cons2["row_norm_dim"]) if cons2 else {}
        wqk, wvo, xp = p["wqk"], p["wvo"], p["xp"]
        L.xattn_absorbed(p["hn_a"], p["hn_a"].stride(-2), D, wqk[0, i], xp, ldw=wqk.stride(-2), w_batch_stride=wqk.stride(0), ldo=xp.stride(-2),
                         M=r2, rows_per_batch=N, B=nctx, H=H, KP=kp, kv_len=p["ctx_len"], q_len=lens if self.zero_masked_queries else None,
                         gate_bias=A2.b_in[A2.gate_col:], scale=c.dim_head ** -0.5, softclamp=self.softclamp, **nk)
        xr, hn = x.reshape(-1, D), p["hn_a"]
        for b in range(nctx):
            rows = slice(b * N, (b + 1) * N)
            kw = dict(self._gate_kw(i, 1))
            if fold2:
                kw.update(self._nprod_ada(i, 2))
                kw.update(norm_ssq=p["ssq_a"][rows], shadow=self._rows(hn[rows]))
            if p["per_sample_t"]:
                kw["gate"] = p["gate_tab"][b, i, 1]
                if fold2:
                    kw["norm_gamma"] = p["norm_tab"][b, i, 2]
            self._mm([self._rows(xp[rows])], wvo[b, i], xr[rows], M=N, N=D, resid=xr[rows], ldo=D, ldr=D, epilogue=L.EPI_GATE_RESID,
                     tile_hint=self._tile_hint("a", "out2"), **kw)

    def _audio_cross_attention(self, i, ly, x, nctx, cons2, fold2, lens):
        p, c, W = self.plan, self.cfg, self.W
        N, D = p["N"], c.dim
        if p["xattn_kp"] and self.absorb_xattn:
            return self._audio_cross_attention_absorbed(i, ly, x, nctx, cons2, fold2, lens)
        inner = c.heads * c.dim_head
        nkv = 2 * c.depth * inner
        r2 = nctx * N
        A2 = ly["a_attn2"]
        if not fold2:
            self._norm_ada(x, p["hn_a"], r2, D, i, 1)
        q2 = p["q2"]
        es = q2.element_size()
        kb = p["ctx_kv"].data_ptr() + i * inner * es
        vb = p["ctx_kv"].data_ptr() + (c.depth + i) * inner * es
        aw = p["ao_a"].stride(-2)
        one_launch = (self.fuse_xattn and self.adc in (L.BF16, L.BF16_SPLIT) and nctx * -(-N // 64) * A2.heads <= 704 and p["nc"] <= 64 and D % 512 == 0
                      and A2.gate_col == A2.inner and (self._fuse_rope or not self.rope_cross))
        if one_launch:
            rk = dict(rope_table=p["rope"], rope_cols=A2.inner, rope_pos_offset=0) if self.rope_cross else {}
            nk = dict(row_ssq=cons2["row_ssq"], row_norm_dim=cons2["row_norm_dim"]) if cons2 else {}
            L.qproj_xattn(p["hn_a"], p["hn_a"].stride(-2), D, A2.w_in, bias=A2.b_in, M=r2, N=A2.n_pad, rows_per_batch=N,
                          k=kb, v=vb, out=p["ao_a"].data_ptr(), split=self.split,
                          kv_strides=(nkv, nkv, p["nc"] * nkv, p["nc"] * nkv), out_strides=(aw, N * aw), B=nctx, H=A2.heads, Nk=p["nc"],
                          kv_len=p["ctx_len"], q_len=lens if self.zero_masked_queries else None, scale=c.dim_head ** -0.5,
                          softclamp=self.softclamp, **rk, **nk)
        elif self.rope_cross and self._fuse_rope:
            self._mm([self._rows(p["hn_a"])], A2.w_in, q2, M=r2, N=A2.n_pad, bias=A2.b_in, ldo=A2.n_pad, rope_table=p["rope"],
                     rope_cols=A2.inner, rope_pos_offset=0, rows_per_batch=N, tile_hint=self._tile_hint("a", "q2"), **cons2)
        else:
            self._mm([self._rows(p["hn_a"])], A2.w_in, q2, M=r2, N=A2.n_pad, bias=A2.b_in, ldo=A2.n_pad,
                     tile_hint=self._tile_hint("a", "q2"), **cons2)
            if self.rope_cross:
                L.rope(q2, rows=r2, row_stride=A2.n_pad, nheads=A2.heads, rows_per_batch=N, pos_offset=0,
                       table=p["rope"], layout=self.rope_layout)
        if not one_launch:
            L.attention(q2.data_ptr(), kb, vb, q2.data_ptr() + A2.gate_col * es, p["ao_a"].data_ptr(),
                        strides=(A2.n_pad, nkv, nkv, A2.n_pad, aw,
                                 N * A2.n_pad, p["nc"] * nkv, p["nc"] * nkv, N * A2.n_pad, N * aw),
                        B=nctx, H=A2.heads, Nq=N, Nk=p["nc"], kv_len=p["ctx_len"],
                        q_len=lens if self.zero_masked_queries else None,
                        scale=c.dim_head ** -0.5, softclamp=self.softclamp, dtype=self.adc, out_split=self.split)
        self._mm([self._rows(p["ao_a"])], A2.w_out, x, M=r2, N=D, resid=x, ldo=D, ldr=D, epilogue=L.EPI_GATE_RESID,
                 tile_hint=self._tile_hint("a", "out2"), **self._gate_kw(i, 1), **(self._nprod_ada(i, 2) if fold2 else {}))

    def prepare(self, text, frames_roll, context, context_mask, t_points, *, lens=None,
                drop_text=None, drop_ctx=None, dt=None, step_cond=None, rope_len=None, rope_ctx_len=None, fold_embed=False):
        p, c, W, dev = self.plan, self.cfg, self.W, self.dev
        B, Bt, T, N, nc, S = p["B"], p["Bt"], p["T"], p["N"], p["nc"], p["S"]
        R, D, Dt, Df = c.num_registers, c.dim, c.dim_text, c.dim_frames
        assert text.shape == (B, T, Dt) and frames_roll.shape == (B, T, c.notes) and context.shape == (B, nc, c.ctx_dim)
        p["valid_T"].fill_(T if rope_len is None else min(T, int(rope_len) - R))
        p["armed"] = p["c0_ok"] = False
        folding = fold_embed and "ybuf" in p and self._fold_ok(p)
        p["step"].zero_()
        if not (folding and same_grid(p["grid_host"], t_points, dt)):
            p["t_pts"].copy_(t_points.to(dev, torch.float32))
            if dt is not None:
                p["dt"].copy_(dt.to(dev, torch.float32))
            L.time_cond(p["t_pts"], W.fourier_w, W.time_wt, W.time_b, p["tc"], S=S, d=D)
            nt = c.depth * 3 * D
            L.gemm([(p["tc"], D, D)], W.norm_gamma_w, p["norm_tab"], M=S, N=nt, compute=L.F32, bias=W.norm_gamma_b, ldo=nt)
            L.gemm([(p["tc"], D, D)], W.gate_w, p["gate_tab"], M=S, N=nt, compute=L.F32, epilogue=L.EPI_SIGMOID,
                   bias=W.gate_b, ldo=nt)
        p["grid_host"] = None
        if folding and t_points.device.type == "cpu" and (dt is None or dt.device.type == "cpu"):
            p["grid_host"] = (t_points.detach().to(torch.float32).clone(), None if dt is None else dt.detach().to(torch.float32).clone())
        if lens is not None and not bool((torch.as_tensor(lens) == T).all()):
            sl = (torch.as_tensor(lens).to(torch.int32) + R).to(dev)
            p["seq_len"].copy_(sl.repeat(Bt // B))
            p["ragged"] = True
        else:
            p["seq_len"].fill_(N)
            p["ragged"] = False
        if drop_text is None:
            drop_text = [False] * B + [True] * (Bt - B)
        if drop_ctx is None:
            drop_ctx = [False] * B
        L.fill_registers(p["t0"], W.text_regs, B=Bt, R=R, d=Dt, out_batch_stride=N * Dt)
        L.fill_registers(p["f0"], W.frames_regs, B=Bt, R=R, d=Df, out_batch_stride=N * Df)
        tx = text.to(dev, torch.float32)
        for s in range(Bt):
            if drop_text[s]:
                p["t0"][s, R:].zero_()
            else:
                p["t0"][s, R:].copy_(tx[s % B])
        fr = frames_roll.to(dev, torch.float32).contiguous()
        L.linear_small(fr, W.pf_wt, W.pf_b, None, p["f0"], M=B * T, K=c.notes, T=T, out_batch_stride=N * Df,
                       row_off=R, d=Df, dup=(B if Bt > B else 0))
        p["has_cond"] = step_cond is not None
        if step_cond is not None:
            assert c.cond_proj_in, "step_cond needs cond_proj_in weights (E2TTS(if_cond_proj_in=True))"
            assert step_cond.shape == (B, T, c.num_channels)
            cb = torch.zeros(B, N, W.cond_k, device=dev)
            cb[:, R:, :c.num_channels] = step_cond.to(dev, torch.float32)
            cb = cb.reshape(B * N, W.cond_k)
            if self.split:
                L.split_bf16(cb, p["condbuf"], rows=B * N, d=W.cond_k)
            else:
                p["condbuf"].copy_(cb)
            p["padd"].copy_(W.pos_emb[:T] + W.cond_b)
        cx = context.to(dev, torch.float32).clone()
        for b in range(B):
            if drop_ctx[b]:
                cx[b] = 0
        if self.split:
            L.split_bf16(cx.reshape(B * nc, -1).contiguous(), p["ctx"], rows=B * nc, d=c.ctx_dim)
        else:
            p["ctx"].copy_(cx.reshape(B * nc, -1))
        cm = context_mask.to(torch.bool).cpu()
        cl = cm.sum(-1).to(torch.int32)
        assert bool((cm == (torch.arange(nc)[None] < cl[:, None])).all()), "context_mask must be a prefix mask"
        p["ctx_len"].copy_(cl)
        inner = c.heads * c.dim_head
        nkv = 2 * c.depth * inner
        self._mm([self._rows(p["ctx"])], W.ctx_kv_w, p["ctx_kv"], M=B * nc, N=nkv, ldo=nkv)
        if self.rope_cross:
            off = (N if rope_len is None else int(rope_len)) - (nc if rope_ctx_len is None else int(rope_ctx_len))
            assert 0 <= off and off + nc <= p["rope"].shape[0], (off, nc, N)
            L.rope(p["ctx_kv"], rows=B * nc, row_stride=nkv, nheads=c.depth * c.heads, rows_per_batch=nc,
                   pos_offset=off, table=p["rope"], layout=self.rope_layout)
        if p["xattn_kp"] and self.absorb_xattn:
            L.xattn_absorb_prepare(p["ctx_kv"], W.xattn_wq, W.xattn_wo, p["wqk"], p["wvo"], B=B, L=c.depth, H=c.heads, D=D, nc=nc,
                                   KP=p["xattn_kp"], k_col=0, v_col=c.depth * inner)
        ly = W.layers[0]
        self._side_block(ly, "t", p["t0"], p["tL0"], Bt, Dt)
        self._side_block(ly, "f", p["f0"], p["fL0"], Bt, Df)
        if folding:
            self.embed(p["y_zero"])
            xa, tl, fl = p["xA"], p["tL0"], p["fL0"]
            rows = p["rows"]
            ht, hf = self._cross_hints()
            self._mm([xa.op, tl.op, fl.op], ly["x_tfa"], p["c0_a"], M=rows, N=D, epilogue=L.EPI_RESID, resid=xa.x, ldo=D, ldr=D,
                     tile_hint=self._tile_hint("a", "x_tfa"))
            self._mm([xa.op, tl.op], ly["x_at"], p["c0_t"], M=rows, N=Dt, epilogue=L.EPI_RESID, resid=tl.x, ldo=Dt, ldr=Dt, tile_hint=ht)
            self._mm([xa.op, fl.op], ly["x_af"], p["c0_f"], M=rows, N=Df, epilogue=L.EPI_RESID, resid=fl.x, ldo=Df, ldr=Df, tile_hint=hf)
            p["c0_ok"] = True

    def begin_steps(self, y0):
        p, c = self.plan, self.cfg
        B, T, N, C_ = p["B"], p["T"], p["N"], c.num_channels
        if "y" not in p:
            p["y"] = torch.empty(B, T, C_, dtype=torch.float32, device=self.dev)
        y = p["y"]
        y.copy_(y0.to(self.dev, torch.float32))
        p["armed"] = False
        if p["c0_ok"] and "ybuf" in p and self._fold_ok(p):
            yb = p["ybuf"]
            for seq in range(p["Bt"]):
                r0 = seq * N + c.num_registers
                L.split_bf16(y[seq % B], yb.t[r0:r0 + T], rows=T, d=C_, ldy=yb.ld)
            p["armed"] = True
        return y

    def embed(self, y):
        p, c, W = self.plan, self.cfg, self.W
        B, Bt, T, N, D = p["B"], p["Bt"], p["T"], p["N"], c.dim
        x = p["xA"]
        L.linear_small(y, W.pin_wt, W.pin_b, p["padd"] if p["has_cond"] else W.pos_emb, x.x, M=B * T, K=c.num_channels, T=T,
                       out_batch_stride=N * D, row_off=c.num_registers, d=D, dup=(B if Bt > B else 0),
                       regs=W.regs, out_bf16=None if self.split or x.sh is None else x.sh.t)
        if self.split:
            L.split_bf16(x.x, x.sh.t, rows=Bt * N, d=D)
        if p["has_cond"]:
            self._mm([self._rows(p["condbuf"])], W.cond_w, x.x, M=B * N, N=D, epilogue=L.EPI_RESID, resid=x.x,
                     ldo=D, ldr=D, shadow=x.sh)

    def _cross_hints(self):
        on_side = self.dev.type == "cuda" and self.plan.get("st") is not None and not self.cross_on_main
        return (self._tile_hint("t", "cross"), self._tile_hint("f", "cross")) if on_side else (0, 0)

    def forward(self, n_ctx_seqs: int | None = None, folded: bool = False):
        p, c, W = self.plan, self.cfg, self.W
        B, Bt, N, rows = p["B"], p["Bt"], p["N"], p["rows"]
        D, Dt, Df = c.dim, c.dim_text, c.dim_frames
        nctx = B if n_ctx_seqs is None else n_ctx_seqs
        lens = p["seq_len"] if p["ragged"] else None
        half = c.depth // 2
        fz = self._fuse_skip()
        inner = c.heads * c.dim_head
        nkv = 2 * c.depth * inner
        xc, xo = p["xA"], p["xB"]
        tc_, fc_ = p["tL0"], p["fL0"]
        tbuf, fbuf = [p["tA"], p["tB"]], [p["fA"], p["fB"]]

        main = torch.cuda.current_stream() if self.dev.type == "cuda" else None
        st, sf = (p.get("st"), p.get("sf")) if main is not None else (None, None)
        multi = st is not None

        class _On:
            def __init__(self, s):
                self.s = s
            def __enter__(self):
                if multi:
                    self.ctx = torch.cuda.stream(self.s)
                    self.ctx.__enter__()
            def __exit__(self, *a):
                if multi:
                    self.ctx.__exit__(*a)

        def rec(stream):
            if not multi:
                return None
            e = torch.cuda.Event()
            e.record(stream)
            return e

        def wait(stream, *evs):
            if multi:
                for e in evs:
                    if e is not None:
                        stream.wait_event(e)

        eT = eF = None
        eA = rec(main) if not self.cross_on_main else None
        for i, ly in enumerate(W.layers):
            last = i == c.depth - 1
            wait(main, eT, eF)
            xn = p["skips"][i] if i < half else xo
            ax, at_, af_ = xc.op, tc_.op, fc_.op
            fused = fz and i >= half
            fold0 = folded and i == 0 and not fused
            if fused:
                wd = p["wide"][c.depth - 1 - i]
                ax = wd.x
                self._mm([wd.whole, at_, af_], ly["x_skip"], p["xS"], M=rows, N=D, ldo=D, tile_hint=self._tile_hint("a", "x_tfa"))
            elif fold0:
                self._mm([p["ybuf"]], W.fold_g[0], xn.x, M=rows, N=D, epilogue=L.EPI_RESID, resid=p["c0_a"], ldo=D, ldr=D,
                         shadow=xn.sh, tile_hint=self._tile_hint("a", "x_tfa"))
            else:
                self._mm([ax, at_, af_], ly["x_tfa"], xn.x, M=rows, N=D, epilogue=L.EPI_RESID, resid=xc.x, ldo=D, ldr=D,
                         shadow=xn.sh, tile_hint=self._tile_hint("a", "x_tfa"))
            if not last:
                nxt = W.layers[i + 1]
                on_side = multi and not self.cross_on_main
                hint_t = self._tile_hint("t", "cross") if on_side else 0
                hint = self._tile_hint("f", "cross") if on_side else 0
                def cross_t():
                    if fold0:
                        return self._mm([p["ybuf"]], W.fold_g[1], tbuf[0].x, M=rows, N=Dt,
                                        epilogue=L.EPI_RESID, resid=p["c0_t"], ldo=Dt, ldr=Dt, tile_hint=hint_t)
                    self._mm([ax, at_], ly["x_at"], tbuf[0].x, M=rows, N=Dt,
                             epilogue=L.EPI_RESID, resid=tc_.x, ldo=Dt, ldr=Dt, tile_hint=hint_t)
                def cross_f():
                    if fold0:
                        return self._mm([p["ybuf"]], W.fold_g[2], fbuf[0].x, M=rows, N=Df,
                                        epilogue=L.EPI_RESID, resid=p["c0_f"], ldo=Df, ldr=Df, tile_hint=hint)
                    self._mm([ax, af_], ly["x_af"], fbuf[0].x, M=rows, N=Df,
                             epilogue=L.EPI_RESID, resid=fc_.x, ldo=Df, ldr=Df, tile_hint=hint)
                if self.cross_on_main or not multi:
                    cross_t()
                    cross_f()
                    eX = rec(main)
                else:
                    eX = rec(main)
                    with _On(st):
                        wait(st, eA)
                        cross_t()
                    with _On(sf):
                        wait(sf, eA)
                        cross_f()
            src = xn.x if i < half else p["xS"]
            if i >= half and not fused:
                self._mm([xn.op, p["skips"][c.depth - 1 - i].op], ly["skip"], src, M=rows, N=D, ldo=D, tile_hint=self._tile_hint("a", "skip"))
            cv = ly["a_conv"]
            fold, fold2 = self._fold(), self._fold_gemm()
            cons = self._ncons("a", D)
            cons2 = cons if fold2 else {}
            x = xo.x
            r2 = nctx * N
            prod1 = {}
            if fold:
                ps, ss = p["per_sample_t"], p["norm_tab"].stride(0)
                L.dwconv(src, x, cv.wt, cv.b, B=Bt, N=N, d=D, ksize=cv.k, lens=lens,
                         norm=dict(out_bf16=p["hn_a"], ld_out_bf16=p["hn_a"].stride(-2), gamma=p["norm_tab"][0, i, 0], ssq=p["ssq_a"],
                                   split=self.split, **(dict(batch_stride=ss) if ps else dict(step=p["step"], step_stride=ss))))
            else:
                L.dwconv(src, x, cv.wt, cv.b, B=Bt, N=N, d=D, ksize=cv.k, lens=lens)
                self._norm_ada(x, p["hn_a"], rows, D, i, 0)
            if fold2:
                prod1 = self._nprod_ada(i, 1, switch_row=r2 if r2 < rows else 0) if nctx > 0 else self._nprod_ada(i, 2)
            self._self_attn(ly["a_attn"], x, "a", Bt, D, dict(epilogue=L.EPI_GATE_RESID, tile_hint=self._tile_hint("a", "out"),
                                                            **self._gate_kw(i, 0), **prod1), dict(tile_hint=self._tile_hint("a", "qkv"), **cons))
            if not last and self.interleave_capture:
                for part in (0, 1):
                    with _On(st):
                        if part == 0:
                            wait(st, eX)
                        self._side_block(nxt, "t", tbuf[0].x, tbuf[1], Bt, Dt, (part,))
                    with _On(sf):
                        if part == 0:
                            wait(sf, eX)
                        self._side_block(nxt, "f", fbuf[0].x, fbuf[1], Bt, Df, (part,))
            if nctx > 0:
                self._audio_cross_attention(i, ly, x, nctx, cons2, fold2, lens)
            if not fold2:
                self._norm_ada(x, p["hn_a"], rows, D, i, 2)
            xsh = dict(shadow=p["wide"][c.depth - 2 - i].x if (fz and half <= i + 1 < c.depth) else xo.sh)
            if last and fold2:
                xsh = dict(shadow=self._rows(p["hn_a"]), norm_gamma=W.final_g, norm_ssq=p["ssq_a"])
            self._ff(ly["a_ff"], x, "a", Bt, D, dict(epilogue=L.EPI_GATE_RESID, tile_hint=self._tile_hint("a", "ff2"), **self._gate_kw(i, 2), **xsh),
                     dict(tile_hint=self._tile_hint("a", "ff1"), **cons2))
            if not last:
                if not self.cross_on_main:
                    eA = rec(main)
                rest = (2,) if self.interleave_capture else (0, 1, 2)
                with _On(st):
                    if not self.interleave_capture:
                        wait(st, eX)
                    self._side_block(nxt, "t", tbuf[0].x, tbuf[1], Bt, Dt, rest)
                    eT = rec(st)
                with _On(sf):
                    if not self.interleave_capture:
                        wait(sf, eX)
                    self._side_block(nxt, "f", fbuf[0].x, fbuf[1], Bt, Df, rest)
                    eF = rec(sf)
                tc_, fc_ = tbuf[1], fbuf[1]
            xc, xo = xo, xc
        if self._fold_gemm():
            self._mm([self._rows(p["hn_a"])], W.pred_w, p["pred"], M=rows, N=c.num_channels, bias=W.pred_b, ldo=c.num_channels,
                     **self._ncons("a", D))
        else:
            L.rmsnorm(xc.x, p["hn_a"], rows=rows, d=D, gamma=W.final_g, split=self.split)
            self._mm([self._rows(p["hn_a"])], W.pred_w, p["pred"], M=rows, N=c.num_channels, bias=W.pred_b, ldo=c.num_channels)
        return p["pred"]

    def euler_step(self, y, cfg_strength: float, remove_parallel_component: bool = False, keep_parallel_frac: float = 0.0):
        p, c = self.plan, self.cfg
        folded = p["armed"] and self._fold_ok(p) and "y" in p and y.data_ptr() == p["y"].data_ptr()
        if not folded:
            self.embed(y)
        self.forward(folded=folded)
        kw = dict(B=p["B"], T=p["T"], C_=c.num_channels, pred_batch_stride=p["N"] * c.num_channels, row_off=c.num_registers)
        planes = None
        if folded:
            yb = p["ybuf"]
            planes = dict(out=yb.t, ld=yb.ld, lo_offset=yb.k, row_off=c.num_registers, rows_per_seq=p["N"], copies=p["Bt"] // p["B"])
        apg = None
        if remove_parallel_component:
            L.apg_reduce(p["pred"], p["apg"], valid_rows=p["valid_T"], **kw)
            apg = p["apg"]
        L.cfg_euler(y, p["pred"], cfg_strength=cfg_strength, dt=p["dt"], step=p["step"], apg=apg, keep=keep_parallel_frac, planes=planes, **kw)
        L.step_advance(p["step"])
```

Before: 3375 mel-frames/s.

## Defer side-stream handoff wait to FF output and add fused pred-GEMM CFG-Euler seam

Measured after the change: 3410 mel-frames/s, median of 6. 1.0% higher.

```diff
diff --git a/include/v2a_cfm.h b/include/v2a_cfm.h
--- a/include/v2a_cfm.h
+++ b/include/v2a_cfm.h
@@ -32,7 +32,8 @@
   V2A_EPI_GATE_RESID = 4,
   V2A_EPI_GEGLU_TANH = 5,
   V2A_EPI_GELU = 6,
-  V2A_EPI_SWIGLU = 7
+  V2A_EPI_SWIGLU = 7,
+  V2A_EPI_CFG_EULER = 8
 };
 
 typedef struct v2a_gemm_args {
@@ -216,6 +217,21 @@
 int v2a_split_bf16(const float* x, int64_t ldx, void* y, int64_t ldy, int64_t rows, int32_t d, v2a_stream_t stream);
 int v2a_cast_bf16(const float* x, void* y, int64_t n, v2a_stream_t stream);
 int v2a_step_advance(int32_t* step, v2a_stream_t stream);
+typedef struct v2a_step_seam {
+  float* y;
+  const float* dt;
+  int32_t* step;
+  uint32_t* arrive;
+  void* planes;
+  int64_t ld;
+  int64_t lo_offset;
+  int32_t B, T;
+  int32_t row_off;
+  int32_t rows_per_seq;
+  float cfg_strength;
+  int32_t reserved;
+} v2a_step_seam;
+int v2a_gemm_cfg_euler(const v2a_gemm_args* g, const v2a_step_seam* s, v2a_stream_t stream);
 
 
 int v2a_im2col(const float* x, int32_t B, int32_t H, int32_t W, int32_t C, int32_t kh, int32_t kw, int32_t stride,
diff --git a/video-to-audio-and-piano-rp_amd/_lib.py b/video-to-audio-and-piano-rp_amd/_lib.py
--- a/video-to-audio-and-piano-rp_amd/_lib.py
+++ b/video-to-audio-and-piano-rp_amd/_lib.py
@@ -103,6 +103,12 @@
                 ("copies", C.c_int32), ("reserved", C.c_int32)]
 
 
+class StepSeam(C.Structure):
+    _fields_ = [("y", C.c_void_p), ("dt", C.c_void_p), ("step", C.c_void_p), ("arrive", C.c_void_p), ("planes", C.c_void_p), ("ld", C.c_int64),
+                ("lo_offset", C.c_int64), ("B", C.c_int32), ("T", C.c_int32), ("row_off", C.c_int32), ("rows_per_seq", C.c_int32),
+                ("cfg_strength", C.c_float), ("reserved", C.c_int32)]
+
+
 class T5AttnArgs(C.Structure):
     _fields_ = [
         ("q", C.c_void_p), ("k", C.c_void_p), ("v", C.c_void_p), ("out", C.c_void_p),
@@ -140,7 +146,7 @@
     "v2a_xattn_absorb_prepare", "v2a_xattn_absorbed",
     "v2a_roll_expand_ratio", "v2a_piano_resize_vt",
     "v2a_roll_notes",
-    "v2a_cfg_euler_planes",
+    "v2a_cfg_euler_planes", "v2a_gemm_cfg_euler",
     "v2a_mel_pad", "v2a_mel_from_dft",
     "v2a_vocos_stage_in", "v2a_vocos_dwconv_ln", "v2a_vocos_gelu", "v2a_vocos_scale_residual", "v2a_vocos_spectrum", "v2a_vocos_overlap_add",
 ]
@@ -185,6 +191,7 @@
     lib.v2a_cfg_euler.argtypes = [vp, vp, i32, i32, i32, i64, i32, f32, vp, vp, vp, f32, vp]
     lib.v2a_cfg_euler_planes.argtypes = [vp, vp, i32, i32, i32, i64, i32, f32, vp, vp, vp, f32, C.POINTER(YPlanes), vp]
     lib.v2a_step_advance.argtypes = [vp, vp]
+    lib.v2a_gemm_cfg_euler.argtypes = [C.POINTER(GemmArgs), C.POINTER(StepSeam), vp]
     lib.v2a_cast_bf16.argtypes = [vp, vp, i64, vp]
     lib.v2a_split_bf16.argtypes = [vp, i64, vp, i64, i64, i32, vp]
     lib.v2a_im2col.argtypes = [vp, i32, i32, i32, i32, i32, i32, i32, i32, i32, i32, vp, i64, i32, i32, i32, vp]
@@ -597,6 +604,14 @@
     check(lib().v2a_step_advance(step.data_ptr(), stream_ptr()))
 
 
+def gemm_cfg_euler(a_segs, w, out, *, y, dt, step, arrive, planes, B, T, row_off, rows_per_seq, cfg_strength, **kw):
+    g, key, flops, nbytes = gemm_args(a_segs, w, out, **kw)
+    s = StepSeam(y.data_ptr(), dt.data_ptr(), step.data_ptr(), arrive.data_ptr(), planes["out"].data_ptr(), planes["ld"], planes["lo_offset"],
+                 B, T, row_off, rows_per_seq, float(cfg_strength), 0)
+    _launch(key.replace("store", "cfg_euler"), flops, nbytes + (8.0 + 8.0) * B * T * kw["N"],
+            lambda: lib().v2a_gemm_cfg_euler(C.byref(g), C.byref(s), stream_ptr()))
+
+
 def split_bf16(x, y, *, rows, d, ldx=None, ldy=None):
     _launch("split_bf16", 0.0, rows * d * 8, lambda: lib().v2a_split_bf16(x.data_ptr(), ldx or d, y.data_ptr(), ldy or 2 * d, rows, d, stream_ptr()))
 
diff --git a/video-to-audio-and-piano-rp_amd/csrc/gemm.hip b/video-to-audio-and-piano-rp_amd/csrc/gemm.hip
--- a/video-to-audio-and-piano-rp_amd/csrc/gemm.hip
+++ b/video-to-audio-and-piano-rp_amd/csrc/gemm.hip
@@ -156,6 +156,77 @@
                   a->out_dtype, a->compute_dtype);
 }
 
+
+template <int TM, int TN, int WM, int WN, int BM, int BN>
+__device__ __forceinline__ void gemm_epilogue_cfg_euler(const GemmParams& p, f32x4 (&acc)[TM][TN], float* tile, const float* rs, int tm, int n0,
+                                                        int wm, int wn, int tid) {
+  constexpr int LD = BN + 4, HB = BM / 2;
+  static_assert(BN / 4 == 16 && HB == 2 * 16, "256 threads: 16 lanes of four columns per row, two rows each");
+  const int lane = tid & 63, lr = lane & 15, lq = lane >> 4;
+  const int32_t stepv = p.seam.step[0];
+  float h = p.seam.dt[stepv];
+  float sv = p.seam.s;
+  asm volatile("" : "+v"(h), "+v"(sv));
+#pragma unroll
+  for (int i = 0; i < TM; ++i)
+#pragma unroll
+    for (int j = 0; j < TN; ++j)
+#pragma unroll
+      for (int jj = 0; jj < 4; ++jj) tile[(wm * WM + i * 16 + lq * 4 + jj) * LD + wn * WN + j * 16 + lr] = acc[i][j][jj];
+  __syncthreads();
+  if (tid == 0) {
+    const uint32_t nwg = gridDim.x;
+    if (atomicAdd(p.seam.arrive, 1u) == nwg - 1) {
+      atomicExch(p.seam.arrive, 0u);
+      p.seam.step[0] = stepv + 1;
+    }
+  }
+  const int c4 = (tid & 15) * 4, r0 = tid >> 4;
+  const int n = n0 + c4;
+  const int mh = p.M >> 1, N = p.N;
+  f32x4 bv = {0.f, 0.f, 0.f, 0.f};
+  if (p.bias) bv = *reinterpret_cast<const f32x4*>(p.bias + n);
+  float* out = reinterpret_cast<float*>(p.out);
+  const int rps = p.seam.rows_per_seq, row_off = p.seam.row_off, T = p.seam.T;
+#pragma unroll
+  for (int q = 0; q < HB / 16; ++q) {
+    const int r = r0 + q * 16;
+    const int m = tm * HB + r;
+    if (m >= mh) continue;
+    f32x4 pc = *reinterpret_cast<const f32x4*>(tile + r * LD + c4);
+    f32x4 pn = *reinterpret_cast<const f32x4*>(tile + (r + HB) * LD + c4);
+    if (rs) {
+      pc *= rs[r];
+      pn *= rs[r + HB];
+    }
+#pragma unroll
+    for (int e = 0; e < 4; ++e) {
+      pc[e] += bv[e];
+      pn[e] += bv[e];
+    }
+    *reinterpret_cast<f32x4*>(out + (int64_t)m * p.ldo + n) = pc;
+    *reinterpret_cast<f32x4*>(out + (int64_t)(mh + m) * p.ldo + n) = pn;
+    const int b = m / rps, t = m - b * rps - row_off;
+    if (t < 0 || t >= T) continue;
+    float* yp = p.seam.y + ((int64_t)b * T + t) * N + n;
+    f32x4 yv = *reinterpret_cast<const f32x4*>(yp);
+#pragma unroll
+    for (int e = 0; e < 4; ++e) yv[e] = cfg_euler_axpy(yv[e], pc[e], pc[e] - pn[e], h, sv);
+    *reinterpret_cast<f32x4*>(yp) = yv;
+    bf16x4 hi, lo;
+#pragma unroll
+    for (int e = 0; e < 4; ++e) {
+      hi[e] = (bf16_t)yv[e];
+      lo[e] = (bf16_t)(yv[e] - (float)hi[e]);
+    }
+#pragma unroll
+    for (int k = 0; k < 2; ++k) {
+      bf16_t* row = p.seam.planes + (int64_t)(k * mh + m) * p.seam.ldp + n;
+      *reinterpret_cast<bf16x4*>(row) = hi;
+      *reinterpret_cast<bf16x4*>(row + p.seam.lo_off) = lo;
+    }
+  }
+}
 
 
 template <int EPI, typename OutT, int BM, int BN, int WGM, int WGN, int NST = 3, bool S3 = false, int BK = 64>
@@ -186,6 +257,12 @@
   int tm, tn;
   tile_of_block(p, blockIdx.x, tm, tn);
   const int m0 = tm * BM, n0 = tn * BN;
+  constexpr bool SEAM = EPI == V2A_EPI_CFG_EULER;
+  static_assert(!SEAM || (S3 && BK == 64), "the step seam runs on the 64-wide K stage split ring");
+  auto seam_row = [&](int j) {
+    const int mh = p.M >> 1, r = tm * (BM / 2) + (j & (BM / 2 - 1));
+    return (j >= BM / 2 ? mh : 0) + (r < mh ? r : mh - 1);
+  };
 
   f32x4 acc[TM][TN];
 #pragma unroll
@@ -209,7 +286,7 @@
   for (int i = 0; i < LPW; ++i) {
     const int g = wave + i * NW;
     if (g < GA) {
-      const int r = m0 + g * RPG + srow;
+      const int r = SEAM ? seam_row(g * RPG + srow) : m0 + g * RPG + srow;
       grow[i] = r < p.M ? r : p.M - 1;
     } else {
       const int r = n0 + (g - GA) * RPG + srow;
@@ -271,12 +348,14 @@
 
   constexpr bool PF = BM * BN <= 128 * 256 && !((EPI == V2A_EPI_GATE_RESID || EPI == V2A_EPI_STORE) && BM * BN == 128 * 256);
   EpiPrefetch<EPI, TM, WN, PF> pf;
-  if (p.vec_epi) pf.load(p, m0 + wm * WM, n0 + wn * WN, lane);
+  if constexpr (!SEAM) {
+    if (p.vec_epi) pf.load(p, m0 + wm * WM, n0 + wn * WN, lane);
+  }
   static_assert(BM <= 64 * NW, "one thread per tile row");
   float* rs_lds = reinterpret_cast<float*>(smem_raw + NST * STAGE_BYTES);
   const bool scaled = p.rssq != nullptr && p.vec_epi;
   RowScaleLoad rsl;
-  if (scaled && tid < BM) rowscale_load(p, m0 + tid, rsl);
+  if (scaled && tid < BM) rowscale_load(p, SEAM ? seam_row(tid) : m0 + tid, rsl);
   const int nk = p.K / BK;
 #pragma unroll
   for (int s0 = 0; s0 < NST - 1; ++s0)
@@ -383,7 +462,11 @@
     if constexpr (NST > 4) { if (kt + 4 < nk) tile(std::integral_constant<int, 4>{}, kt + 4); }
     if constexpr (NST > 5) { if (kt + 5 < nk) tile(std::integral_constant<int, 5>{}, kt + 5); }
   }
-  if (p.vec_epi) {
+  if constexpr (SEAM) {
+    __builtin_amdgcn_s_barrier();
+    static_assert(BM * (BN + 4) * 4 <= NST * STAGE_BYTES, "the staged tile must fit in the ring memory");
+    gemm_epilogue_cfg_euler<TM, TN, WM, WN, BM, BN>(p, acc, reinterpret_cast<float*>(smem_raw), scaled ? rs_lds : nullptr, tm, n0, wm, wn, tid);
+  } else if (p.vec_epi) {
     __builtin_amdgcn_s_barrier();
     static_assert(NW * 16 * (WN + 4) * 4 <= NST * STAGE_BYTES, "epilogue slabs must fit in the ring memory");
     float* tile = reinterpret_cast<float*>(smem_raw) + wave * (16 * (WN + 4));
@@ -766,6 +849,36 @@
 
 extern "C" int v2a_gemm(const v2a_gemm_args* a, v2a_stream_t stream) { return gemm_dispatch(a, {(hipStream_t)stream, nullptr}); }
 
+extern "C" int v2a_gemm_cfg_euler(const v2a_gemm_args* a, const v2a_step_seam* s, v2a_stream_t stream) {
+  GemmParams p;
+  if (int rc = gemm_prepare(a, p)) return rc;
+  V2A_REQUIRE(s && s->y && s->dt && s->step && s->arrive && s->planes, "v2a_gemm_cfg_euler: null pointer");
+  V2A_REQUIRE(a->a_dtype == V2A_BF16_SPLIT && a->compute_dtype == V2A_BF16 && a->epilogue == V2A_EPI_STORE && a->out_dtype == V2A_F32 && p.vec_epi &&
+                  !a->out_bf16 && !a->rope_table && !a->relu && !a->a_row_offset && !a->a_ktile_offset && !a->out_row_offset && a->ldo >= a->N,
+              "v2a_gemm_cfg_euler: the GEMM must be a split-operand STORE launch with dense fp32 rows and no shadow, rope, relu or offset tables");
+  V2A_REQUIRE(a->N % 64 == 0 && s->B > 0 && s->T > 0 && s->row_off >= 0 && s->rows_per_seq >= s->row_off + s->T &&
+                  (int64_t)a->M == 2 * (int64_t)s->B * s->rows_per_seq,
+              "v2a_gemm_cfg_euler: N=%d (%% 64), M=%d = 2 * B (%d) * rows_per_seq (%d), rows_per_seq >= row_off (%d) + T (%d)", a->N, a->M, s->B,
+              s->rows_per_seq, s->row_off, s->T);
+  V2A_REQUIRE(((uintptr_t)s->y & 15) == 0 && ((uintptr_t)s->planes & 7) == 0 && s->lo_offset >= a->N && s->lo_offset % 4 == 0 && s->ld % 4 == 0 &&
+                  s->ld >= s->lo_offset + a->N,
+              "v2a_gemm_cfg_euler: y needs 16-byte, planes 8-byte alignment, lo_offset (%lld) >= N, ld (%lld) >= lo_offset + N, both multiples of 4",
+              (long long)s->lo_offset, (long long)s->ld);
+  constexpr int BM = 64, BN = 64, NST = 3, BK = 64;
+  const int bands = (a->M / 2 + BM / 2 - 1) / (BM / 2);
+  const int m_real = p.M;
+  p.M = bands * BM;
+  v2a_detail::fill_tile_map(p, BM, BN);
+  p.M = m_real;
+  p.seam = {s->y, s->dt, s->step, s->arrive, reinterpret_cast<bf16_t*>(s->planes), s->ld, s->lo_offset, s->rows_per_seq, s->row_off, s->T, s->cfg_strength};
+  constexpr size_t smem = NST * (size_t)(BM + BN) * (BK * 2) * 2 + BM * 4 + 16;
+  auto kern = gemm_bf16_dma_kernel<V2A_EPI_CFG_EULER, float, BM, BN, 2, 2, NST, true, BK>;
+  static std::atomic<uint64_t> lds_set{0};
+  if (int rc = v2a_enable_lds(reinterpret_cast<const void*>(kern), smem, lds_set, "v2a_gemm_cfg_euler")) return rc;
+  hipLaunchKernelGGL(kern, dim3(p.tiles_m * p.tiles_n), dim3(256), smem, (hipStream_t)stream, p);
+  return v2a_check_launch("v2a_gemm_cfg_euler");
+}
+
 extern "C" int v2a_gemm_choose(const v2a_gemm_args* a, v2a_gemm_choice* choice) {
   V2A_REQUIRE(choice != nullptr, "v2a_gemm_choose: null choice");
   *choice = {};
diff --git a/video-to-audio-and-piano-rp_amd/csrc/gemm_common.h b/video-to-audio-and-piano-rp_amd/csrc/gemm_common.h
--- a/video-to-audio-and-piano-rp_amd/csrc/gemm_common.h
+++ b/video-to-audio-and-piano-rp_amd/csrc/gemm_common.h
@@ -49,6 +49,16 @@
   int64_t out2_lo;
   int32_t s3_kl;
   int32_t dbg;
+  struct Seam {
+    float* y;
+    const float* dt;
+    int32_t* step;
+    uint32_t* arrive;
+    bf16_t* planes;
+    int64_t ldp, lo_off;
+    int32_t rows_per_seq, row_off, T;
+    float s;
+  } seam;
 };
 
 struct GemmTuning {
diff --git a/video-to-audio-and-piano-rp_amd/csrc/rowops.hip b/video-to-audio-and-piano-rp_amd/csrc/rowops.hip
--- a/video-to-audio-and-piano-rp_amd/csrc/rowops.hip
+++ b/video-to-audio-and-piano-rp_amd/csrc/rowops.hip
@@ -528,7 +528,7 @@
       const float par = coef * pc[j];
       upd = (upd - par) + par * keep;
     }
-    yv[j] += h * (pc[j] + upd * s);
+    yv[j] = cfg_euler_axpy(yv[j], pc[j], upd, h, s);
   }
   *reinterpret_cast<f32x4*>(y + e) = yv;
   return yv;
diff --git a/video-to-audio-and-piano-rp_amd/csrc/v2a_common.h b/video-to-audio-and-piano-rp_amd/csrc/v2a_common.h
--- a/video-to-audio-and-piano-rp_amd/csrc/v2a_common.h
+++ b/video-to-audio-and-piano-rp_amd/csrc/v2a_common.h
@@ -58,6 +58,7 @@
 }
 __device__ __forceinline__ float sigmoid_f(float x) { return 1.0f / (1.0f + __expf(-x)); }
 __device__ __forceinline__ float silu_f(float x) { return x / (1.0f + __expf(-x)); }
+__device__ __forceinline__ float cfg_euler_axpy(float y, float pc, float upd, float h, float s) { return y + h * (pc + upd * s); }
 __device__ __forceinline__ float silu_exact_f(float x) { return x / (1.0f + expf(-x)); }
 __device__ __forceinline__ float gelu_erf_f(float x) { return 0.5f * x * (1.0f + erff(x * 0.70710678118654752f)); }
 __device__ __forceinline__ float gelu_fast_f(float x) {
diff --git a/video-to-audio-and-piano-rp_amd/dit.py b/video-to-audio-and-piano-rp_amd/dit.py
--- a/video-to-audio-and-piano-rp_amd/dit.py
+++ b/video-to-audio-and-piano-rp_amd/dit.py
@@ -249,6 +249,23 @@
     return s
 
 
+class StreamHandoffs:
+
+    def current(self, dev):
+        return torch.cuda.current_stream() if dev.type == "cuda" else None
+
+    def on(self, stream):
+        return torch.cuda.stream(stream)
+
+    def rec(self, stream):
+        e = torch.cuda.Event()
+        e.record(stream)
+        return e
+
+    def wait(self, stream, event):
+        stream.wait_event(event)
+
+
 class DiTEngine:
 
     def __init__(self, cfg: DiTConfig, state_dict: dict, device="cuda", compute: str = "bf16",
@@ -271,7 +288,10 @@
         self.fuse_xattn = True
         self.absorb_xattn = os.environ.get("V2A_ABSORB_XATTN", "1") != "0"
         self.fold_embed = os.environ.get("V2A_FOLD_EMBED", "1") != "0"
+        self.fuse_step_seam = os.environ.get("V2A_FUSE_STEP_SEAM", "0") == "1"
         self.cross_on_main = False
+        self.late_ex = os.environ.get("V2A_LATE_EX", "1") != "0"
+        self.handoffs = StreamHandoffs()
         self.interleave_capture = False
         self._fuse_rope = compute != "fp32" and rope_layout == "interleaved"
         assert cfg.dim_head == 64, "kernels are built for dim_head = 64 (x3:717)"
@@ -347,6 +367,7 @@
         p["t_pts"] = e(S)
         p["dt"] = e(S)
         p["step"] = torch.zeros(1, dtype=torch.int32, device=dev)
+        p["arrive"] = torch.zeros(1, dtype=torch.int32, device=dev)
         p["apg"] = torch.zeros(2 * B, dtype=torch.float64, device=dev)
         p["valid_T"] = torch.full((1,), T, dtype=torch.int32, device=dev)
         p["seq_len"] = torch.full((Bt,), N, dtype=torch.int32, device=dev)
@@ -371,7 +392,7 @@
         p = self.plan
         return (p["ragged"], p["has_cond"], p["per_sample_t"], self.multi_stream, self.side_tile, tuple(sorted(self.side_tiles.items())),
                 tuple(sorted(self.big_tiles.items())), tuple(sorted(self.split_tiles.items())), tuple(sorted(self.split_big_tiles.items())), self.main_tile, self.fold_norm, self.fold_gemm_all, self.fuse_skip, self.fuse_xattn, self.cross_on_main,
-                self.interleave_capture, self.rope_cross, self.zero_masked_queries, self.absorb_xattn, p["xattn_kp"], self.fold_embed, p["armed"])
+                self.interleave_capture, self.rope_cross, self.zero_masked_queries, self.absorb_xattn, p["xattn_kp"], self.fold_embed, p["armed"], self.late_ex, self.fuse_step_seam)
 
     def _rows(self, t):
         return L.Operand(t, t.stride(-2), t.shape[-1] // (2 if self.split else 1))
@@ -460,12 +481,14 @@
                     scale=self.cfg.dim_head ** -0.5, softclamp=self.softclamp, dtype=self.adc, out_split=self.split)
         self._mm([self._rows(ao)], A.w_out, x, M=rows, N=d, resid=x, ldo=d, ldr=d, **out_kw)
 
-    def _ff(self, Fw: _FF, x, s, nseq, d, out_kw, in_kw={}):
+    def _ff(self, Fw: _FF, x, s, nseq, d, out_kw, in_kw={}, before_out=None):
         p = self.plan
         rows = nseq * p["N"]
         hn, ffh = p[f"hn_{s}"], p[f"ffh_{s}"]
         self._mm([self._rows(hn)], Fw.w1, ffh, M=rows, N=2 * Fw.inner, epilogue=L.EPI_GEGLU, bias=Fw.b1, ldo=ffh.stride(-2),
                  **(dict(out_split=True) if self.split else {}), **in_kw)
+        if before_out is not None:
+            before_out()
         self._mm([self._rows(ffh)], Fw.w2, x, M=rows, N=d, bias=Fw.b2, resid=x, ldo=d, ldr=d, **out_kw)
 
     def _tile_hint(self, stream, op):
@@ -482,7 +505,7 @@
         narrow = self.main_tile if op in ("x_tfa", "skip", "out", "out2", "ff2") else -1
         return max(self.side_tiles.get((stream, op), self.side_tile if side else narrow), -1) + 1
 
-    def _side_block(self, ly, s, src, dst, nseq, d, parts=(0, 1, 2)):
+    def _side_block(self, ly, s, src, dst, nseq, d, parts=(0, 1, 2), before_out=None):
         p = self.plan
         N, rows = p["N"], nseq * p["N"]
         lens = p["seq_len"] if p["ragged"] else None
@@ -507,7 +530,7 @@
         if 2 in parts:
             if not fold2:
                 self._norm_plain(x, hn, rows, d, ly[f"{s}_g2"])
-            self._ff(ly[f"{s}_ff"], x, s, nseq, d, dict(epilogue=L.EPI_RESID, tile_hint=h2, shadow=dst.sh), cons2)
+            self._ff(ly[f"{s}_ff"], x, s, nseq, d, dict(epilogue=L.EPI_RESID, tile_hint=h2, shadow=dst.sh), cons2, before_out=before_out)
 
     def _absorb(self, B, N, nc):
         c = self.cfg
@@ -736,7 +759,7 @@
         on_side = self.dev.type == "cuda" and self.plan.get("st") is not None and not self.cross_on_main
         return (self._tile_hint("t", "cross"), self._tile_hint("f", "cross")) if on_side else (0, 0)
 
-    def forward(self, n_ctx_seqs: int | None = None, folded: bool = False):
+    def forward(self, n_ctx_seqs: int | None = None, folded: bool = False, seam: dict | None = None):
         p, c, W = self.plan, self.cfg, self.W
         B, Bt, N, rows = p["B"], p["Bt"], p["N"], p["rows"]
         D, Dt, Df = c.dim, c.dim_text, c.dim_frames
@@ -750,33 +773,31 @@
         tc_, fc_ = p["tL0"], p["fL0"]
         tbuf, fbuf = [p["tA"], p["tB"]], [p["fA"], p["fB"]]
 
-        main = torch.cuda.current_stream() if self.dev.type == "cuda" else None
+        H = self.handoffs
+        main = H.current(self.dev)
         st, sf = (p.get("st"), p.get("sf")) if main is not None else (None, None)
         multi = st is not None
+        late = self.late_ex and multi and not self.cross_on_main and p["tA"].sh is not None and p["fA"].sh is not None
 
         class _On:
             def __init__(self, s):
                 self.s = s
             def __enter__(self):
                 if multi:
-                    self.ctx = torch.cuda.stream(self.s)
+                    self.ctx = H.on(self.s)
                     self.ctx.__enter__()
             def __exit__(self, *a):
                 if multi:
                     self.ctx.__exit__(*a)
 
         def rec(stream):
-            if not multi:
-                return None
-            e = torch.cuda.Event()
-            e.record(stream)
-            return e
+            return H.rec(stream) if multi else None
 
         def wait(stream, *evs):
             if multi:
                 for e in evs:
                     if e is not None:
-                        stream.wait_event(e)
+                        H.wait(stream, e)
 
         eT = eF = None
         eA = rec(main) if not self.cross_on_main else None
@@ -851,11 +872,11 @@
             if not last and self.interleave_capture:
                 for part in (0, 1):
                     with _On(st):
-                        if part == 0:
+                        if part == 0 and not late:
                             wait(st, eX)
                         self._side_block(nxt, "t", tbuf[0].x, tbuf[1], Bt, Dt, (part,))
                     with _On(sf):
-                        if part == 0:
+                        if part == 0 and not late:
                             wait(sf, eX)
                         self._side_block(nxt, "f", fbuf[0].x, fbuf[1], Bt, Df, (part,))
             if nctx > 0:
@@ -872,23 +893,26 @@
                     eA = rec(main)
                 rest = (2,) if self.interleave_capture else (0, 1, 2)
                 with _On(st):
-                    if not self.interleave_capture:
+                    if not self.interleave_capture and not late:
                         wait(st, eX)
-                    self._side_block(nxt, "t", tbuf[0].x, tbuf[1], Bt, Dt, rest)
+                    self._side_block(nxt, "t", tbuf[0].x, tbuf[1], Bt, Dt, rest, before_out=(lambda: wait(st, eX)) if late else None)
                     eT = rec(st)
                 with _On(sf):
-                    if not self.interleave_capture:
+                    if not self.interleave_capture and not late:
                         wait(sf, eX)
-                    self._side_block(nxt, "f", fbuf[0].x, fbuf[1], Bt, Df, rest)
+                    self._side_block(nxt, "f", fbuf[0].x, fbuf[1], Bt, Df, rest, before_out=(lambda: wait(sf, eX)) if late else None)
                     eF = rec(sf)
                 tc_, fc_ = tbuf[1], fbuf[1]
             xc, xo = xo, xc
+        pk = dict(M=rows, N=c.num_channels, bias=W.pred_b, ldo=c.num_channels)
         if self._fold_gemm():
-            self._mm([self._rows(p["hn_a"])], W.pred_w, p["pred"], M=rows, N=c.num_channels, bias=W.pred_b, ldo=c.num_channels,
-                     **self._ncons("a", D))
+            pk.update(self._ncons("a", D))
         else:
             L.rmsnorm(xc.x, p["hn_a"], rows=rows, d=D, gamma=W.final_g, split=self.split)
-            self._mm([self._rows(p["hn_a"])], W.pred_w, p["pred"], M=rows, N=c.num_channels, bias=W.pred_b, ldo=c.num_channels)
+        if seam is not None:
+            L.gemm_cfg_euler([self._rows(p["hn_a"])], W.pred_w, p["pred"], compute=L.BF16, a_split=True, **pk, **seam)
+        else:
+            self._mm([self._rows(p["hn_a"])], W.pred_w, p["pred"], **pk)
         return p["pred"]
 
     def euler_step(self, y, cfg_strength: float, remove_parallel_component: bool = False, keep_parallel_frac: float = 0.0):
@@ -896,6 +920,11 @@
         folded = p["armed"] and self._fold_ok(p) and "y" in p and y.data_ptr() == p["y"].data_ptr()
         if not folded:
             self.embed(y)
+        if folded and self.fuse_step_seam and not remove_parallel_component:
+            yb = p["ybuf"]
+            self.forward(folded=True, seam=dict(y=y, dt=p["dt"], step=p["step"], arrive=p["arrive"], planes=dict(out=yb.t, ld=yb.ld, lo_offset=yb.k),
+                                                B=p["B"], T=p["T"], row_off=c.num_registers, rows_per_seq=p["N"], cfg_strength=cfg_strength))
+            return
         self.forward(folded=folded)
         kw = dict(B=p["B"], T=p["T"], C_=c.num_channels, pred_batch_stride=p["N"] * c.num_channels, row_off=c.num_registers)
         planes = None
```
